# ai-forever/Kandinsky-2

Hardware: AMD Instinct MI355X
Metric: UNet denoise steps/sec @ 768x768 bs=1, 50 steps (higher is better)
Workload: dtype bf16; 1 GPU; Kandinsky-2.x text2img 768x768, decoder_steps=50, bs=1/GPU (CFG batch 2x4x96x96), 2.1-architecture UNet (1.23B) p_sampler step; parity pinned against the reference's modules; head=2.1, tile_configs_measured_in_this_process=0, images_per_gpu=1, parallelism=prompt-sharded x1, weights by one RCCL broadcast, world_size_observed=1, graph=True, chains=1, loop_graph=a 5-step loop replayed as ONE hipGraph (83 replay(s) = 415 timed steps)

## Files before the change

### include/k22.h

```cpp
#ifndef K22_H
#define K22_H
#include <stddef.h>
#include <stdint.h>
#ifdef __cplusplus
extern "C" {
#endif

#define K22_OK 0
#define K22_EINVAL (-1)
#define K22_EHIP (-2)
#define K22_ENOMEM (-3)

#define K22_BF16 0
#define K22_F32 1
#define K22_F16 2
#define K22_F16X3 3
#define K22_F16X2 4

int k22_version(void);
#define K22_BUILD_PACKED_FP32 1
#define K22_BUILD_DEBUG_VARIANTS 2
int k22_build_flags(void);
const char* k22_last_error(void);
int k22_set_option(const char* name, int value);
// ... 48 lines not shown

int k22_unet_sample_loop(K22UNet* u, float* x, float* x_tmp, const float* timesteps, const float* noise_seq, const float* init_img,
                         const float* mask, const float* inpaint_image, const float* inpaint_mask, const float* table,
                         const int* table_rows, int n_steps, float guidance, float clamp_lo, float clamp_hi, int pct_index,
                         double pct_gamma, void* scratch, int use_graph, void* stream);
enum { K22_LOOP_DDIM = 0, K22_LOOP_PLMS = 1 };
int k22_unet_ddim_loop(K22UNet* u, int kind, float* x, float* x_tmp, float* x0_out, const float* timesteps, const float* table,
                       const float* noise_seq, const float* inpaint_image, const float* inpaint_mask, float* eps_hist, int n_steps,
                       float guidance, int use_graph, void* stream);
int k22_unet_num_ops(const K22UNet* u);
int k22_unet_set_autotune(K22UNet* u, int on);
int k22_unet_tuning_report(const K22UNet* u, char* buf, size_t cap);

int k22_comm_broadcast_weights(void* arena, size_t bytes, int root, void* nccl_comm, void* stream);

int k22_tile_table_load(const char* path);
int k22_tile_table_save(const char* path);
int k22_tile_table_size(void);
int k22_tile_table_measured(void);
void k22_tile_table_clear(void);

int k22_unet_profile(K22UNet* u, int reps, double* ms, double* flops, double* bytes, int* launches, void* stream);

size_t k22_sampler_scratch_bytes(int N, int HW);
int k22_ddim_step(const float* x, const float* model_out, const float* noise, const float* table_row, float guidance, int use_cfg,
                  float* x_out, float* x0_out, int N, int HW, void* stream);
int k22_prepare_mask(const float* mask, float* out, int C, int H, int W, void* stream);
int k22_plms_step(const float* x, const float* model_out, const float* eps_hist1, const float* eps_hist2, const float* eps_hist3, int order,
                  const float* table_row, float guidance, int use_cfg, float* x_out, float* eps_out, float* x0_out, int N, int HW, void* stream);
int k22_sampler_step(const float* x, const float* model_out, const float* noise, const float* init_img,
                     const float* mask, const float* table, int step_index, float guidance, int use_cfg,
                     float clamp_lo, float clamp_hi, int pct_index, double pct_gamma, void* scratch,
                     float* x_out, float* x0_out, int N, int HW, void* stream);

int k22_gemm(const void* A0, const void* A1, const void* Wp, const float* bias, const void* residual, void* out,
             void* partial, int M, int N, int Npad, int K0, int K1, long lda0, long lda1, int ldo, int ldr,
             int out_f32, int act, int splitk, int bm, int bn, int dtype, void* stream);
int k22_x3_pack(const float* src, void* dst, long n, float scale, void* stream);
int k22_conv3x3(const void* x_padded, const void* Wp, const float* bias, const void* residual, void* out,
                void* partial, int B, int H, int W, int Cin, int Cout, int Npad, int out_mode, int act, int splitk,
                int bm, int bn, int dtype, void* stream);
int k22_conv3x3_skip(const void* x_padded, const void* Wp, const float* bias, const void* skip0, const void* skip1,
                     int SK0, int SK1, const void* Ws, const float* bias_s, void* out, void* partial, int B, int H, int W,
                     int Cin, int Cout, int Npad, int splitk, int bm, int dtype, void* stream);
int k22_conv3x3_gnstats(const void* x_padded, const void* Wp, const float* bias, const void* residual, void* out,
                        void* partial, int B, int H, int W, int Cin, int Cout, int Npad, int splitk, int bm, int bn,
                        float* stats, int stats_capacity_rows, int* rows_per_image, int dtype, void* stream);
int k22_gemm_gnstats(const void* A, const void* Wp, const float* bias, const void* residual, void* out, void* partial,
                     int B, int H, int W, int N, int Npad, int K, int splitk, int bm, float* stats,
                     int stats_capacity_rows, int* rows_per_image, int dtype, void* stream);
typedef struct K22IgemmProblem {
  int dtype, taps, M, N, Kc, K0, H, W;
  int out_mode, res_f32, act, a_raw, want_stats;
  int SK0, SK1;
  int att_T, att_S, att_Tkp;
  int ldo, ldr;
  int has_frag;
  int algo, bm, bn, splitk, stages;
} K22IgemmProblem;
typedef struct K22IgemmOperands {
  const void *A0, *A1, *Wp, *bias, *residual;
  void *out, *partial;
  const void *S0, *S1, *Ws, *bias2;
  void *kall, *vtall;
  const void *Wfrag, *Wsfrag;
  float* stats;
  int stats_capacity_rows;
} K22IgemmOperands;
int k22_igemm_cfg_accepted(const K22IgemmProblem* pr);
int k22_igemm_cfg(const K22IgemmProblem* pr, const K22IgemmOperands* ops, int* rows_per_image, void* stream);
int k22_debug_conv_trace(const void* x_padded, const void* Wp, const float* bias, void* out, int B, int H, int W, int Cin, int Cout,
                         int Npad, unsigned long long* trace, void* stream);
int k22_conv3x3_gn(const void* x0, const void* x1, int C0, int C1, const float* gamma, const float* beta, const float* film, long film_ld,
                   float eps, int act, void* scratch, const void* Wp, const float* bias, const void* residual, void* out, void* partial,
                   int B, int H, int W, int Cout, int Npad, int splitk, int bm, int algo, int dtype, void* stream);
int k22_groupnorm(const void* x0, const void* x1, int C0, int C1, int B, int H, int W, const float* gamma,
                  const float* beta, const float* film, long film_ld, float eps, int act, int mode, int pad,
                  void* scratch, void* out, int dtype, void* stream);
size_t k22_groupnorm_scratch_bytes(int B, int C);
int k22_attention(const void* qkv, const void* ctxkv, void* kall, void* vtall, void* out, int B, int H, int T, int S,
                  int dtype, void* stream);
int k22_qkv_project(const void* x, const void* Wp, const float* bias, void* q_out, void* kall, void* vtall,
                    int B, int H, int T, int S, int K, int bm, int bn, int dtype, void* stream);
int k22_qkv_project_stream(const void* x, const void* Wp, const float* bias, void* q_out, void* kall, void* vtall, void* partial,
                           int B, int H, int T, int S, int K, int bm, int splitk, int dtype, void* stream);
int k22_linear_smallm(const float* x, const void* W, const float* bias, const float* add, float* out, int M, int N,
                      int K, int act_in, int act_out, int wdtype, void* stream);
int k22_conv3x3_direct(const float* x, const float* w, const float* bias, float* y, int B, int Cin, int Cout, int Hin, int Win,
                       int stride, int act, void* stream);

size_t k22_afrag_bytes(int M, int K);
int k22_afrag_pack(const void* A, long lda, void* out, int M, int K, int dtype, void* stream);
int k22_skinny_gemm(const void* Afrag, const void* Wfrag, const float* bias, void* out, float* partial, int M, int N, int Npad, int K,
                    int splitk, int epi, int act, int ldo, int mt, int nb, int dtype, void* stream);
int k22_finish_ln(const float* partial, int splitk, const float* bias, float* x, long ldx, const float* gain, const float* beta, void* yfrag,
                  int M, int N, float eps, int dtype, void* stream);
int k22_small_attention(const void* qkv, const float* qkv_partial, int nsplit, const float* qkv_bias, void* out, int out_frag, int B, int H, int T,
                        int causal, const float* key_valid, int kv_n, int dtype, void* stream);

typedef struct K22PriorConfig {
  int dtype;
  int text_ctx;
  int xf_width;
  int xf_layers;
  int xf_heads;
  int xf_final_ln;
  int clip_dim;
  int clip_xf_width;
} K22PriorConfig;
typedef struct K22Prior K22Prior;
int k22_prior_create(const K22PriorConfig* cfg, const K22Weight* weights, int n_weights, K22Prior** out);
void k22_prior_destroy(K22Prior* m);
int k22_prior_plan(K22Prior* m, int B, size_t* workspace_bytes);
int k22_prior_bind(K22Prior* m, void* workspace, size_t workspace_bytes);
int k22_prior_tuning_report(const K22Prior* m, char* buf, size_t cap);
int k22_prior_forward(K22Prior* m, const float* x, const float* timesteps, const float* text_emb, const float* text_enc,
                      const float* key_valid, float* out, void* stream);
int k22_prior_sampler_step(const float* x, const float* model_out, const float* noise, const float* scales, const float* table_row,
                           float clamp, float* x_out, int bs, int D, void* stream);

typedef struct K22MoVQConfig {
  int dtype;
  int ch;
  int n_levels;
  int ch_mult[8];
  int num_res_blocks;
  int attn_levels;
  int z_channels;
  int out_ch;
} K22MoVQConfig;
typedef struct K22MoVQ K22MoVQ;
int k22_movq_create(const K22MoVQConfig* cfg, const K22Weight* weights, int n_weights, K22MoVQ** out);
void k22_movq_destroy(K22MoVQ* m);
int k22_movq_plan(K22MoVQ* m, int B, int h, int w, size_t* workspace_bytes);
int k22_movq_bind(K22MoVQ* m, void* workspace, size_t workspace_bytes);
int k22_movq_decode(K22MoVQ* m, const float* z, float* out, unsigned char* out_u8, void* stream);
int k22_movq_plan_encoder(K22MoVQ* m, int B, int H, int W, size_t* workspace_bytes);
int k22_movq_encode(K22MoVQ* m, const float* image, float* latent, void* stream);
int k22_movq_num_ops(const K22MoVQ* m);

enum { K22_ENC_CLIP_TEXT = 0, K22_ENC_CLIP_VISION = 1, K22_ENC_XLMR = 2 };
typedef struct K22EncoderConfig {
  int dtype;
  int kind;
  int width;
  int layers;
  int heads;
  int n_ctx;
  int vocab;
  int out_dim;
  int image_size;
  int patch;
  int max_pos;
  int pad_id;
  float ln_eps;
  int mlp_dim;
  int hidden_act;
} K22EncoderConfig;
typedef struct K22Encoder K22Encoder;
int k22_encoder_create(const K22EncoderConfig* cfg, const K22Weight* weights, int n_weights, K22Encoder** out);
void k22_encoder_destroy(K22Encoder* m);
int k22_encoder_plan(K22Encoder* m, int B, size_t* workspace_bytes);
int k22_encoder_bind(K22Encoder* m, void* workspace, size_t workspace_bytes);
int k22_encoder_forward(K22Encoder* m, const int* tokens, const float* key_valid, const float* image, float* seq_out, float* pooled_out,
                        void* stream);

// ... 34 lines not shown
```

### kandinsky-2_amd/_lib.py

```python
from __future__ import annotations

import ctypes as C
import os

_HERE = os.path.dirname(os.path.abspath(__file__))
LIB_PATH = os.environ.get("K22_LIB_PATH") or os.path.join(_HERE, "libk22hip.so")
TILE_TABLE_PATH = os.path.join(_HERE, "tiles_gfx950.txt")

K22_BF16, K22_F32, K22_F16, K22_F16X3, K22_F16X2 = 0, 1, 2, 3, 4
K22_LOOP_DDIM, K22_LOOP_PLMS = 0, 1
F16X3 = "f16x3"
F16X2 = "f16x2"
SPLIT_DTYPES = (F16X3, F16X2)
X3_WSCALE = 256.0


def dtype_code(backend_dtype) -> int:
    import torch
    try:
        return {torch.bfloat16: K22_BF16, torch.float32: K22_F32, torch.float16: K22_F16, F16X3: K22_F16X3, F16X2: K22_F16X2}[backend_dtype]
    except KeyError:
        raise ValueError('backend_dtype must be torch.bfloat16, torch.float16, torch.float32 "f16x3" or "f16x2"') from None
ACT_NONE, ACT_SILU, ACT_GELU = 0, 1, 2
OUT_ROWMAJOR, OUT_ROWMAJOR_F32, OUT_NCHW_F32, OUT_QKV = 0, 1, 2, 3
# ... 32 lines not shown


class K22EncoderConfig(C.Structure):
    _fields_ = [("dtype", C.c_int), ("kind", C.c_int), ("width", C.c_int), ("layers", C.c_int), ("heads", C.c_int), ("n_ctx", C.c_int),
                ("vocab", C.c_int), ("out_dim", C.c_int), ("image_size", C.c_int), ("patch", C.c_int), ("max_pos", C.c_int),
                ("pad_id", C.c_int), ("ln_eps", C.c_float), ("mlp_dim", C.c_int), ("hidden_act", C.c_int)]


class K22Weight(C.Structure):
    _fields_ = [("name", C.c_char_p), ("ptr", C.c_void_p)]


_P, _I, _L, _F, _D, _Z = C.c_void_p, C.c_int, C.c_long, C.c_float, C.c_double, C.c_size_t

SIGNATURES = {
    "k22_version": (_I, []),
    "k22_build_flags": (_I, []),
    "k22_last_error": (C.c_char_p, []),
    "k22_set_option": (_I, [C.c_char_p, _I]),
    "k22_comm_broadcast_weights": (_I, [_P, _Z, _I, _P, _P]),
    "k22_tile_table_load": (_I, [C.c_char_p]),
    "k22_tile_table_save": (_I, [C.c_char_p]),
    "k22_tile_table_size": (_I, []),
    "k22_tile_table_measured": (_I, []),
    "k22_tile_table_clear": (None, []),
    "k22_unet_create": (_I, [C.POINTER(K22UNetConfig), C.POINTER(K22Weight), _I, C.POINTER(_P)]),
    "k22_unet_destroy": (None, [_P]),
    "k22_unet_plan": (_I, [_P, _I, _I, _I, C.POINTER(_Z)]),
    "k22_unet_bind": (_I, [_P, _P, _Z]),
    "k22_unet_set_condition": (_I, [_P, _P, _P, _P, _P]),
    "k22_unet_set_hint": (_I, [_P, _P, _P]),
    "k22_unet_forward": (_I, [_P, _P, _P, _P, _P, _P, _I, _P]),
    "k22_unet_sample_loop": (_I, [_P, _P, _P, _P, _P, _P, _P, _P, _P, _P, C.POINTER(_I), _I, _F, _F, _F, _I, _D, _P, _I, _P]),
    "k22_unet_ddim_loop": (_I, [_P, _I, _P, _P, _P, _P, _P, _P, _P, _P, _P, _I, _F, _I, _P]),
    "k22_unet_num_ops": (_I, [_P]),
    "k22_unet_set_autotune": (_I, [_P, _I]),
    "k22_unet_tuning_report": (_I, [_P, C.c_char_p, _Z]),
    "k22_unet_profile": (_I, [_P, _I, C.POINTER(_D), C.POINTER(_D), C.POINTER(_D), C.POINTER(_I), _P]),
    "k22_afrag_bytes": (_Z, [_I, _I]),
    "k22_afrag_pack": (_I, [_P, _L, _P, _I, _I, _I, _P]),
    "k22_skinny_gemm": (_I, [_P, _P, _P, _P, _P, _I, _I, _I, _I, _I, _I, _I, _I, _I, _I, _I, _P]),
    "k22_finish_ln": (_I, [_P, _I, _P, _P, _L, _P, _P, _P, _I, _I, _F, _I, _P]),
    "k22_small_attention": (_I, [_P, _P, _I, _P, _P, _I, _I, _I, _I, _I, _P, _I, _I, _P]),
    "k22_prior_create": (_I, [C.POINTER(K22PriorConfig), C.POINTER(K22Weight), _I, C.POINTER(_P)]),
    "k22_prior_destroy": (None, [_P]),
    "k22_prior_plan": (_I, [_P, _I, C.POINTER(_Z)]),
    "k22_prior_bind": (_I, [_P, _P, _Z]),
    "k22_prior_tuning_report": (_I, [_P, C.c_char_p, _Z]),
    "k22_prior_forward": (_I, [_P, _P, _P, _P, _P, _P, _P, _P]),
    "k22_prior_sampler_step": (_I, [_P, _P, _P, _P, _P, _F, _P, _I, _I, _P]),
    "k22_encoder_create": (_I, [C.POINTER(K22EncoderConfig), C.POINTER(K22Weight), _I, C.POINTER(_P)]),
    "k22_encoder_destroy": (None, [_P]),
    "k22_encoder_plan": (_I, [_P, _I, C.POINTER(_Z)]),
    "k22_encoder_bind": (_I, [_P, _P, _Z]),
    "k22_encoder_forward": (_I, [_P, _P, _P, _P, _P, _P, _P]),
    "k22_movq_create": (_I, [C.POINTER(K22MoVQConfig), C.POINTER(K22Weight), _I, C.POINTER(_P)]),
    "k22_movq_destroy": (None, [_P]),
    "k22_movq_plan": (_I, [_P, _I, _I, _I, C.POINTER(_Z)]),
    "k22_movq_bind": (_I, [_P, _P, _Z]),
    "k22_movq_decode": (_I, [_P, _P, _P, _P, _P]),
    "k22_movq_plan_encoder": (_I, [_P, _I, _I, _I, C.POINTER(_Z)]),
    "k22_movq_encode": (_I, [_P, _P, _P, _P]),
    "k22_movq_num_ops": (_I, [_P]),
    "k22_ddim_step": (_I, [_P, _P, _P, _P, _F, _I, _P, _P, _I, _I, _P]),
    "k22_blend_noised": (_I, [_P, _P, _P, _P, _F, _F, _P, _I, _I, _I, _I, _P]),
    "k22_prepare_mask": (_I, [_P, _P, _I, _I, _I, _P]),
    "k22_plms_step": (_I, [_P, _P, _P, _P, _P, _I, _P, _F, _I, _P, _P, _P, _I, _I, _P]),
    "k22_sampler_scratch_bytes": (_Z, [_I, _I]),
    "k22_sampler_step": (_I, [_P, _P, _P, _P, _P, _P, _I, _F, _I, _F, _F, _I, _D, _P, _P, _P, _I, _I, _P]),
    "k22_gemm": (_I, [_P, _P, _P, _P, _P, _P, _P, _I, _I, _I, _I, _I, _L, _L, _I, _I, _I, _I, _I, _I, _I, _I, _P]),
    "k22_x3_pack": (_I, [_P, _P, _L, _F, _P]),
    "k22_conv3x3": (_I, [_P, _P, _P, _P, _P, _P, _I, _I, _I, _I, _I, _I, _I, _I, _I, _I, _I, _I, _P]),
    "k22_conv3x3_skip": (_I, [_P, _P, _P, _P, _P, _I, _I, _P, _P, _P, _P, _I, _I, _I, _I, _I, _I, _I, _I, _I, _P]),
    "k22_gemm_gnstats": (_I, [_P, _P, _P, _P, _P, _P, _I, _I, _I, _I, _I, _I, _I, _I, _P, _I, C.POINTER(_I), _I, _P]),
    "k22_conv3x3_gnstats": (_I, [_P, _P, _P, _P, _P, _P, _I, _I, _I, _I, _I, _I, _I, _I, _I, _P, _I, C.POINTER(_I), _I, _P]),
    "k22_igemm_cfg_accepted": (_I, [C.POINTER(K22IgemmProblem)]),
    "k22_igemm_cfg": (_I, [C.POINTER(K22IgemmProblem), C.POINTER(K22IgemmOperands), C.POINTER(_I), _P]),
    "k22_conv3x3_gn": (_I, [_P, _P, _I, _I, _P, _P, _P, _L, _F, _I, _P, _P, _P, _P, _P, _P, _I, _I, _I, _I, _I, _I, _I, _I, _I, _P]),
    "k22_debug_conv_trace": (_I, [_P, _P, _P, _P, _I, _I, _I, _I, _I, _I, _P, _P]),
    "k22_groupnorm": (_I, [_P, _P, _I, _I, _I, _I, _I, _P, _P, _P, _L, _F, _I, _I, _I, _P, _P, _I, _P]),
    "k22_groupnorm_scratch_bytes": (_Z, [_I, _I]),
    "k22_attention": (_I, [_P, _P, _P, _P, _P, _I, _I, _I, _I, _I, _P]),
    "k22_qkv_project": (_I, [_P, _P, _P, _P, _P, _P, _I, _I, _I, _I, _I, _I, _I, _I, _P]),
    "k22_qkv_project_stream": (_I, [_P, _P, _P, _P, _P, _P, _P, _I, _I, _I, _I, _I, _I, _I, _I, _P]),
    "k22_linear_smallm": (_I, [_P, _P, _P, _P, _P, _I, _I, _I, _I, _I, _I, _P]),
    "k22_conv3x3_direct": (_I, [_P, _P, _P, _P, _I, _I, _I, _I, _I, _I, _I, _P]),
    "k22_debug_counter": (_L, [C.c_char_p]),
    "k22_stream_frag_bytes": (C.c_size_t, [_I, _I, _I, _I]),
    "k22_stream_repack": (_I, [_P, _P, _I, _I, _I, _I, _P]),
    "k22_debug_set_stream_frag": (_I, [_P, _P]),
    "k22_debug_set_stream_scratch": (_I, [_P, C.c_size_t]),
    "k22_spatialnorm_apply": (_I, [_P, _P, _P, _P, _P, _P, _P, _P, _I, _I, _I, _I, _I, _I, _I, _I, _I, _I, _P]),
    "k22_upsample2_pad": (_I, [_P, _P, _I, _I, _I, _I, _I, _P]),
    "k22_pad_copy": (_I, [_P, _P, _I, _I, _I, _I, _I, _P]),
    "k22_subsample_odd": (_I, [_P, _P, _I, _I, _I, _I, _I, _P]),
    "k22_softmax_rows": (_I, [_P, _L, _I, _F, _I, _P]),
    "k22_movq_prepare": (_I, [_P, _P, _P, _P, _P, _I, _I, _I, _I, _I, _P]),
    "k22_movq_enc_prepare": (_I, [_P, _P, _I, _I, _I, _I, _I, _P]),
    "k22_movq_quant_conv": (_I, [_P, _P, _P, _P, _I, _I, _P]),
    "k22_to_uint8_nhwc": (_I, [_P, _P, _I, _I, _I, _I, _P]),
    "k22_enc_layernorm": (_I, [_P, _L, _P, _P, _P, _L, _P, _I, _I, _F, _I, _P]),
    "k22_enc_embed": (_I, [_P, _P, _P, _P, _P, _I, _I, _I, _I, _I, _I, _I, _P]),
    "k22_enc_gather_eot": (_I, [_P, _P, _P, _I, _I, _I, _P]),
    "k22_enc_masked_mean": (_I, [_P, _P, _P, _I, _I, _I, _P]),
    "k22_enc_patchify": (_I, [_P, _P, _I, _I, _I, _I, _I, _P]),
    "k22_enc_vision_assemble": (_I, [_P, _P, _P, _P, _I, _I, _I, _P]),
    "k22_enc_mlp_act": (_I, [_P, _P, _L, _I, _I, _P]),
    "k22_enc_attention_generic": (_I, [_P, _P, _I, _I, _I, _I, _I, _P]),
    "k22_prior_layernorm": (_I, [_P, _L, _P, _P, _P, _I, _I, _I, _I, _P]),
    "k22_prior_finish_input": (_I, [_P, _P, _P, _I, _I, _I, _P]),
    "k22_attention_masked": (_I, [_P, _P, _P, _P, _P, _I, _I, _I, _I, _I, _P, _I, _I, _I, _P]),
}

_lib = None


def lib() -> C.CDLL:
    global _lib
    if _lib is None:
        if not os.path.exists(LIB_PATH):
            raise RuntimeError(
                f"{LIB_PATH} is missing: the HIP extension is the only compute path (no CPU fallback). "
                "Build it with `python -c 'import __graft_entry__ as g; g.build()'`.")
        l = C.CDLL(LIB_PATH)
        for name, (res, args) in SIGNATURES.items():
            fn = getattr(l, name)
            fn.restype = res
            fn.argtypes = args
        _lib = l
        tbl = os.environ.get("K22_TILE_TABLE", TILE_TABLE_PATH)
        if tbl != "0" and os.path.exists(tbl):
            if l.k22_tile_table_load(tbl.encode()) < 0:
                raise RuntimeError(f"k22: cannot read the tile table {tbl}")
    return _lib


def check(rc: int) -> None:
    if rc != 0:
        msg = lib().k22_last_error()
        raise RuntimeError(f"k22 error {rc}: {msg.decode() if msg else ''}")


def weight_array(arena, table):
    base = arena.data_ptr()
    arr = (K22Weight * len(table))()
    names = []
    for i, (name, (off, _n)) in enumerate(table.items()):
        nb = name.encode()
        names.append(nb)
        arr[i].name = nb
        arr[i].ptr = base + off
    return arr, names


def plan_and_bind(plan_fn, bind_fn, handle, device, *shape):
    import torch
    nbytes = C.c_size_t()
    check(plan_fn(handle, *shape, C.byref(nbytes)))
    ws = torch.empty(nbytes.value + 256, dtype=torch.uint8, device=device)
    check(bind_fn(handle, (ws.data_ptr() + 255) // 256 * 256, nbytes.value))
    return ws


def ptr(t) -> int:
    if t is None:
        return None
# ... 8 lines not shown
```

### kandinsky-2_amd/csrc/capi.hip

```cpp
#include "kernels.h"
#include "elementwise.h"
#include "../../include/k22.h"
#include "tuning.h"
#include "skinny.h"
#include <dlfcn.h>
#include <stdio.h>
#include <string.h>

static thread_local char g_err[512] = "";

int k22_set_error(int code, const char* msg) {
  snprintf(g_err, sizeof(g_err), "%s", msg ? msg : "");
  return code;
}
int k22_set_error_hip(hipError_t e, const char* file, int line) {
  snprintf(g_err, sizeof(g_err), "HIP error %d (%s) at %s:%d", (int)e, hipGetErrorString(e), file, line);
  return K22_EHIP;
}

extern "C" {

int k22_version(void) { return 100; }
int k22_build_flags(void) {
  int f = 0;
#ifndef K22_NOPK
  f |= K22_BUILD_PACKED_FP32;
#endif
#if defined(K22_DEBUG_VARIANTS) || defined(K22_STREAM_DEBUG) || defined(K22_SKINNY_DEBUG)
  f |= K22_BUILD_DEBUG_VARIANTS;
#endif
  return f;
}

int k22_set_option(const char* name, int value) {
  if (name && !strcmp(name, "igemm_stages")) { igemm_set_default_stages(value); return K22_OK; }
  if (name && !strcmp(name, "igemm_xcd_remap")) { igemm_set_xcd_remap(value); return K22_OK; }
  if (name && !strcmp(name, "conv_algo")) { igemm_set_conv_algo(value); return K22_OK; }
  if (name && !strcmp(name, "gemm_algo")) { igemm_set_gemm_algo(value); return K22_OK; }
  if (name && !strcmp(name, "att_pipe")) { attention_set_pipe(value); return K22_OK; }
  return k22_set_error(K22_EINVAL, "k22_set_option: unknown option");
}
const char* k22_last_error(void) { return g_err; }

#ifdef K22_STREAM_DEBUG
static unsigned long long* g_dbg_trace = nullptr;
extern "C" int k22_debug_set_stream_trace(unsigned long long* t) { g_dbg_trace = t; return K22_OK; }
#define K22_DBG_TRACE(p) (p).st_trace = g_dbg_trace
#else
#define K22_DBG_TRACE(p) (void)0
#endif
static const void* g_dbg_wfrag = nullptr;
static const void* g_dbg_wsfrag = nullptr;
static void* g_dbg_scratch = nullptr;
static size_t g_dbg_scratch_bytes = 0;
static int dbg_frag(IgemmParams& p, int dtype, hipStream_t st) {
  K22_DBG_TRACE(p);
  p.Wfrag = g_dbg_wfrag; p.Wsfrag = g_dbg_wsfrag;
  if (g_dbg_wfrag || !g_dbg_scratch || dtype == K22_F32 || (p.taps != 1 && p.taps != 9) || p.Kc % 64 || p.Npad % 64) return K22_OK;
  const size_t n1 = stream_frag_bytes(p.Npad, p.taps, p.Kc, dtype);
  const bool skip = p.S0 != nullptr && p.Ws != nullptr && (p.SK0 + p.SK1) % 64 == 0;
  const size_t n2 = skip ? stream_frag_bytes(p.Npad, 1, p.SK0 + p.SK1, dtype) : 0;
  if (n1 + n2 > g_dbg_scratch_bytes) return k22_set_error(K22_ENOMEM, "debug stream scratch too small");
  if (int rc = launch_stream_repack(p.Wp, g_dbg_scratch, p.Npad, p.taps, p.Kc, dtype, st)) return rc;
  p.Wfrag = g_dbg_scratch;
  if (skip) {
    void* w2 = static_cast<char*>(g_dbg_scratch) + n1;
    if (int rc = launch_stream_repack(p.Ws, w2, p.Npad, 1, p.SK0 + p.SK1, dtype, st)) return rc;
    p.Wsfrag = w2;
  }
  return K22_OK;
}
#define K22_DBG_FRAG(p) do { if (int rc_ = dbg_frag((p), dtype, reinterpret_cast<hipStream_t>(stream))) return rc_; } while (0)
int k22_debug_set_stream_frag(const void* wfrag, const void* wsfrag) { g_dbg_wfrag = wfrag; g_dbg_wsfrag = wsfrag; return K22_OK; }
int k22_debug_set_stream_scratch(void* scratch, size_t bytes) { g_dbg_scratch = scratch; g_dbg_scratch_bytes = scratch ? bytes : 0; return K22_OK; }
size_t k22_stream_frag_bytes(int Npad, int taps, int Kc, int dtype) { return stream_frag_bytes(Npad, taps, Kc, dtype); }
int k22_stream_repack(const void* W, void* out, int Npad, int taps, int Kc, int dtype, void* stream) {
  return launch_stream_repack(W, out, Npad, taps, Kc, dtype, reinterpret_cast<hipStream_t>(stream));
}

long k22_debug_counter(const char* name) {
  if (name && !strcmp(name, "stream_launches")) return stream_launch_count();
  if (name && !strcmp(name, "loop_captures")) return loop_capture_count();
  if (name && !strcmp(name, "loop_launches")) return loop_launch_count();
  return -1;
}

int k22_comm_broadcast_weights(void* arena, size_t bytes, int root, void* nccl_comm, void* stream) {
  if (!arena || !nccl_comm) return k22_set_error(K22_EINVAL, "k22_comm_broadcast_weights: null arena / communicator");
  typedef int (*bcast_fn)(const void*, void*, size_t, int , int, void*, hipStream_t);
  static bcast_fn fn = nullptr;
  if (!fn) {
    void* sym = dlsym(RTLD_DEFAULT, "ncclBroadcast");
    if (!sym) {
      void* h = dlopen("librccl.so.1", RTLD_NOW | RTLD_GLOBAL);
      if (!h) h = dlopen("librccl.so", RTLD_NOW | RTLD_GLOBAL);
      if (h) sym = dlsym(h, "ncclBroadcast");
    }
    if (!sym) return k22_set_error(K22_EINVAL, "k22_comm_broadcast_weights: RCCL (ncclBroadcast) is not loadable in this process");
    fn = reinterpret_cast<bcast_fn>(sym);
  }
  const size_t piece = (size_t)1 << 30;
  char* base = reinterpret_cast<char*>(arena);
  for (size_t off = 0; off < bytes; off += piece) {
    const size_t n = bytes - off < piece ? bytes - off : piece;
    const int rc = fn(base + off, base + off, n,  1, root, nccl_comm, reinterpret_cast<hipStream_t>(stream));
    if (rc != 0) { char msg[96]; snprintf(msg, sizeof msg, "k22_comm_broadcast_weights: ncclBroadcast returned %d", rc); return k22_set_error(K22_EHIP, msg); }
  }
  return K22_OK;
}

int k22_tile_table_load(const char* path) {
  if (!path) return k22_set_error(K22_EINVAL, "k22_tile_table_load: null path");
  const int n = tile_table_load_file(path);
  if (n < 0) return k22_set_error(K22_EINVAL, "k22_tile_table_load: cannot read the file");
  return n;
}
int k22_tile_table_save(const char* path) {
  if (!path) return k22_set_error(K22_EINVAL, "k22_tile_table_save: null path");
  const int n = tile_table_save_file(path);
  if (n < 0) return k22_set_error(K22_EINVAL, "k22_tile_table_save: cannot write the file");
  return n;
}
int k22_tile_table_size(void) {
  TileTable& tt = tile_table();
  std::lock_guard<std::mutex> lk(tt.mu);
  return (int)tt.m.size();
}
int k22_tile_table_measured(void) {
  TileTable& tt = tile_table();
  std::lock_guard<std::mutex> lk(tt.mu);
  return (int)tt.measured;
}
void k22_tile_table_clear(void) {
  TileTable& tt = tile_table();
  std::lock_guard<std::mutex> lk(tt.mu);
  tt.m.clear();
  tt.measured = 0;
}

int k22_gemm(const void* A0, const void* A1, const void* Wp, const float* bias, const void* residual, void* out,
             void* partial, int M, int N, int Npad, int K0, int K1, long lda0, long lda1, int ldo, int ldr,
             int out_f32, int act, int splitk, int bm, int bn, int dtype, void* stream) {
  IgemmParams p = {};
    p.stages = -1;
  p.A0 = A0; p.A1 = A1; p.Wp = Wp; p.bias = bias; p.residual = residual; p.out = out;
  p.partial = reinterpret_cast<float*>(partial);
  p.M = M; p.N = N; p.Npad = Npad; p.Kc = K0 + K1; p.K0 = K0; p.taps = 1; p.lda0 = lda0; p.lda1 = lda1;
  p.ldo = ldo; p.ldr = ldr; p.out_mode = out_f32 ? IG_OUT_ROWMAJOR_F32 : IG_OUT_ROWMAJOR; p.act = act;
  p.splitk = splitk; p.force_bm = bm; p.force_bn = bn;
  p.a_raw = k22_is_split(dtype) ? 1 : 0;
  if (p.splitk == 0) p.splitk = partial ? igemm_choose_splitk(p, dtype) : 1;
  K22_DBG_FRAG(p);
  return launch_igemm(p, dtype, reinterpret_cast<hipStream_t>(stream));
}

int k22_x3_pack(const float* src, void* dst, long n, float scale, void* stream) {
  if (!src || !dst || n < 0) return k22_set_error(K22_EINVAL, "x3_pack: null argument");
  return launch_x3_pack(src, dst, n, scale, reinterpret_cast<hipStream_t>(stream));
}

int k22_conv3x3(const void* x_padded, const void* Wp, const float* bias, const void* residual, void* out,
                void* partial, int B, int H, int W, int Cin, int Cout, int Npad, int out_mode, int act, int splitk,
                int bm, int bn, int dtype, void* stream) {
  IgemmParams p = {};
    p.stages = -1;
  p.A0 = x_padded; p.Wp = Wp; p.bias = bias; p.residual = residual; p.out = out;
// ... 127 lines not shown
  }
  return launch_igemm(q, d.dtype, reinterpret_cast<hipStream_t>(stream));
}

int k22_debug_conv_trace(const void* x_padded, const void* Wp, const float* bias, void* out, int B, int H, int W, int Cin, int Cout,
                         int Npad, unsigned long long* trace, void* stream) {
  IgemmParams p = {};
  p.stages = -1;
  p.A0 = x_padded; p.Wp = Wp; p.bias = bias; p.out = out;
  p.M = B * H * W; p.N = Cout; p.Npad = Npad; p.Kc = Cin; p.K0 = Cin; p.taps = 9; p.H = H; p.W = W;
  p.ldo = Cout; p.ldr = Cout; p.out_mode = IG_OUT_ROWMAJOR; p.act = K22_ACT_NONE; p.splitk = 1; p.trace = trace;
  return launch_conv3_halo_trace(p, K22_BF16, reinterpret_cast<hipStream_t>(stream));
}

size_t k22_groupnorm_scratch_bytes(int B, int C) {
  return (size_t)B * 128 * C * 2 * sizeof(float) + (size_t)B * C * 2 * sizeof(float) + 512;
}

int k22_groupnorm(const void* x0, const void* x1, int C0, int C1, int B, int H, int W, const float* gamma,
                  const float* beta, const float* film, long film_ld, float eps, int act, int mode, int pad,
                  void* scratch, void* out, int dtype, void* stream) {
  hipStream_t st = reinterpret_cast<hipStream_t>(stream);
  const int C = C0 + C1, HW = H * W;
  const int out_x3 = k22_is_split(dtype) ? 1 : 0;
  dtype = k22_storage_dtype(dtype);
  float* partial = reinterpret_cast<float*>(scratch);
  float* coeff = partial + (size_t)B * 128 * C * 2;
  const int rc = launch_gn_stats_coeff(x0, x1, C0, C1, B, HW, eps, gamma, beta, film, film_ld, partial, coeff, dtype, st);
  if (rc) return rc;
  GnApplyParams ap = {};
  ap.x0 = x0; ap.x1 = x1; ap.C0 = C0; ap.C1 = C1; ap.B = B; ap.H = H; ap.W = W; ap.mode = mode; ap.pad = pad; ap.act = act;
  ap.coeff = coeff; ap.out = out; ap.out_x3 = out_x3;
  return launch_gn_apply(ap, dtype, st);
}

int k22_conv3x3_gn(const void* x0, const void* x1, int C0, int C1, const float* gamma, const float* beta, const float* film, long film_ld,
                   float eps, int act, void* scratch, const void* Wp, const float* bias, const void* residual, void* out, void* partial,
                   int B, int H, int W, int Cout, int Npad, int splitk, int bm, int algo, int dtype, void* stream) {
  hipStream_t st = reinterpret_cast<hipStream_t>(stream);
  const int C = C0 + C1, HW = H * W;
  const int sdt = k22_storage_dtype(dtype);
  float* part = reinterpret_cast<float*>(scratch);
  float* coeff = part + (size_t)B * 128 * C * 2;
  const int rc = launch_gn_stats_coeff(x0, x1, C0, C1, B, HW, eps, gamma, beta, film, film_ld, part, coeff, sdt, st);
  if (rc) return rc;
  IgemmParams p = {};
  p.stages = -1;
  p.Wp = Wp; p.bias = bias; p.residual = residual; p.out = out; p.partial = reinterpret_cast<float*>(partial);
  p.M = B * H * W; p.N = Cout; p.Npad = Npad; p.Kc = C; p.K0 = C; p.taps = 9; p.H = H; p.W = W;
  p.ldo = Cout; p.ldr = Cout; p.out_mode = IG_OUT_ROWMAJOR; p.act = K22_ACT_NONE; p.splitk = splitk > 0 ? splitk : 1; p.force_bm = bm; p.algo = algo;
  p.gn_coeff = coeff; p.gn_x0 = x0; p.gn_x1 = x1; p.gn_C0 = C0; p.gn_act = act;
  return launch_igemm(p, dtype, st);
}


int k22_attention(const void* qkv, const void* ctxkv, void* kall, void* vtall, void* out, int B, int H, int T, int S,
                  int dtype, void* stream) {
  hipStream_t st = reinterpret_cast<hipStream_t>(stream);
  const int C = H * 64, Tk = S + T, Tkp = (Tk + 63) / 64 * 64;
  KvPackParams kp;
  kp.qkv = qkv; kp.ctxkv = ctxkv; kp.kall = kall; kp.vtall = vtall; kp.B = B; kp.H = H; kp.T = T; kp.S = S; kp.Tkp = Tkp;
  int rc = launch_kv_pack(kp, k22_storage_dtype(dtype), st);
  if (rc) return rc;
  AttentionParams ap = {};
  ap.q = qkv; ap.ldq = 3 * C; ap.kall = kall; ap.vtall = vtall; ap.out = out; ap.ldo = C;
  ap.B = B; ap.H = H; ap.T = T; ap.Tk = Tk; ap.Tkp = Tkp; ap.scale = 0.125f;
  return launch_attention(ap, dtype, st);
}

int k22_qkv_project(const void* x, const void* Wp, const float* bias, void* q_out, void* kall, void* vtall,
                    int B, int H, int T, int S, int K, int bm, int bn, int dtype, void* stream) {
  const int C = H * 64, Tkp = (S + T + 63) / 64 * 64;
  IgemmParams p = {};
  p.stages = -1;
  p.A0 = x; p.Wp = Wp; p.bias = bias; p.out = q_out; p.kall = kall; p.vtall = vtall;
  p.M = B * T; p.N = 3 * C; p.Npad = 3 * C; p.Kc = K; p.K0 = K; p.taps = 1; p.lda0 = K; p.lda1 = 0;
  p.ldo = C; p.ldr = 3 * C; p.out_mode = IG_OUT_QKV; p.act = K22_ACT_NONE; p.splitk = 1; p.force_bm = bm; p.force_bn = bn;
  p.att_T = T; p.att_S = S; p.att_Tkp = Tkp; p.H = 1; p.W = T;
  p.a_raw = k22_is_split(dtype) ? 1 : 0;
  K22_DBG_FRAG(p);
  return launch_igemm(p, dtype, reinterpret_cast<hipStream_t>(stream));
}

int k22_qkv_project_stream(const void* x, const void* Wp, const float* bias, void* q_out, void* kall, void* vtall, void* partial,
                           int B, int H, int T, int S, int K, int bm, int splitk, int dtype, void* stream) {
  const int C = H * 64, Tkp = (S + T + 63) / 64 * 64;
  IgemmParams p = {};
  p.stages = -1;
  p.A0 = x; p.Wp = Wp; p.bias = bias; p.out = q_out; p.kall = kall; p.vtall = vtall; p.partial = reinterpret_cast<float*>(partial);
  p.M = B * T; p.N = 3 * C; p.Npad = 3 * C; p.Kc = K; p.K0 = K; p.taps = 1; p.lda0 = K; p.lda1 = 0;
  p.ldo = C; p.ldr = 3 * C; p.out_mode = IG_OUT_QKV; p.act = K22_ACT_NONE; p.splitk = splitk > 0 ? splitk : 1; p.force_bm = bm; p.algo = 20;
  p.att_T = T; p.att_S = S; p.att_Tkp = Tkp; p.H = 1; p.W = T;
  if (!stream_supported(p, dtype, bm == 288 ? 9 : 5)) return k22_set_error(K22_EINVAL, "qkv_project_stream: unsupported problem");
  K22_DBG_FRAG(p);
  return launch_igemm(p, dtype, reinterpret_cast<hipStream_t>(stream));
}

size_t k22_afrag_bytes(int M, int K) { return afrag_bytes(M, K); }
int k22_afrag_pack(const void* A, long lda, void* out, int M, int K, int dtype, void* stream) {
  return launch_afrag_pack(A, lda, out, M, K, dtype, reinterpret_cast<hipStream_t>(stream));
}
int k22_skinny_gemm(const void* Afrag, const void* Wfrag, const float* bias, void* out, float* partial, int M, int N, int Npad, int K,
                    int splitk, int epi, int act, int ldo, int mt, int nb, int dtype, void* stream) {
  SkinnyParams q = {};
  q.Af = Afrag; q.Wf = Wfrag; q.bias = bias; q.out = out; q.partial = partial; q.M = M; q.N = N; q.Npad = Npad; q.K = K; q.MA = (M + 31) / 32;
  q.splitk = splitk > 0 ? splitk : 1; q.epi = epi; q.act = act; q.ldo = ldo;
  q.trace = reinterpret_cast<unsigned long long*>(g_dbg_scratch);
  return launch_skinny(q, dtype, mt, nb, reinterpret_cast<hipStream_t>(stream));
}
int k22_finish_ln(const float* partial, int splitk, const float* bias, float* x, long ldx, const float* gain, const float* beta, void* yfrag,
                  int M, int N, float eps, int dtype, void* stream) {
  FinishLnParams q = {};
  q.partial = partial; q.splitk = splitk; q.bias = bias; q.x = x; q.ldx = ldx; q.g = gain; q.b = beta; q.yfrag = yfrag; q.M = M; q.N = N;
  q.MA = (M + 31) / 32; q.eps = eps;
  return launch_finish_ln(q, dtype, reinterpret_cast<hipStream_t>(stream));
}
int k22_small_attention(const void* qkv, const float* qkv_partial, int nsplit, const float* qkv_bias, void* out, int out_frag, int B, int H, int T,
                        int causal, const float* key_valid, int kv_n, int dtype, void* stream) {
  SmallAttnParams ap = {};
  ap.qkv = qkv; ap.part = qkv_partial; ap.nsplit = nsplit; ap.bias = qkv_bias; ap.ldq = 3 * H * 64; ap.out = out; ap.ldo = H * 64; ap.out_frag = out_frag; ap.MA = (B * T + 31) / 32;
  ap.B = B; ap.H = H; ap.T = T; ap.scale = 0.125f; ap.causal = causal; ap.key_valid = key_valid; ap.kv_ld = kv_n; ap.kv_n = kv_n;
  return launch_small_attention(ap, dtype, reinterpret_cast<hipStream_t>(stream));
}

int k22_linear_smallm(const float* x, const void* W, const float* bias, const float* add, float* out, int M, int N,
                      int K, int act_in, int act_out, int wdtype, void* stream) {
  LinearSmallParams lp = {};
  lp.x = x; lp.ldx = K; lp.W = W; lp.bias = bias; lp.add = add; lp.ld_add = N; lp.out = out; lp.ldo = N;
  lp.M = M; lp.N = N; lp.K = K; lp.act_in = act_in; lp.act_out = act_out;
  return launch_linear_smallm(lp, wdtype, reinterpret_cast<hipStream_t>(stream));
}

int k22_conv3x3_direct(const float* x, const float* w, const float* bias, float* y, int B, int Cin, int Cout, int Hin, int Win,
                       int stride, int act, void* stream) {
  if (!x || !w || !bias || !y) return k22_set_error(K22_EINVAL, "conv3x3_direct: null argument");
  if (B < 1 || Cin < 1 || Cout < 1 || Hin < 1 || Win < 1) return k22_set_error(K22_EINVAL, "conv3x3_direct: empty shape");
  if (act != K22_ACT_NONE && act != K22_ACT_SILU) return k22_set_error(K22_EINVAL, "conv3x3_direct: act must be 0 (none) or 1 (SiLU)");
  ConvDirectParams p = {};
  p.x = x; p.w = w; p.bias = bias; p.y = y;
  p.B = B; p.Cin = Cin; p.Cout = Cout; p.Hin = Hin; p.Win = Win; p.stride = stride; p.act = act;
  return launch_conv3x3_direct(p, reinterpret_cast<hipStream_t>(stream));
}

int k22_ddim_step(const float* x, const float* model_out, const float* noise, const float* table_row, float guidance, int use_cfg,
                  float* x_out, float* x0_out, int N, int HW, void* stream) {
  if (!x || !model_out || !table_row || !x_out) return k22_set_error(K22_EINVAL, "ddim_step: null argument");
  return launch_ddim_step(x, model_out, noise, table_row, guidance, use_cfg, x_out, x0_out, N, HW, reinterpret_cast<hipStream_t>(stream));
}

int k22_prepare_mask(const float* mask, float* out, int C, int H, int W, void* stream) {
  if (!mask || !out) return k22_set_error(K22_EINVAL, "prepare_mask: null argument");
  return launch_prepare_mask(mask, out, C, H, W, reinterpret_cast<hipStream_t>(stream));
}

int k22_plms_step(const float* x, const float* model_out, const float* eps_hist1, const float* eps_hist2, const float* eps_hist3, int order,
                  const float* table_row, float guidance, int use_cfg, float* x_out, float* eps_out, float* x0_out, int N, int HW, void* stream) {
  if (!x || !model_out || !table_row || !x_out) return k22_set_error(K22_EINVAL, "plms_step: null argument");
  return launch_plms_step(x, model_out, eps_hist1, eps_hist2, eps_hist3, order, table_row, guidance, use_cfg, x_out, eps_out, x0_out, N, HW,
                          reinterpret_cast<hipStream_t>(stream));
}

size_t k22_sampler_scratch_bytes(int N, int HW) { return (size_t)N * 4 * HW * sizeof(float) + 256; }

int k22_sampler_step(const float* x, const float* model_out, const float* noise, const float* init_img,
                     const float* mask, const float* table, int step_index, float guidance, int use_cfg,
                     float clamp_lo, float clamp_hi, int pct_index, double pct_gamma, void* scratch,
// ... 98 lines not shown
```

### kandinsky-2_amd/csrc/conv3_halo.hip

```cpp
#include "conv3_common.h"

int launch_conv3_halo_spec(const IgemmParams& p, int dtype, int bm, int nbst, int splitk, hipStream_t stream);
#ifdef K22_DEBUG_VARIANTS
int launch_conv3_halo_spec_debug(const IgemmParams& p, int nbst, int splitk, hipStream_t stream);
#endif

template <typename T, int BM, int NBST, bool TRACE = false, int LW = 8, int MODE = 0>
__global__ __launch_bounds__(512) void conv3_halo_kernel(const IgemmParams p) {
  constexpr bool PIPE = MODE == 1;
  constexpr bool GASM = MODE == 1 || MODE == 2;
  constexpr bool DBG_NOLOAD = MODE == 3;
  constexpr bool DBG_NOMMA = MODE == 4;
  using TR = TT<T>;
  constexpr int BK = TR::BK, EPC = TR::EPC, KSTEPS = TR::KSTEPS;
  constexpr int BN = HALO_BN, NW = LW, WM = 4, WN = 2;
  constexpr int MI = BM / (WM * 32), NI = BN / (WN * 32);
  constexpr int B_SLOTS = BN / 8 / NW;
  constexpr int B_BYTES = BN * 128;
  constexpr int APT = HALO_NW / LW;
  constexpr int A_SLOTS = (10 - NBST) * APT;
  constexpr int GM = 8;
  extern __shared__ __attribute__((aligned(16))) char smem[];

  const int tid = threadIdx.x, lane = tid & 63;
// ... 130 lines not shown
          constexpr int ta_ = ((TAP) + NBST - 1) % 9;                                                      \
          const int sa_ = ((TAP) + NBST - 1 >= 9) ? sn : s;                                                \
          K22_ISSUE_B(sa_, ta_, fill);                                                                     \
          if constexpr ((TAP) <= 9 - NBST) {                                                               \
            _Pragma("unroll") for (int a_ = 0; a_ < APT; ++a_) {                                           \
              constexpr int qb_ = ((TAP) <= 9 - NBST ? (TAP) : 0) * APT;                                   \
              K22_ISSUE_A(qb_ + a_, sn, Anext);                                                            \
            }                                                                                              \
          }                                                                                                \
        }                                                                                                  \
        const char* Bcur = Bst + cur * B_BYTES;                                                            \
        const int shift = ((TAP) / 3) * W2 + ((TAP) % 3);                                                  \
        const char* arow[MI];                                                                              \
        int asw[MI];                                                                                       \
        _Pragma("unroll") for (int mi = 0; mi < MI; ++mi) {                                                \
          const int ar = abase + mi * 32 + shift;                                                          \
          arow[mi] = Acur + ar * 128;                                                                      \
          asw[mi] = (ar >> 1) & 7;                                                                         \
        }                                                                                                  \
        if constexpr (PIPE) {                                                                              \
          FragA<T> ca[MI];                                                                                 \
          Frag<T> cb[NI];                                                                                  \
          _Pragma("unroll") for (int ks = 0; ks < KSTEPS; ks += 2) {                                       \
            _Pragma("unroll") for (int mi = 0; mi < MI; ++mi) ld_frag_at(ca[mi], arow[mi], asw[mi], ks, h); \
            _Pragma("unroll") for (int ni = 0; ni < NI; ++ni) ld_frag_at(cb[ni], Bcur + brow[ni], bsw, ks, h); \
            __builtin_amdgcn_sched_barrier(0);                                                             \
            _Pragma("unroll") for (int mi = 0; mi < MI; ++mi)                                              \
              _Pragma("unroll") for (int ni = 0; ni < NI; ++ni) mma_atom(acc[mi][ni], pb[ni], pa[mi]);     \
            __builtin_amdgcn_sched_barrier(0);                                                             \
            _Pragma("unroll") for (int mi = 0; mi < MI; ++mi) ld_frag_at(pa[mi], arow[mi], asw[mi], ks + 1, h); \
            _Pragma("unroll") for (int ni = 0; ni < NI; ++ni) ld_frag_at(pb[ni], Bcur + brow[ni], bsw, ks + 1, h); \
            __builtin_amdgcn_sched_barrier(0);                                                             \
            _Pragma("unroll") for (int mi = 0; mi < MI; ++mi)                                              \
              _Pragma("unroll") for (int ni = 0; ni < NI; ++ni) mma_atom(acc[mi][ni], cb[ni], ca[mi]);     \
            __builtin_amdgcn_sched_barrier(0);                                                             \
          }                                                                                                \
           \
          asm volatile("s_waitcnt lgkmcnt(0)" ::: "memory");                                               \
        } else {                                                                                           \
        _Pragma("unroll") for (int ks = 0; ks < KSTEPS; ++ks) {                                            \
          FragA<T> a[MI];                                                                                  \
          Frag<T> b[NI];                                                                                   \
          _Pragma("unroll") for (int mi = 0; mi < MI; ++mi) ld_frag_at(a[mi], arow[mi], asw[mi], ks, h);   \
          _Pragma("unroll") for (int ni = 0; ni < NI; ++ni) ld_frag_at(b[ni], Bcur + brow[ni], bsw, ks, h); \
          if constexpr (DBG_NOMMA) {                                                                       \
            _Pragma("unroll") for (int mi = 0; mi < MI; ++mi) asm volatile("" ::"v"(a[mi].v));             \
            _Pragma("unroll") for (int ni = 0; ni < NI; ++ni) asm volatile("" ::"v"(b[ni].v));             \
          } else {                                                                                         \
          _Pragma("unroll") for (int mi = 0; mi < MI; ++mi)                                                \
            _Pragma("unroll") for (int ni = 0; ni < NI; ++ni) mma_atom(acc[mi][ni], b[ni], a[mi]);         \
          }                                                                                                \
        }                                                                                                  \
         \
        asm volatile("s_waitcnt lgkmcnt(0)" ::: "memory");                                                 \
        }                                                                                                  \
        if constexpr (TRACE) {                                                                             \
                      \
          asm volatile("" ::"v"(acc[0][0][0]), "v"(acc[MI - 1][NI - 1][15]));                             \
          const unsigned long long tr3_ = __builtin_amdgcn_s_memtime();                                    \
          if (blockIdx.x == 0 && (wave == 0 || wave == 5) && lane == 0 && p.trace != nullptr) {            \
            unsigned long long* o_ = p.trace + ((size_t)(wave ? 1 : 0) * 4096 + (size_t)trace_it * 4);     \
            if (trace_it < 1024) { o_[0] = tr0_; o_[1] = tr1_; o_[2] = tr2_; o_[3] = tr3_; }                \
          }                                                                                                \
          ++trace_it;                                                                                      \
        }                                                                                                  \
        cur = (cur + 1 == NBST) ? 0 : cur + 1;                                                             \
        fill = (fill + 1 == NBST) ? 0 : fill + 1;                                                          \
      }
      K22_TAP(0) K22_TAP(1) K22_TAP(2) K22_TAP(3) K22_TAP(4) K22_TAP(5) K22_TAP(6) K22_TAP(7) K22_TAP(8)
#undef K22_TAP
    }
  }
#undef K22_ISSUE_A
#undef K22_ISSUE_B
  if constexpr (PIPE) {
#pragma unroll
    for (int mi = 0; mi < MI; ++mi)
#pragma unroll
      for (int ni = 0; ni < NI; ++ni) mma_atom(acc[mi][ni], pb[ni], pa[mi]);
  }
  halo_tail<T, BM>(p, acc, smem, bx, bz, img, v0, n0);
}

template <typename T, int BM, int NST, bool ARAW = false>
__global__ __launch_bounds__(512) void gemm8_kernel(const IgemmParams p) {
  using TR = TT<T>;
  constexpr int BK = TR::BK, EPC = TR::EPC, KSTEPS = TR::KSTEPS;
  constexpr int BN = HALO_BN, NW = HALO_NW, WM = 4, WN = 2;
  constexpr int MI = BM / (WM * 32), NI = BN / (WN * 32);
  constexpr int A_SLOTS = BM / 8 / NW, B_SLOTS = BN / 8 / NW, CH = A_SLOTS + B_SLOTS;
  constexpr int A_BYTES = BM * 128, B_BYTES = BN * 128, BUF = A_BYTES + B_BYTES;
  constexpr int GM = 8;
  extern __shared__ __attribute__((aligned(16))) char smem[];

  const int tid = threadIdx.x, lane = tid & 63;
  const int wave = __builtin_amdgcn_readfirstlane(tid >> 6);
  const int wm = wave >> 1, wn = wave & 1;
  const int h = lane >> 5, l31 = lane & 31;

  const int HW = p.H > 0 ? p.H * p.W : p.M;
  const int TPI = (HW + BM - 1) / BM;
  const int B = p.M / HW;
  const int gx = B * TPI, gy = (p.N + BN - 1) / BN;
  int L = p.xcd_remap ? xcd_remap_h(blockIdx.x, gridDim.x) : (int)blockIdx.x;
  const int per_z = gx * gy;
  const int bz = L / per_z;
  L -= bz * per_z;
  const int grp = L / (GM * gy);
  const int first_m = grp * GM;
  const int gsz = gx - first_m < GM ? gx - first_m : GM;
  const int lin = L - grp * GM * gy;
  const int bx = first_m + lin % gsz, by = lin / gsz;
  const int img = bx / TPI, v0 = (bx - img * TPI) * BM;
  const int n0 = by * BN;

  const T* __restrict__ A = reinterpret_cast<const T*>(p.A0) + (int64_t)img * HW * p.lda0;
  const T* __restrict__ Wp = reinterpret_cast<const T*>(p.Wp);
  int aoff[A_SLOTS], boff[B_SLOTS];
#pragma unroll
  for (int i = 0; i < A_SLOTS; ++i) {
    const int row = 8 * (wave + NW * i) + (lane >> 3);
    int v = v0 + row;
    if (v > HW - 1) v = HW - 1;
    aoff[i] = v * (int)p.lda0 + ((lane & 7) ^ ((row >> 1) & 7)) * EPC;
  }
#pragma unroll
  for (int i = 0; i < B_SLOTS; ++i) {
    const int row = 8 * (wave + NW * i) + (lane >> 3);
    int n = n0 + row;
    if (n > p.Npad - 1) n = p.Npad - 1;
    boff[i] = n * p.Kc + ((lane & 7) ^ ((row >> 1) & 7)) * EPC;
  }
  const int nslab = p.Kc / BK;
  int s0 = 0, s1 = nslab;
  if (p.splitk > 1) {
    const int per = (nslab + p.splitk - 1) / p.splitk;
    s0 = bz * per;
    s1 = s0 + per < nslab ? s0 + per : nslab;
  }

  f32x16_t acc[MI][NI];
#pragma unroll
  for (int mi = 0; mi < MI; ++mi)
#pragma unroll
    for (int ni = 0; ni < NI; ++ni)
#pragma unroll
      for (int r = 0; r < 16; ++r) acc[mi][ni][r] = 0.f;

  const unsigned lds0 = __builtin_amdgcn_readfirstlane((unsigned)(size_t)(__attribute__((address_space(3))) char*)smem);
#define K22_ISSUE_G(SLAB, STAGE)                                                                           \
  {                                                                                                        \
    int sl_ = (SLAB);                                                                                      \
    if (sl_ > s1 - 1) sl_ = s1 - 1;       \
    const unsigned d_ = lds0 + (STAGE) * BUF + wave * 1024;                                                \
    _Pragma("unroll") for (int i = 0; i < A_SLOTS; ++i)                                                    \
        glds16_asm(A + aoff[i] + sl_ * BK, __builtin_amdgcn_readfirstlane(d_ + i * NW * 1024));            \
    _Pragma("unroll") for (int i = 0; i < B_SLOTS; ++i)                                                    \
        glds16w_asm(Wp + boff[i] + sl_ * BK, __builtin_amdgcn_readfirstlane(d_ + A_BYTES + i * NW * 1024)); \
  }
  int arow[MI], brow[NI];
#pragma unroll
  for (int mi = 0; mi < MI; ++mi) arow[mi] = (wm * (BM / WM) + mi * 32 + l31) * 128;
#pragma unroll
  for (int ni = 0; ni < NI; ++ni) brow[ni] = A_BYTES + (wn * (BN / WN) + ni * 32 + l31) * 128;
  const int sw = (l31 >> 1) & 7;

  if (s0 < s1) {
#pragma unroll
    for (int t = 0; t < NST - 1; ++t) K22_ISSUE_G(s0 + t, t);
    int cur = 0, fill = NST - 1;
    for (int s = s0; s < s1; ++s) {
      wait_vmcnt<(NST - 2) * CH>();
      raw_barrier();
      K22_ISSUE_G(s + NST - 1, fill);
      const char* St = smem + cur * BUF;
#pragma unroll
      for (int ks = 0; ks < KSTEPS; ++ks) {
        FragA<T> a[MI];
        Frag<T> b[NI];
#pragma unroll
        for (int mi = 0; mi < MI; ++mi) ld_frag_at_a<ARAW, T>(a[mi], St + arow[mi], sw, ks, h);
#pragma unroll
        for (int ni = 0; ni < NI; ++ni) ld_frag_at(b[ni], St + brow[ni], sw, ks, h);
#pragma unroll
        for (int mi = 0; mi < MI; ++mi)
#pragma unroll
          for (int ni = 0; ni < NI; ++ni) mma_atom(acc[mi][ni], b[ni], a[mi]);
      }
      cur = (cur + 1 == NST) ? 0 : cur + 1;
      fill = (fill + 1 == NST) ? 0 : fill + 1;
    }
  }
#undef K22_ISSUE_G
  halo_tail<T, BM, true>(p, acc, smem, bx, bz, img, v0, n0);
}

template <typename T, int BM, int NST>
__global__ __launch_bounds__(512) void gemm8_spec_kernel(const IgemmParams p) {
  using TR = TT<T>;
  static_assert(sizeof(T) == 2, "gemm8_spec_kernel: 16-bit operands");
  constexpr int BK = TR::BK, EPC = TR::EPC, KSTEPS = TR::KSTEPS;
  static_assert(KSTEPS % 2 == 0, "two-set fragment pipeline");
  constexpr int BN = HALO_BN, NWL = 4, WM = 2, WN = 2;
  constexpr int MI = BM / (WM * 32), NI = BN / (WN * 32);
  constexpr int A_SLOTS = BM / 8 / NWL, B_SLOTS = BN / 8 / NWL, CH = A_SLOTS + B_SLOTS;
  constexpr int A_BYTES = BM * 128, B_BYTES = BN * 128, BUF = A_BYTES + B_BYTES;
  constexpr int GM = 8;
  extern __shared__ __attribute__((aligned(16))) char smem[];

  const int tid = threadIdx.x, lane = tid & 63;
  const int wave = __builtin_amdgcn_readfirstlane(tid >> 6);
  const bool producer = wave >= 4;
  const int h = lane >> 5, l31 = lane & 31;

  const int HW = p.H > 0 ? p.H * p.W : p.M;
  const int TPI = (HW + BM - 1) / BM;
  const int B = p.M / HW;
  const int gx = B * TPI, gy = (p.N + BN - 1) / BN;
  int L = p.xcd_remap ? xcd_remap_h(blockIdx.x, gridDim.x) : (int)blockIdx.x;
  const int per_z = gx * gy;
  const int bz = L / per_z;
  L -= bz * per_z;
  const int grp = L / (GM * gy);
  const int first_m = grp * GM;
  const int gsz = gx - first_m < GM ? gx - first_m : GM;
  const int lin = L - grp * GM * gy;
  const int bx = first_m + lin % gsz, by = lin / gsz;
  const int img = bx / TPI, v0 = (bx - img * TPI) * BM;
  const int n0 = by * BN;

  const int nslab = p.Kc / BK;
  int s0 = 0, s1 = nslab;
  if (p.splitk > 1) {
    const int per = (nslab + p.splitk - 1) / p.splitk;
    s0 = bz * per;
    s1 = s0 + per < nslab ? s0 + per : nslab;
  }

  f32x16_t acc[MI][NI];
#pragma unroll
  for (int mi = 0; mi < MI; ++mi)
#pragma unroll
    for (int ni = 0; ni < NI; ++ni)
#pragma unroll
      for (int r = 0; r < 16; ++r) acc[mi][ni][r] = 0.f;

  if (s0 < s1) {
    if (producer) {
      const int lw = wave - 4;
      const T* __restrict__ A = reinterpret_cast<const T*>(p.A0) + (int64_t)img * HW * p.lda0;
      const T* __restrict__ Wp = reinterpret_cast<const T*>(p.Wp);
      int aoff[A_SLOTS], boff[B_SLOTS];
#pragma unroll
      for (int i = 0; i < A_SLOTS; ++i) {
        const int row = 8 * (lw + NWL * i) + (lane >> 3);
        int v = v0 + row;
        if (v > HW - 1) v = HW - 1;
        aoff[i] = v * (int)p.lda0 + ((lane & 7) ^ ((row >> 1) & 7)) * EPC;
      }
#pragma unroll
      for (int i = 0; i < B_SLOTS; ++i) {
        const int row = 8 * (lw + NWL * i) + (lane >> 3);
        int n = n0 + row;
        if (n > p.Npad - 1) n = p.Npad - 1;
        boff[i] = n * p.Kc + ((lane & 7) ^ ((row >> 1) & 7)) * EPC;
      }
      const unsigned lds0 = __builtin_amdgcn_readfirstlane((unsigned)(size_t)(__attribute__((address_space(3))) char*)smem);
#define K22_ISSUE_GS(SLAB, STAGE)                                                                          \
      {                                                                                                    \
        int sl_ = (SLAB);                                                                                  \
        if (sl_ > s1 - 1) sl_ = s1 - 1;    \
        const unsigned d_ = lds0 + (STAGE) * BUF + lw * 1024;                                              \
        _Pragma("unroll") for (int i = 0; i < A_SLOTS; ++i)                                                \
            glds16_asm(A + aoff[i] + sl_ * BK, __builtin_amdgcn_readfirstlane(d_ + i * NWL * 1024));       \
        _Pragma("unroll") for (int i = 0; i < B_SLOTS; ++i)                                                \
            glds16w_asm(Wp + boff[i] + sl_ * BK, __builtin_amdgcn_readfirstlane(d_ + A_BYTES + i * NWL * 1024)); \
      }
#pragma unroll
      for (int t = 0; t < NST - 1; ++t) K22_ISSUE_GS(s0 + t, t);
      int fill = NST - 1;
      for (int s = s0; s < s1; ++s) {
        wait_vmcnt<(NST - 2) * CH>();
        raw_barrier();
        K22_ISSUE_GS(s + NST - 1, fill);
        fill = (fill + 1 == NST) ? 0 : fill + 1;
      }
#undef K22_ISSUE_GS
    } else {
      const int wm = wave >> 1, wn = wave & 1;
      int arow[MI], brow[NI];
#pragma unroll
      for (int mi = 0; mi < MI; ++mi) arow[mi] = (wm * (BM / WM) + mi * 32 + l31) * 128;
#pragma unroll
      for (int ni = 0; ni < NI; ++ni) brow[ni] = A_BYTES + (wn * (BN / WN) + ni * 32 + l31) * 128;
      const int sw = (l31 >> 1) & 7;
      Frag<T> pa[MI], pb[NI];
#pragma unroll
      for (int mi = 0; mi < MI; ++mi) pa[mi] = Frag<T>{};
#pragma unroll
      for (int ni = 0; ni < NI; ++ni) pb[ni] = Frag<T>{};
      constexpr int NRD = MI + NI, NMF = MI * NI, MPR = NMF / NRD;
#define K22_GS_INTERLEAVE()                                                                                \
      {                                                                                                    \
        _Pragma("unroll") for (int i_ = 0; i_ < NRD; ++i_) {                                               \
          __builtin_amdgcn_sched_group_barrier(0x008, MPR, 0);                                             \
          __builtin_amdgcn_sched_group_barrier(0x100, 1, 0);                                               \
        }                                                                                                  \
        if constexpr (NMF - MPR * NRD > 0) __builtin_amdgcn_sched_group_barrier(0x008, NMF - MPR * NRD, 0); \
        __builtin_amdgcn_sched_barrier(0);                                                                 \
      }
      int cur = 0;
      for (int s = s0; s < s1; ++s) {
        raw_barrier();
        const char* St = smem + cur * BUF;
        Frag<T> ca[MI], cb[NI];
#pragma unroll
        for (int ks = 0; ks < KSTEPS; ks += 2) {
#pragma unroll
          for (int mi = 0; mi < MI; ++mi) ld_frag_at(ca[mi], St + arow[mi], sw, ks, h);
#pragma unroll
          for (int ni = 0; ni < NI; ++ni) ld_frag_at(cb[ni], St + brow[ni], sw, ks, h);
#pragma unroll
          for (int mi = 0; mi < MI; ++mi)
#pragma unroll
            for (int ni = 0; ni < NI; ++ni) mma_atom(acc[mi][ni], pb[ni], pa[mi]);
          K22_GS_INTERLEAVE();
#pragma unroll
          for (int mi = 0; mi < MI; ++mi) ld_frag_at(pa[mi], St + arow[mi], sw, ks + 1, h);
#pragma unroll
          for (int ni = 0; ni < NI; ++ni) ld_frag_at(pb[ni], St + brow[ni], sw, ks + 1, h);
#pragma unroll
          for (int mi = 0; mi < MI; ++mi)
#pragma unroll
            for (int ni = 0; ni < NI; ++ni) mma_atom(acc[mi][ni], cb[ni], ca[mi]);
          K22_GS_INTERLEAVE();
        }
        asm volatile("s_waitcnt lgkmcnt(0)" ::: "memory");
        cur = (cur + 1 == NST) ? 0 : cur + 1;
      }
#undef K22_GS_INTERLEAVE
#pragma unroll
      for (int mi = 0; mi < MI; ++mi)
#pragma unroll
        for (int ni = 0; ni < NI; ++ni) mma_atom(acc[mi][ni], pb[ni], pa[mi]);
    }
  }
  halo_tail<T, BM, true, true>(p, acc, smem, bx, bz, img, v0, n0);
}

namespace {
__device__ __forceinline__ void ld_frag64(Frag<bf16_t>& f, const char* rowp, int sw, int ks, int h) {
  f.v = *reinterpret_cast<const u32x4_t*>(rowp + (((2 * ks + h) ^ sw) << 4));
}
__device__ __forceinline__ void ld_frag64(Frag<f16_t>& f, const char* rowp, int sw, int ks, int h) {
  f.v = *reinterpret_cast<const u32x4_t*>(rowp + (((2 * ks + h) ^ sw) << 4));
}
__device__ __forceinline__ void ld_frag64(Frag<float>& f, const char* rowp, int sw, int , int h) {
  const float4 a = *reinterpret_cast<const float4*>(rowp + (((2 * h) ^ sw) << 4));
  const float4 b = *reinterpret_cast<const float4*>(rowp + (((2 * h + 1) ^ sw) << 4));
  f.v[0] = a.x; f.v[1] = a.y; f.v[2] = a.z; f.v[3] = a.w;
  f.v[4] = b.x; f.v[5] = b.y; f.v[6] = b.z; f.v[7] = b.w;
}
template <int RB> constexpr int halo3_wait(int ky) { return RB == 2 ? 0 : (RB == 3 ? (ky == 0 ? 3 : 6) : (ky == 0 ? 6 : (ky == 1 ? 9 : 12))); }
constexpr int HALO3_ASLOTS = 6;
}

template <typename T, int BM, int RB>
__global__ __launch_bounds__(512) void conv3_halo3_kernel(const IgemmParams p) {
  constexpr int EPH = 64 / (int)sizeof(T);
  constexpr int EPC = TT<T>::EPC;
  constexpr int KS_U = EPH / 16;
// ... 98 lines not shown
      K22_ISSUE_B3(hs_, j % 3, j);
    }
    int cur = 0, fill = RB - 1;
    for (int hs = h0; hs < h1; ++hs) {
      char* const Acur = smem + ((hs - h0) & 1) * A_BYTES;
      char* const Anext = smem + (((hs - h0) & 1) ^ 1) * A_BYTES;
      const int hn = hs + 1 < h1 ? hs + 1 : h1 - 1;
#define K22_IT3(KY)                                                                                        \
      {                                                                                                    \
        wait_vmcnt<halo3_wait<RB>(KY)>();                                                                  \
        raw_barrier();                                                                      \
        if constexpr ((KY) < 2) {                                                                          \
          K22_ISSUE_A3(3 * ((KY) < 2 ? (KY) : 0) + 0, hn, Anext);                                          \
          K22_ISSUE_A3(3 * ((KY) < 2 ? (KY) : 0) + 1, hn, Anext);                                          \
          K22_ISSUE_A3(3 * ((KY) < 2 ? (KY) : 0) + 2, hn, Anext);                                          \
        }                                                                                                  \
        {                                                                                                  \
          constexpr int kya_ = ((KY) + RB - 1) % 3;                                                        \
          int hsa_ = hs + ((KY) + RB - 1) / 3;                                                             \
          if (hsa_ > h1 - 1) hsa_ = h1 - 1;                                                                \
          K22_ISSUE_B3(hsa_, kya_, fill);                                                                  \
        }                                                                                                  \
        const char* Bcur = Bring + cur * BT_BYTES;                                                         \
        _Pragma("unroll") for (int kx = 0; kx < 3; ++kx) {                                                 \
          const int shift = (KY) * W2 + kx;                                                                \
          const char* arow[MI];                                                                            \
          int asw[MI];                                                                                     \
          _Pragma("unroll") for (int mi = 0; mi < MI; ++mi) {                                              \
            const int ar = abase + mi * 32 + shift;                                                        \
            arow[mi] = Acur + ar * 64;                                                                     \
            asw[mi] = (ar >> 2) & 3;                                                                       \
          }                                                                                                \
          _Pragma("unroll") for (int ks = 0; ks < KS_U; ++ks) {                                            \
            Frag<T> a[MI], b[NI];                                                                          \
            _Pragma("unroll") for (int mi = 0; mi < MI; ++mi) ld_frag64(a[mi], arow[mi], asw[mi], ks, h);  \
            _Pragma("unroll") for (int ni = 0; ni < NI; ++ni) ld_frag64(b[ni], Bcur + kx * BN * 64 + brow[ni], bsw, ks, h); \
            _Pragma("unroll") for (int mi = 0; mi < MI; ++mi)                                              \
              _Pragma("unroll") for (int ni = 0; ni < NI; ++ni) mma_atom(acc[mi][ni], b[ni], a[mi]);       \
          }                                                                                                \
        }                                                                                                  \
        cur = (cur + 1 == RB) ? 0 : cur + 1;                                                               \
        fill = (fill + 1 == RB) ? 0 : fill + 1;                                                            \
      }
      K22_IT3(0) K22_IT3(1) K22_IT3(2)
#undef K22_IT3
    }
  }
#undef K22_ISSUE_A3
#undef K22_ISSUE_B3
  halo_tail<T, BM>(p, acc, smem, bx, bz, img, v0, n0);
}

static int halo3_rows(const IgemmParams& p, int bm) { return (bm + 2 * (p.W + 2) + 2 + 15) & ~15; }
static size_t halo3_smem_bytes(const IgemmParams& p, int bm, int rb) {
  const size_t main_loop = (size_t)2 * halo3_rows(p, bm) * 64 + (size_t)rb * 3 * HALO_BN * 64;
  const size_t epi = (size_t)bm * (HALO_BN * 4 + 16);
  const size_t skip = p.S0 ? (size_t)(bm == 256 ? 3 : 4) * (bm * 128 + HALO_BN * 128) : 0;
  size_t m = main_loop > epi ? main_loop : epi;
  return m > skip ? m : skip;
}
static int halo3_pick_rb(const IgemmParams& p, int bm) {
  if (halo3_rows(p, bm) / 16 > HALO3_ASLOTS * HALO_NW) return 0;
  for (int rb : {4, 3, 2})
    if (halo3_smem_bytes(p, bm, rb) <= 160 * 1024) return rb;
  return 0;
}

static int gemm8_nst(int bm, int stages) { return bm == 256 ? 3 : (stages == 2 ? 2 : 4); }
static size_t gemm8_smem_bytes(int bm, int nst) {
  const size_t main_loop = (size_t)nst * (bm + HALO_BN) * 128;
  const size_t epi = (size_t)bm * (HALO_BN * 4 + 16);
  return main_loop > epi ? main_loop : epi;
}
int gemm8_tiles_per_image(const IgemmParams& p, int bm) { return ((p.H > 0 ? p.H * p.W : p.M) + bm - 1) / bm; }

bool gemm8_supported(const IgemmParams& p, int dtype, int bm) {
  const int BK = k22_bk(dtype);
  if (p.taps != 1 || (bm != 256 && bm != 128) || p.N < 128) return false;
  if (p.K0 != p.Kc || p.S0 != nullptr || p.res_f32) return false;
  if (p.out_mode != IG_OUT_ROWMAJOR && p.out_mode != IG_OUT_ROWMAJOR_F32 && p.out_mode != IG_OUT_QKV) return false;
  if (p.N % 8 || p.ldo % 8 || (p.residual && p.ldr % 8) || p.Kc % BK || p.lda0 % 8) return false;
  const int hw = p.H > 0 ? p.H * p.W : p.M;
  if (hw <= 0 || p.M % hw) return false;
  if (p.out_mode == IG_OUT_QKV && (p.att_T != hw || p.N % 384)) return false;
  if ((int64_t)p.M * p.lda0 >= (1ll << 31) || (int64_t)p.Npad * p.Kc >= (1ll << 31)) return false;
  return true;
}

template <typename T, int BM, int NST, bool ARAW = false>
static int launch_gemm8_cfg(const IgemmParams& p, int splitk, hipStream_t stream) {
  if constexpr (is_x3<T>::value && !ARAW) { if (p.a_raw) return launch_gemm8_cfg<T, BM, NST, true>(p, splitk, stream); }
  const size_t smem = gemm8_smem_bytes(BM, NST);
  static LdsAttrGuard attr_guard;
  if (int rc_ = k22_ensure_lds_attr(attr_guard, reinterpret_cast<const void*>(&gemm8_kernel<T, BM, NST, ARAW>), 160 * 1024, __FILE__, __LINE__)) return rc_;
  IgemmParams q = p;
  q.splitk = splitk;
  const int hw = p.H > 0 ? p.H * p.W : p.M;
  const int nblocks = (p.M / hw) * gemm8_tiles_per_image(p, BM) * ((p.N + HALO_BN - 1) / HALO_BN) * splitk;
  hipLaunchKernelGGL((gemm8_kernel<T, BM, NST, ARAW>), dim3(nblocks), dim3(512), smem, stream, q);
  K22_CHECK_LAUNCH();
  return K22_OK;
}

template <typename T, int BM, int NST>
static int launch_gemm8_spec_cfg(const IgemmParams& p, int splitk, hipStream_t stream) {
  const size_t smem = gemm8_smem_bytes(BM, NST);
  static LdsAttrGuard attr_guard;
  if (int rc_ = k22_ensure_lds_attr(attr_guard, reinterpret_cast<const void*>(&gemm8_spec_kernel<T, BM, NST>), 160 * 1024, __FILE__, __LINE__)) return rc_;
  IgemmParams q = p;
  q.splitk = splitk;
  const int hw = p.H > 0 ? p.H * p.W : p.M;
  const int nblocks = (p.M / hw) * gemm8_tiles_per_image(p, BM) * ((p.N + HALO_BN - 1) / HALO_BN) * splitk;
  hipLaunchKernelGGL((gemm8_spec_kernel<T, BM, NST>), dim3(nblocks), dim3(512), smem, stream, q);
  K22_CHECK_LAUNCH();
  return K22_OK;
}

bool gemm8_spec_supported(int dtype) { return dtype == K22_BF16 || dtype == K22_F16; }

int launch_gemm8(const IgemmParams& p, int dtype, int bm, int splitk, hipStream_t stream) {
  if (!gemm8_supported(p, dtype, bm)) return k22_set_error(K22_EINVAL, "gemm8: unsupported problem");
  if ((p.stages == 3 || p.stages == 4) && gemm8_spec_supported(dtype)) {
    if (p.stages == 4 && bm == 128) return dtype == K22_BF16 ? launch_gemm8_spec_cfg<bf16_t, 128, 2>(p, splitk, stream) : launch_gemm8_spec_cfg<f16_t, 128, 2>(p, splitk, stream);
    if (dtype == K22_BF16) return bm == 256 ? launch_gemm8_spec_cfg<bf16_t, 256, 3>(p, splitk, stream) : launch_gemm8_spec_cfg<bf16_t, 128, 4>(p, splitk, stream);
    return bm == 256 ? launch_gemm8_spec_cfg<f16_t, 256, 3>(p, splitk, stream) : launch_gemm8_spec_cfg<f16_t, 128, 4>(p, splitk, stream);
  }
  const int nst = gemm8_nst(bm, p.stages);
  if (dtype == K22_BF16) {
    if (bm == 256) return launch_gemm8_cfg<bf16_t, 256, 3>(p, splitk, stream);
    return nst == 2 ? launch_gemm8_cfg<bf16_t, 128, 2>(p, splitk, stream) : launch_gemm8_cfg<bf16_t, 128, 4>(p, splitk, stream);
  }
  if (dtype == K22_F16) {
    if (bm == 256) return launch_gemm8_cfg<f16_t, 256, 3>(p, splitk, stream);
    return nst == 2 ? launch_gemm8_cfg<f16_t, 128, 2>(p, splitk, stream) : launch_gemm8_cfg<f16_t, 128, 4>(p, splitk, stream);
  }
  if (dtype == K22_F16X3) {
    if (bm == 256) return launch_gemm8_cfg<x3_t, 256, 3>(p, splitk, stream);
    return nst == 2 ? launch_gemm8_cfg<x3_t, 128, 2>(p, splitk, stream) : launch_gemm8_cfg<x3_t, 128, 4>(p, splitk, stream);
  }
  if (dtype == K22_F16X2) {
    if (bm == 256) return launch_gemm8_cfg<x2_t, 256, 3>(p, splitk, stream);
    return nst == 2 ? launch_gemm8_cfg<x2_t, 128, 2>(p, splitk, stream) : launch_gemm8_cfg<x2_t, 128, 4>(p, splitk, stream);
  }
  if (bm == 256) return launch_gemm8_cfg<float, 256, 3>(p, splitk, stream);
  return nst == 2 ? launch_gemm8_cfg<float, 128, 2>(p, splitk, stream) : launch_gemm8_cfg<float, 128, 4>(p, splitk, stream);
}

bool conv3_halo_supported(const IgemmParams& p, int dtype, int bm) {
  const int BK = k22_bk(dtype);
  if (p.taps != 9 || (bm != 256 && bm != 128)) return false;
  if (k22_is_split(dtype) && (p.a_raw || p.algo == 3)) return false;
  if (p.gn_coeff != nullptr) {
    if (!conv3_algo_fuses_gn(p.algo) || !p.gn_x0 || p.gn_C0 <= 0 || p.gn_C0 > p.Kc || p.gn_C0 % BK || (p.gn_C0 < p.Kc && !p.gn_x1)) return false;
    if ((int64_t)p.H * p.W * p.Kc >= (1ll << 31)) return false;
  }
  if (p.out_mode != IG_OUT_ROWMAJOR && p.out_mode != IG_OUT_ROWMAJOR_F32) return false;
  if (p.N % 8 || p.ldo % 8 || (p.residual && p.ldr % 8) || p.Kc % BK) return false;
  if (p.H <= 0 || p.W <= 0 || p.M % (p.H * p.W)) return false;
  if (p.S0 != nullptr) {
    if (!p.Ws || p.SK0 % BK || p.SK1 % BK || (p.SK1 > 0 && !p.S1) || p.SK0 <= 0) return false;
    if ((int64_t)p.M * (p.SK0 > p.SK1 ? p.SK0 : p.SK1) >= (1ll << 31) || (int64_t)p.Npad * (p.SK0 + p.SK1) >= (1ll << 31)) return false;
  }
  if ((p.algo == 3 ? halo3_pick_rb(p, bm) : halo_pick_nbst(p, bm)) == 0) return false;
  if ((int64_t)(p.H + 2) * (p.W + 2) * p.Kc >= (1ll << 31) || (int64_t)p.Npad * 9 * p.Kc >= (1ll << 31)) return false;
  return true;
}

int conv3_halo_tiles_per_image(const IgemmParams& p, int bm) { return (p.H * (p.W + 2) + bm - 1) / bm; }

template <typename T, int BM, int NBST, int LW, int MODE>
static int launch_halo_cfg(const IgemmParams& p, int splitk, hipStream_t stream) {
  const size_t smem = halo_smem_bytes(p, BM, NBST);
  static LdsAttrGuard attr_guard;
  if (int rc_ = k22_ensure_lds_attr(attr_guard, reinterpret_cast<const void*>(&conv3_halo_kernel<T, BM, NBST, false, LW, MODE>), 160 * 1024, __FILE__, __LINE__)) return rc_;
  IgemmParams q = p;
  q.splitk = splitk;
  const int B = p.M / (p.H * p.W);
  const int nblocks = B * conv3_halo_tiles_per_image(p, BM) * ((p.N + HALO_BN - 1) / HALO_BN) * splitk;
  hipLaunchKernelGGL((conv3_halo_kernel<T, BM, NBST, false, LW, MODE>), dim3(nblocks), dim3(512), smem, stream, q);
  K22_CHECK_LAUNCH();
  return K22_OK;
}

template <typename T, int BM, int LW, int MODE>
static int launch_halo_nbst(const IgemmParams& p, int nbst, int splitk, hipStream_t stream) {
  if (nbst == 2) return launch_halo_cfg<T, BM, 2, LW, MODE>(p, splitk, stream);
  if (nbst == 3) return launch_halo_cfg<T, BM, 3, LW, MODE>(p, splitk, stream);
  if (nbst <= 5) return launch_halo_cfg<T, BM, 4, LW, MODE>(p, splitk, stream);
  return launch_halo_cfg<T, BM, 6, LW, MODE>(p, splitk, stream);
}

template <typename T, int BM, int RB>
static int launch_halo3_cfg(const IgemmParams& p, int splitk, hipStream_t stream) {
  const size_t smem = halo3_smem_bytes(p, BM, RB);
  static LdsAttrGuard attr_guard;
  if (int rc_ = k22_ensure_lds_attr(attr_guard, reinterpret_cast<const void*>(&conv3_halo3_kernel<T, BM, RB>), 160 * 1024, __FILE__, __LINE__)) return rc_;
// ... 83 lines not shown
```

### kandinsky-2_amd/csrc/elementwise.h

```cpp
#pragma once
#include "common.h"

struct GnStatsParams {
  const void* x0; const void* x1;
  int C0, C1, HW, B, groups, nsplit;
  float* partial;
};
struct GnSrc { const float* st; int rpi, C; };
struct GnCoeffParams {
  GnSrc src[2];
  int HW, C, groups; float eps;
  const float* gamma; const float* beta;
  const float* film; int64_t film_ld;
  float* coeff;
};
struct GnApplyParams {
  const void* x0; const void* x1; int C0, C1;
  int B, H, W;
  int mode;
  int pad;
  int act;
  const float* coeff;
  void* out;
  int out_x3;
};
struct ConvInParams {
  const float* x; const float* img; const float* mask;
  const float* w; const float* bias;
  void* out;
  int B, H, W, Cin, Cout;
  int img_premul;
};
struct ConvDirectParams {
  const float* x; const float* w; const float* bias; float* y;
  int B, Cin, Cout, Hin, Win, stride, act;
};
int launch_conv3x3_direct(const ConvDirectParams& p, hipStream_t s);
struct LinearSmallParams {
  const float* x; int64_t ldx;
  const void* W;
  const float* bias;
  const float* add; int64_t ld_add;
  int add_mod;
  float* out; int64_t ldo;
  int M, N, K, act_in, act_out;
  int rows_per_wave;
};
struct KvPackParams {
  const void* qkv; const void* ctxkv; void* kall; void* vtall;
  int B, H, T, S, Tkp;
};
struct AttentionParams {
  const void* q; int64_t ldq;
  const void* kall; const void* vtall;
  void* out; int64_t ldo;
  int B, H, T, Tk, Tkp;
  float scale;
  int causal;
  const float* key_valid;
  int kv_ld, kv_n;
  int out_x3;
};
struct SmallAttnParams {
  const void* qkv; int64_t ldq;
  const float* part; int nsplit; const float* bias;
  void* out; int64_t ldo;
  int out_frag, MA;
  int B, H, T;
  float scale;
  int causal;
  const float* key_valid; int kv_ld, kv_n;
};
struct SamplerParams {
  const float* x;
  const float* model_out;
  const float* noise;
  const float* init_img;
  const float* mask;
  const float* table;
  const int* step;
  int step_host;
  float guidance, clamp_lo, clamp_hi;
  int use_cfg;
  int n_lo; double gamma;
  float* x0_buf;
  float* s_buf;
  float* x_out;
  float* x0_out;
  int N, HW;
};

int launch_x3_pack(const float* in, void* out, int64_t n, float scale, hipStream_t s);
int gn_nsplit(int B, int HW);
int launch_gn_stats(const GnStatsParams& p, int dtype, hipStream_t s);
int launch_gn_coeff(const GnCoeffParams& p, int B, hipStream_t s);
inline int launch_gn_stats_coeff(const void* x0, const void* x1, int C0, int C1, int B, int HW, float eps, const float* gamma, const float* beta,
                                 const float* film, int64_t film_ld, float* partial, float* coeff, int dtype, hipStream_t s) {
  const int nsplit = gn_nsplit(B, HW), C = C0 + C1;
  GnStatsParams sp = {};
  sp.x0 = x0; sp.x1 = x1; sp.C0 = C0; sp.C1 = C1; sp.HW = HW; sp.B = B; sp.groups = 32; sp.nsplit = nsplit; sp.partial = partial;
  const int rc = launch_gn_stats(sp, dtype, s);
  if (rc) return rc;
  GnCoeffParams cp = {};
  cp.src[0].st = partial; cp.src[0].rpi = nsplit; cp.src[0].C = C;
  cp.HW = HW; cp.C = C; cp.groups = 32; cp.eps = eps; cp.gamma = gamma; cp.beta = beta; cp.film = film; cp.film_ld = film_ld; cp.coeff = coeff;
  return launch_gn_coeff(cp, B, s);
}
int launch_gn_apply(const GnApplyParams& p, int dtype, hipStream_t s);
int launch_resample(const void* x, void* y, int B, int H, int W, int C, int mode, int dtype, hipStream_t s);
int launch_conv_in(const ConvInParams& p, int dtype, hipStream_t s);
int launch_timestep_embedding(const float* t, const float* freqs, float* out, int B, int half, hipStream_t s);
int launch_linear_smallm(const LinearSmallParams& p, int wdtype, hipStream_t s);
int launch_layernorm_f32(const float* x, const float* g, const float* b, float* y, int rows, int D, float eps, hipStream_t s);
int launch_cast_rows(const float* x, void* y, int rows, int cols, int64_t ldx, int64_t ldy, int dtype, hipStream_t s);
// ... 30 lines not shown
```

### kandinsky-2_amd/csrc/elementwise.hip

```cpp
#include "kernels.h"
#include "elementwise.h"

__device__ __forceinline__ void load4(const bf16_t* p, float* f) {
  const uint2 r = *reinterpret_cast<const uint2*>(p);
  f[0] = __uint_as_float(r.x << 16); f[1] = __uint_as_float(r.x & 0xffff0000u);
  f[2] = __uint_as_float(r.y << 16); f[3] = __uint_as_float(r.y & 0xffff0000u);
}
__device__ __forceinline__ void load4(const f16_t* p, float* f) {
  const uint2 r = *reinterpret_cast<const uint2*>(p);
  unpack2_f16(r.x, f[0], f[1]); unpack2_f16(r.y, f[2], f[3]);
}
__device__ __forceinline__ void load4(const float* p, float* f) {
  const float4 r = *reinterpret_cast<const float4*>(p);
  f[0] = r.x; f[1] = r.y; f[2] = r.z; f[3] = r.w;
}

template <typename T>
__global__ __launch_bounds__(256) void gn_stats_kernel(GnStatsParams p) {
  __shared__ float red[1024 * 2 * 2];
  const int tid = threadIdx.x, b = blockIdx.y, s = blockIdx.x;
  const int C = p.C0 + p.C1, VP = C / 4;
  const int per = (p.HW + p.nsplit - 1) / p.nsplit;
  const int pix0 = s * per, pix1 = min(p.HW, pix0 + per);
  const T* x0 = reinterpret_cast<const T*>(p.x0) + (int64_t)b * p.HW * p.C0;
// ... 100 lines not shown
          const float2 v = *reinterpret_cast<const float2*>(base + ((int64_t)r * sr.C + cc) * 2);
          s += (double)v.x;
          q += (double)v.y;
        }
      }
    }
    off += sr.C;
  }
#pragma unroll
  for (int o = 32; o > 0; o >>= 1) {
    s += __shfl_xor(s, o, 64);
    q += __shfl_xor(q, o, 64);
  }
  if (lane == 0) { red[wave][0] = s; red[wave][1] = q; }
  __syncthreads();
  if (tid == 0) {
    const double st = (red[0][0] + red[1][0]) + (red[2][0] + red[3][0]);
    const double qt = (red[0][1] + red[1][1]) + (red[2][1] + red[3][1]);
    const double n = (double)p.HW * (double)cg;
    const double mean = st / n;
    double var = qt / n - mean * mean;
    if (var < 0.0) var = 0.0;
    ms[0] = (float)mean;
    ms[1] = (float)(1.0 / sqrt(var + (double)p.eps));
  }
  __syncthreads();
  const float mean_f = ms[0], rstd_f = ms[1];
  if (tid < cg) {
    const int c = g * cg + tid;
    float A = rstd_f * pg;
    float Bc = pb - mean_f * A;
    if (p.film != nullptr) {
      A *= psc;
      Bc = Bc * psc + psh;
    }
    *reinterpret_cast<float2*>(p.coeff + ((int64_t)b * p.C + c) * 2) = make_float2(A, Bc);
  }
}

template <typename T>
__global__ __launch_bounds__(256) void gn_apply_kernel(GnApplyParams p) {
  constexpr int EPV = Vec16<T>::N;
  const bool fast = p.out_x3 != 0;
  const int C = p.C0 + p.C1, CV = C / EPV;
  const int Ho = p.mode == 1 ? p.H / 2 : (p.mode == 2 ? p.H * 2 : p.H);
  const int Wo = p.mode == 1 ? p.W / 2 : (p.mode == 2 ? p.W * 2 : p.W);
  const int pad = p.pad, Hp = Ho + 2 * pad, Wp = Wo + 2 * pad;
  const int idx = blockIdx.x * 256 + threadIdx.x;
  if (idx >= Wp * CV) return;
  const int xp = idx / CV, cv = idx - xp * CV;
  const int xo = xp - pad, yo = (int)blockIdx.y - pad, b = blockIdx.z;
  T* out = reinterpret_cast<T*>(p.out) + (((int64_t)b * Hp + blockIdx.y) * Wp + xp) * C + cv * EPV;
  Vec16<T> o;
  if (xo < 0 || yo < 0 || xo >= Wo || yo >= Ho) {
#pragma unroll
    for (int k = 0; k < EPV / 2; ++k) o.set2(k, 0.f, 0.f);
  } else {
    const int c = cv * EPV;
    const T* src; int cs, ld;
    if (c < p.C0) { src = reinterpret_cast<const T*>(p.x0); cs = c; ld = p.C0; }
    else { src = reinterpret_cast<const T*>(p.x1); cs = c - p.C0; ld = p.C1; }
    float A[EPV], Bc[EPV];
    const float* cf = p.coeff + ((int64_t)b * C + c) * 2;
#pragma unroll
    for (int k = 0; k < EPV; k += 2) {
      const float4 q = *reinterpret_cast<const float4*>(cf + 2 * k);
      A[k] = q.x; Bc[k] = q.y; A[k + 1] = q.z; Bc[k + 1] = q.w;
    }
    float r[EPV];
    if (p.mode == 1) {
      Vec16<T> v[4];
#pragma unroll
      for (int dy = 0; dy < 2; ++dy)
#pragma unroll
        for (int dx = 0; dx < 2; ++dx)
          v[dy * 2 + dx].raw = *reinterpret_cast<const decltype(v[0].raw)*>(src + ((int64_t)(b * p.H + 2 * yo + dy) * p.W + 2 * xo + dx) * ld + cs);
#pragma unroll
      for (int k = 0; k < EPV; ++k) {
        float acc = 0.f;
#pragma unroll
        for (int q = 0; q < 4; ++q) acc += fast ? apply_act_sel<true>(v[q].get(k) * A[k] + Bc[k], p.act) : apply_act_sel<false>(v[q].get(k) * A[k] + Bc[k], p.act);
        r[k] = acc * 0.25f;
      }
    } else {
      const int yi = p.mode == 2 ? yo >> 1 : yo, xi = p.mode == 2 ? xo >> 1 : xo;
      Vec16<T> v;
      v.raw = *reinterpret_cast<const decltype(v.raw)*>(src + ((int64_t)(b * p.H + yi) * p.W + xi) * ld + cs);
#pragma unroll
      for (int k = 0; k < EPV; ++k) r[k] = fast ? apply_act_sel<true>(v.get(k) * A[k] + Bc[k], p.act) : apply_act_sel<false>(v.get(k) * A[k] + Bc[k], p.act);
    }
#pragma unroll
    for (int k = 0; k < EPV / 2; ++k) o.set2(k, r[2 * k], r[2 * k + 1]);
  }
  if constexpr (sizeof(T) == 4) {
    if (p.out_x3) { x3_store4(out, x3_split4(o.raw)); return; }
  }
  *reinterpret_cast<decltype(o.raw)*>(out) = o.raw;
}

template <typename T>
__global__ __launch_bounds__(256) void resample_kernel(const void* xin, void* yout, int B, int H, int W, int C, int mode) {
  constexpr int EPV = Vec16<T>::N;
  const int CV = C / EPV;
  const int Ho = mode == 1 ? H / 2 : H * 2, Wo = mode == 1 ? W / 2 : W * 2;
  const int64_t total = (int64_t)B * Ho * Wo * CV;
  const T* x = reinterpret_cast<const T*>(xin);
  T* y = reinterpret_cast<T*>(yout);
  for (int64_t i = (int64_t)blockIdx.x * 256 + threadIdx.x; i < total; i += (int64_t)gridDim.x * 256) {
    const int cv = (int)(i % CV);
    int64_t t = i / CV;
    const int xo = (int)(t % Wo); t /= Wo;
    const int yo = (int)(t % Ho);
    const int b = (int)(t / Ho);
    Vec16<T> o;
    if (mode == 1) {
      float r[EPV];
#pragma unroll
      for (int k = 0; k < EPV; ++k) r[k] = 0.f;
#pragma unroll
      for (int dy = 0; dy < 2; ++dy)
#pragma unroll
        for (int dx = 0; dx < 2; ++dx) {
          Vec16<T> v;
          v.raw = *reinterpret_cast<const decltype(v.raw)*>(x + ((int64_t)(b * H + 2 * yo + dy) * W + 2 * xo + dx) * C + cv * EPV);
#pragma unroll
          for (int k = 0; k < EPV; ++k) r[k] += v.get(k);
        }
#pragma unroll
      for (int k = 0; k < EPV / 2; ++k) o.set2(k, r[2 * k] * 0.25f, r[2 * k + 1] * 0.25f);
    } else {
      o.raw = *reinterpret_cast<const decltype(o.raw)*>(x + ((int64_t)(b * H + (yo >> 1)) * W + (xo >> 1)) * C + cv * EPV);
    }
    *reinterpret_cast<decltype(o.raw)*>(y + i * EPV) = o.raw;
  }
}

constexpr int CONV_IN_PT = 8;
template <typename T, int CIN>
__global__ __launch_bounds__(128) void conv_in_kernel(ConvInParams p) {
  constexpr int PT = CONV_IN_PT, PW = PT + 2;
  __shared__ float patch[CIN][3][PW];
  const int tid = threadIdx.x;
  const int xt = blockIdx.x, y = blockIdx.y, b = blockIdx.z;
  const int x0 = xt * PT;
  const int hw = p.H * p.W;
  for (int i = tid; i < CIN * 3 * PW; i += 128) {
    const int c = i / (3 * PW), r = (i / PW) % 3, xx = i % PW;
    const int yy = y + r - 1, xs = x0 + xx - 1;
    float v = 0.f;
    if (yy >= 0 && yy < p.H && xs >= 0 && xs < p.W) {
      const int64_t o = (int64_t)yy * p.W + xs;
      if (c < 4) v = p.x[((int64_t)b * 4 + c) * hw + o];
      else if (c < 8) v = p.img[((int64_t)b * 4 + (c - 4)) * hw + o] * (p.img_premul ? 1.f : p.mask[(int64_t)b * hw + o]);
      else v = p.mask[(int64_t)b * hw + o];
    }
    patch[c][r][xx] = v;
  }
  __syncthreads();
  T* out = reinterpret_cast<T*>(p.out);
  for (int n = tid; n < p.Cout; n += 128) {
    float w[CIN * 9];
#pragma unroll
    for (int k = 0; k < CIN * 9; ++k) w[k] = p.w[(int64_t)k * p.Cout + n];
    const float bias = p.bias[n];
    for (int px = 0; px < PT && x0 + px < p.W; ++px) {
      float acc = bias;
#pragma unroll
      for (int c = 0; c < CIN; ++c)
#pragma unroll
        for (int r = 0; r < 3; ++r)
#pragma unroll
          for (int q = 0; q < 3; ++q) acc += w[c * 9 + r * 3 + q] * patch[c][r][px + q];
      out[((int64_t)(b * p.H + y) * p.W + x0 + px) * p.Cout + n] = from_f32<T>(acc);
    }
  }
}

template <int OCB>
__global__ __launch_bounds__(256) void conv3x3_direct_kernel(ConvDirectParams p) {
  const int Ho = (p.Hin - 1) / p.stride + 1, Wo = (p.Win - 1) / p.stride + 1;
  const int pix = blockIdx.x * 256 + threadIdx.x;
  const int oc0 = blockIdx.y * OCB, b = blockIdx.z;
  if (pix >= Ho * Wo) return;
  const int yo = pix / Wo, xo = pix - yo * Wo;
  const int yi = yo * p.stride - 1, xi = xo * p.stride - 1;
  float acc[OCB];
#pragma unroll
  for (int o = 0; o < OCB; ++o) acc[o] = (oc0 + o < p.Cout) ? p.bias[oc0 + o] : 0.f;
  const int64_t plane = (int64_t)p.Hin * p.Win;
  for (int c = 0; c < p.Cin; ++c) {
    const float* xp = p.x + ((int64_t)b * p.Cin + c) * plane;
    float v[9];
#pragma unroll
    for (int r = 0; r < 3; ++r)
#pragma unroll
      for (int q = 0; q < 3; ++q) {
        const int yy = yi + r, xx = xi + q;
        v[r * 3 + q] = (yy >= 0 && yy < p.Hin && xx >= 0 && xx < p.Win) ? xp[(int64_t)yy * p.Win + xx] : 0.f;
      }
#pragma unroll
    for (int o = 0; o < OCB; ++o) {
      if (oc0 + o < p.Cout) {
        const float* wp = p.w + ((int64_t)(oc0 + o) * p.Cin + c) * 9;
#pragma unroll
        for (int k = 0; k < 9; ++k) acc[o] += wp[k] * v[k];
      }
    }
  }
#pragma unroll
  for (int o = 0; o < OCB; ++o)
    if (oc0 + o < p.Cout) p.y[(((int64_t)b * p.Cout + oc0 + o) * Ho + yo) * Wo + xo] = apply_act(acc[o], p.act);
}

__global__ void timestep_embedding_kernel(const float* t, const float* freqs, float* out, int B, int half) {
  const int i = blockIdx.x * blockDim.x + threadIdx.x;
  if (i >= B * half) return;
  const int b = i / half, k = i - b * half;
  const float a = t[b] * freqs[k];
  out[(int64_t)b * 2 * half + k] = cosf(a);
  out[(int64_t)b * 2 * half + half + k] = sinf(a);
}

template <typename TW, int MT>
__global__ __launch_bounds__(256) void linear_smallm_kernel(LinearSmallParams p) {
  constexpr int EPC = 16 / sizeof(TW);
  extern __shared__ __attribute__((aligned(16))) char smem_lin[];
  float* xs = reinterpret_cast<float*>(smem_lin);
  const int tid = threadIdx.x, lane = tid & 63, wave = tid >> 6;
  for (int i = tid; i < MT * p.K; i += 256) {
    const int m = i / p.K, k = i - m * p.K;
    float xv = m < p.M ? p.x[(int64_t)m * p.ldx + k] : 0.f;
    if (p.act_in == K22_ACT_SILU) xv = silu_f(xv);
    xs[i] = xv;
  }
  __syncthreads();
  const int per_wave = p.rows_per_wave;
  const int n_begin = (blockIdx.x * 4 + wave) * per_wave;
  for (int r = 0; r < per_wave; ++r) {
    const int n = n_begin + r;
    if (n >= p.N) return;
    const TW* w = reinterpret_cast<const TW*>(p.W) + (int64_t)n * p.K;
    float acc[MT];
#pragma unroll
    for (int m = 0; m < MT; ++m) acc[m] = 0.f;
    for (int k = lane * EPC; k < p.K; k += 64 * EPC) {
      Vec16<TW> wv;
      wv.raw = *reinterpret_cast<const decltype(wv.raw)*>(w + k);
#pragma unroll
      for (int m = 0; m < MT; ++m) {
        const float* xr = xs + m * p.K + k;
#pragma unroll
        for (int e = 0; e < EPC; e += 4) {
          const float4 xv = *reinterpret_cast<const float4*>(xr + e);
          acc[m] += xv.x * wv.get(e) + xv.y * wv.get(e + 1) + xv.z * wv.get(e + 2) + xv.w * wv.get(e + 3);
        }
      }
    }
// ... 22 lines not shown
  const float mean = (red[0] + red[1] + red[2] + red[3]) / D;
  float q = 0.f;
  for (int i = tid; i < D; i += 256) { const float d = xr[i] - mean; q += d * d; }
  q = wave_sum(q);
  if ((tid & 63) == 0) red[4 + (tid >> 6)] = q;
  __syncthreads();
  const float rstd = rsqrtf((red[4] + red[5] + red[6] + red[7]) / D + eps);
  for (int i = tid; i < D; i += 256) y[(int64_t)row * D + i] = (xr[i] - mean) * rstd * g[i] + bta[i];
}

template <typename T>
__global__ void cast_rows_kernel(const float* x, void* yout, int rows, int cols, int64_t ldx, int64_t ldy) {
  T* y = reinterpret_cast<T*>(yout);
  const int64_t total = (int64_t)rows * cols;
  for (int64_t i = (int64_t)blockIdx.x * blockDim.x + threadIdx.x; i < total; i += (int64_t)gridDim.x * blockDim.x) {
    const int r = (int)(i / cols), c = (int)(i - (int64_t)r * cols);
    y[r * ldy + c] = from_f32<T>(x[r * ldx + c]);
  }
}

template <typename T>
__global__ __launch_bounds__(256) void kv_pack_kernel(KvPackParams p) {
  __shared__ T vt[64][66];
  const int tid = threadIdx.x, jt = blockIdx.x, h = blockIdx.y, b = blockIdx.z;
  const int C = p.H * 64, Tk = p.S + p.T;
  const T* qkv = reinterpret_cast<const T*>(p.qkv);
  const T* ckv = reinterpret_cast<const T*>(p.ctxkv);
  T* Kall = reinterpret_cast<T*>(p.kall) + ((int64_t)(b * p.H + h) * p.Tkp) * 64;
  T* VTall = reinterpret_cast<T*>(p.vtall) + ((int64_t)(b * p.H + h) * 64) * p.Tkp;
  for (int i = tid; i < 64 * 64; i += 256) {
    const int jj = i >> 6, d = i & 63;
    const int j = jt * 64 + jj;
    T kv = from_f32<T>(0.f), vv = from_f32<T>(0.f);
    if (j < p.S) {
      const T* r = ckv + (int64_t)(b * p.S + j) * 2 * C + h * 64 + d;
      kv = r[0]; vv = r[C];
    } else if (j < Tk) {
      const T* r = qkv + (int64_t)(b * p.T + (j - p.S)) * 3 * C + C + h * 64 + d;
      kv = r[0]; vv = r[C];
    }
    Kall[(int64_t)j * 64 + d] = kv;
    vt[d][jj] = vv;
  }
  __syncthreads();
  for (int i = tid; i < 64 * 64; i += 256) {
    const int d = i >> 6, jj = i & 63;
    VTall[(int64_t)d * p.Tkp + jt * 64 + jj] = vt[d][jj];
  }
}

__global__ __launch_bounds__(256) void x3_pack_kernel(const float4* __restrict__ in, u32x4_t* __restrict__ out, int64_t n4, float scale) {
  for (int64_t i = (int64_t)blockIdx.x * 256 + threadIdx.x; i < n4; i += (int64_t)gridDim.x * 256) {
    const float4 v = in[i];
    x3_store4(out + i, x3_split4(v.x * scale, v.y * scale, v.z * scale, v.w * scale));
  }
}
int launch_x3_pack(const float* in, void* out, int64_t n, float scale, hipStream_t s) {
  if (n % 8 || (uintptr_t)in % 16 || (uintptr_t)out % 32) return k22_set_error(K22_EINVAL, "x3_pack: n % 8 == 0, 16-byte aligned input, 32-byte aligned output (groups of eight)");
  const int64_t n4 = n / 4;
  int nb = (int)((n4 + 255) / 256);
  if (nb > 4096) nb = 4096;
  if (nb < 1) return K22_OK;
  hipLaunchKernelGGL(x3_pack_kernel, dim3(nb), dim3(256), 0, s, reinterpret_cast<const float4*>(in), reinterpret_cast<u32x4_t*>(out), n4, scale);
  K22_CHECK_LAUNCH();
  return K22_OK;
}

static inline int grid_for(int64_t total, int threads, int cap) {
  int64_t nb = (total + threads - 1) / threads;
  if (nb > cap) nb = cap;
  if (nb < 1) nb = 1;
  return (int)nb;
}

int gn_nsplit(int B, int HW) {
  int ns = 512 / (B > 0 ? B : 1);
  if (ns > 128) ns = 128;
  while (ns > 1 && HW / ns < 32) ns >>= 1;
  return ns < 1 ? 1 : ns;
}

int launch_gn_stats(const GnStatsParams& p, int dtype, hipStream_t s) {
  const int C = p.C0 + p.C1;
  if (p.groups != 32 || C % 128 != 0 || p.C0 % 4 != 0) return k22_set_error(K22_EINVAL, "gn_stats: need 32 groups, C % 128 == 0");
  if (C / 4 > 768) return k22_set_error(K22_EINVAL, "gn_stats: C too large (max 3072)");
  if (C / 4 < 256 && (256 / (C / 4)) * C > 2048) return k22_set_error(K22_EINVAL, "gn_stats: internal LDS bound");
  dim3 grid(p.nsplit, p.B);
  if (dtype == K22_BF16) hipLaunchKernelGGL(gn_stats_kernel<bf16_t>, grid, dim3(256), 0, s, p);
  else if (dtype == K22_F16) hipLaunchKernelGGL(gn_stats_kernel<f16_t>, grid, dim3(256), 0, s, p);
  else hipLaunchKernelGGL(gn_stats_kernel<float>, grid, dim3(256), 0, s, p);
  K22_CHECK_LAUNCH();
  return K22_OK;
}
int launch_gn_coeff(const GnCoeffParams& p, int B, hipStream_t s) {
  if (p.C / p.groups > 256) return k22_set_error(K22_EINVAL, "gn_coeff: more than 256 channels per group");
  hipLaunchKernelGGL(gn_coeff_kernel, dim3(p.groups, B), dim3(256), 0, s, p);
  K22_CHECK_LAUNCH();
  return K22_OK;
}
int launch_gn_apply(const GnApplyParams& p, int dtype, hipStream_t s) {
  const int C = p.C0 + p.C1;
  const int epv = dtype == K22_F32 ? 4 : 8;
  if (C % epv || p.C0 % epv) return k22_set_error(K22_EINVAL, "gn_apply: channel alignment");
  if (p.out_x3 && dtype != K22_F32) return k22_set_error(K22_EINVAL, "gn_apply: x3-chunk output is an option of the fp32 launch");
  const int Ho = p.mode == 1 ? p.H / 2 : (p.mode == 2 ? p.H * 2 : p.H);
  const int Wo = p.mode == 1 ? p.W / 2 : (p.mode == 2 ? p.W * 2 : p.W);
  const int Hp = Ho + 2 * p.pad, Wp = Wo + 2 * p.pad;
  if (Hp > 65535 || p.B > 65535) return k22_set_error(K22_EINVAL, "gn_apply: tensor too large");
  dim3 grid((Wp * (C / epv) + 255) / 256, Hp, p.B);
  if (dtype == K22_BF16) hipLaunchKernelGGL(gn_apply_kernel<bf16_t>, grid, dim3(256), 0, s, p);
  else if (dtype == K22_F16) hipLaunchKernelGGL(gn_apply_kernel<f16_t>, grid, dim3(256), 0, s, p);
  else hipLaunchKernelGGL(gn_apply_kernel<float>, grid, dim3(256), 0, s, p);
  K22_CHECK_LAUNCH();
  return K22_OK;
}
int launch_resample(const void* x, void* y, int B, int H, int W, int C, int mode, int dtype, hipStream_t s) {
  const int epv = dtype == K22_F32 ? 4 : 8;
  const int Ho = mode == 1 ? H / 2 : H * 2, Wo = mode == 1 ? W / 2 : W * 2;
  const int nb = grid_for((int64_t)B * Ho * Wo * (C / epv), 256, 8192);
  if (dtype == K22_BF16) hipLaunchKernelGGL(resample_kernel<bf16_t>, dim3(nb), dim3(256), 0, s, x, y, B, H, W, C, mode);
  else if (dtype == K22_F16) hipLaunchKernelGGL(resample_kernel<f16_t>, dim3(nb), dim3(256), 0, s, x, y, B, H, W, C, mode);
  else hipLaunchKernelGGL(resample_kernel<float>, dim3(nb), dim3(256), 0, s, x, y, B, H, W, C, mode);
  K22_CHECK_LAUNCH();
  return K22_OK;
}
int launch_conv_in(const ConvInParams& p, int dtype, hipStream_t s) {
  dim3 grid((p.W + CONV_IN_PT - 1) / CONV_IN_PT, p.H, p.B);
  if (p.Cin == 4) {
    if (dtype == K22_BF16) hipLaunchKernelGGL((conv_in_kernel<bf16_t, 4>), grid, dim3(128), 0, s, p);
    else if (dtype == K22_F16) hipLaunchKernelGGL((conv_in_kernel<f16_t, 4>), grid, dim3(128), 0, s, p);
    else hipLaunchKernelGGL((conv_in_kernel<float, 4>), grid, dim3(128), 0, s, p);
  } else if (p.Cin == 9) {
    if (dtype == K22_BF16) hipLaunchKernelGGL((conv_in_kernel<bf16_t, 9>), grid, dim3(128), 0, s, p);
    else if (dtype == K22_F16) hipLaunchKernelGGL((conv_in_kernel<f16_t, 9>), grid, dim3(128), 0, s, p);
    else hipLaunchKernelGGL((conv_in_kernel<float, 9>), grid, dim3(128), 0, s, p);
  } else if (p.Cin == 8) {
    if (dtype == K22_BF16) hipLaunchKernelGGL((conv_in_kernel<bf16_t, 8>), grid, dim3(128), 0, s, p);
    else if (dtype == K22_F16) hipLaunchKernelGGL((conv_in_kernel<f16_t, 8>), grid, dim3(128), 0, s, p);
    else hipLaunchKernelGGL((conv_in_kernel<float, 8>), grid, dim3(128), 0, s, p);
  } else {
    return k22_set_error(K22_EINVAL, "conv_in: in_channels must be 4, 8 or 9");
  }
  K22_CHECK_LAUNCH();
  return K22_OK;
}
int launch_conv3x3_direct(const ConvDirectParams& p, hipStream_t s) {
  if (p.stride != 1 && p.stride != 2) return k22_set_error(K22_EINVAL, "conv3x3_direct: stride must be 1 or 2");
  const int Ho = (p.Hin - 1) / p.stride + 1, Wo = (p.Win - 1) / p.stride + 1;
  constexpr int OCB = 8;
  dim3 grid((Ho * Wo + 255) / 256, (p.Cout + OCB - 1) / OCB, p.B);
  hipLaunchKernelGGL((conv3x3_direct_kernel<OCB>), grid, dim3(256), 0, s, p);
  K22_CHECK_LAUNCH();
  return K22_OK;
}
int launch_timestep_embedding(const float* t, const float* freqs, float* out, int B, int half, hipStream_t s) {
  hipLaunchKernelGGL(timestep_embedding_kernel, dim3((B * half + 255) / 256), dim3(256), 0, s, t, freqs, out, B, half);
  K22_CHECK_LAUNCH();
  return K22_OK;
}
template <typename TW>
static void launch_linear_m(const LinearSmallParams& p, int Mt, dim3 grid, size_t smem, hipStream_t s) {
  switch (Mt) {
    case 1: hipLaunchKernelGGL((linear_smallm_kernel<TW, 1>), grid, dim3(256), smem, s, p); break;
    case 2: hipLaunchKernelGGL((linear_smallm_kernel<TW, 2>), grid, dim3(256), smem, s, p); break;
    case 4: hipLaunchKernelGGL((linear_smallm_kernel<TW, 4>), grid, dim3(256), smem, s, p); break;
    default: hipLaunchKernelGGL((linear_smallm_kernel<TW, 8>), grid, dim3(256), smem, s, p); break;
  }
}
int launch_linear_smallm(const LinearSmallParams& p0, int wdtype, hipStream_t s) {
  if (p0.M > 8 || p0.M < 1) return k22_set_error(K22_EINVAL, "linear_smallm: M must be in 1..8");
  const int epc = wdtype == K22_F32 ? 4 : 8;
  if (p0.K % epc) return k22_set_error(K22_EINVAL, "linear_smallm: K alignment");
  const int Mt = p0.M <= 2 ? p0.M : (p0.M <= 4 ? 4 : 8);
  const size_t smem = (size_t)Mt * p0.K * 4;
  if (smem > 64 * 1024) return k22_set_error(K22_EINVAL, "linear_smallm: M*K too large for the LDS stage");
  LinearSmallParams p = p0;
  int rpw = 1;
  while (rpw < 8 && (p.N + 8 * rpw - 1) / (8 * rpw) >= 1024) rpw *= 2;
  p.rows_per_wave = rpw;
  dim3 grid((p.N + 4 * rpw - 1) / (4 * rpw));
  if (wdtype == K22_BF16) launch_linear_m<bf16_t>(p, Mt, grid, smem, s);
  else if (wdtype == K22_F16) launch_linear_m<f16_t>(p, Mt, grid, smem, s);
  else launch_linear_m<float>(p, Mt, grid, smem, s);
  K22_CHECK_LAUNCH();
  return K22_OK;
}
int launch_layernorm_f32(const float* x, const float* g, const float* b, float* y, int rows, int D, float eps, hipStream_t s) {
  hipLaunchKernelGGL(layernorm_f32_kernel, dim3(rows), dim3(256), 0, s, x, g, b, y, D, eps);
  K22_CHECK_LAUNCH();
  return K22_OK;
}
int launch_cast_rows(const float* x, void* y, int rows, int cols, int64_t ldx, int64_t ldy, int dtype, hipStream_t s) {
  const int nb = grid_for((int64_t)rows * cols, 256, 4096);
  if (dtype == K22_BF16) hipLaunchKernelGGL(cast_rows_kernel<bf16_t>, dim3(nb), dim3(256), 0, s, x, y, rows, cols, ldx, ldy);
  else if (dtype == K22_F16) hipLaunchKernelGGL(cast_rows_kernel<f16_t>, dim3(nb), dim3(256), 0, s, x, y, rows, cols, ldx, ldy);
  else hipLaunchKernelGGL(cast_rows_kernel<float>, dim3(nb), dim3(256), 0, s, x, y, rows, cols, ldx, ldy);
  K22_CHECK_LAUNCH();
  return K22_OK;
}
int launch_kv_pack(const KvPackParams& p, int dtype, hipStream_t s) {
  if (p.Tkp % 64) return k22_set_error(K22_EINVAL, "kv_pack: Tkp % 64");
  dim3 grid(p.Tkp / 64, p.H, p.B);
  if (dtype == K22_BF16) hipLaunchKernelGGL(kv_pack_kernel<bf16_t>, grid, dim3(256), 0, s, p);
  else if (dtype == K22_F16) hipLaunchKernelGGL(kv_pack_kernel<f16_t>, grid, dim3(256), 0, s, p);
  else hipLaunchKernelGGL(kv_pack_kernel<float>, grid, dim3(256), 0, s, p);
  K22_CHECK_LAUNCH();
  return K22_OK;
}
```

### kandinsky-2_amd/csrc/engine.hip

```cpp
#include "kernels.h"
#include "elementwise.h"
#include "../../include/k22.h"
#include "tuning.h"
#include "plan.h"

#include <atomic>
#include <deque>
#include <functional>
#include <map>
#include <memory>
#include <string>
#include <tuple>
#include <unordered_map>
#include <vector>
#include <stdio.h>
#include <stdlib.h>
#include <string.h>

int launch_step_advance(int* step, int delta, hipStream_t s);

static std::atomic<long> g_loop_captures{0}, g_loop_launches{0};
long loop_capture_count() { return g_loop_captures.load(); }
long loop_launch_count() { return g_loop_launches.load(); }
static void loop_count_capture() { g_loop_captures.fetch_add(1); }
static void loop_count_launch() { g_loop_launches.fetch_add(1); }
enum : unsigned long long { K22_LOOP_KIND_P = 0, K22_LOOP_KIND_DDIM = 1, K22_LOOP_KIND_PLMS = 2 };
static unsigned long long loop_key_ptr(const void* p) { return (unsigned long long)(uintptr_t)p; }
static unsigned long long loop_key_bits(double v) { unsigned long long b; memcpy(&b, &v, 8); return b; }

namespace {

enum OpKind { OP_CONV3 = 0, OP_GEMM = 1, OP_GN = 2, OP_ATTN = 3, OP_MISC = 4, OP_NKINDS = 5 };

struct Op {
  std::function<int(hipStream_t)> fn;
  int kind = OP_MISC;
  double flops = 0.0;
  double flops2 = 0.0;
  double bytes = 0.0;
  int kernels = 1;
  Op() {}
  template <typename F> Op(F f, int k = OP_MISC, double fl = 0.0, double by = 0.0, int nk = 1) : fn(f), kind(k), flops(fl), bytes(by), kernels(nk) {}
  int operator()(hipStream_t st) const { return fn(st); }
};
typedef std::vector<Op> OpList;

struct Act {
  Slot* s0 = nullptr; int C0 = 0;
  Slot* s1 = nullptr; int C1 = 0;
  int H = 0, W = 0;
  const Tuned* p0 = nullptr; Slot* st0 = nullptr;
  const Tuned* p1 = nullptr; Slot* st1 = nullptr;
  int C() const { return C0 + C1; }
};

}

struct K22UNet : GraphPlan {
  K22UNetConfig cfg;
  int sdt;

  int B = 0, H = 0, W = 0;
  OpList ops;
  OpList cond_ops;
  OpList hint_ops;
  bool hint_set = false;
  int fuse_skip = 1;
  int fuse_gn = 0;
  struct GnLink { const Tuned* consumer = nullptr; };
  std::deque<GnLink> gn_links;
  int stream_frag = 1;
  struct FragJob { const void* W; Slot* slot; int Npad, taps, Kc; };
  std::vector<FragJob> frag_jobs;
  bool frag_done = false;
  int repack_frags(hipStream_t st) {
    for (auto& j : frag_jobs) {
      int rc = launch_stream_repack(j.W, ptr(j.slot), j.Npad, j.taps, j.Kc, dtype, st);
      if (rc) return rc;
    }
    frag_done = true;
    return K22_OK;
  }
  bool cond_set = false;
  GraphCache loop;
  std::vector<unsigned long long> loop_key;

  Slot *s_xin, *s_img, *s_mask, *s_t, *s_out;
  Slot *s_temb, *s_e1, *s_emb, *s_film, *s_xfproj, *s_ctx;
  Slot *s_full, *s_pool, *s_imgemb, *s_tmpf, *s_tmpf2, *s_fullT;
  Slot *s_part, *s_coeff, *s_P1, *s_U1, *s_P2, *s_S, *s_N, *s_QKV, *s_KALL, *s_VT, *s_ATT, *s_splitk, *s_flush;
  Slot *s_U1st;
  Slot *s_ctxf = nullptr, *s_hint = nullptr, *s_hintin = nullptr, *s_hbuf[2] = {nullptr, nullptr};
  Slot* s_h[3];
  Slot* s_hst[3];
  std::vector<Slot*> s_ctxkv;
  int n_attn = 0;
  int64_t film_total = 0;
  float* film_all = nullptr;
  size_t film_all_bytes = 0;
  int hoist_time = 1;
  const float* film_cur = nullptr;
  const float* film_base() const { return film_cur ? film_cur : ptr<float>(s_film); }
  struct TimeW { const float* freqs; const float* w0; const float* b0; const float* w2; const float* b2; const void* we; const float* be; int mc, ted, dt; } tw = {};
  int time_rows(const float* t, float* temb, float* e1, float* emb, float* film, int rows, hipStream_t st) {
    int rc = launch_timestep_embedding(t, tw.freqs, temb, rows, tw.mc / 2, st);
    if (rc) return rc;
    LinearSmallParams lp = {};
    lp.x = temb; lp.ldx = tw.mc; lp.W = tw.w0; lp.bias = tw.b0; lp.out = e1; lp.ldo = tw.ted;
    lp.M = rows; lp.N = tw.ted; lp.K = tw.mc; lp.act_in = K22_ACT_NONE; lp.act_out = K22_ACT_SILU;
    rc = launch_linear_smallm(lp, K22_F32, st);
    if (rc) return rc;
    lp.x = e1; lp.ldx = tw.ted; lp.W = tw.w2; lp.bias = tw.b2; lp.add = ptr<float>(s_xfproj); lp.ld_add = tw.ted; lp.add_mod = B;
    lp.out = emb; lp.K = tw.ted; lp.act_out = K22_ACT_NONE;
    rc = launch_linear_smallm(lp, K22_F32, st);
    if (rc) return rc;
    LinearSmallParams le = {};
    le.x = emb; le.ldx = tw.ted; le.W = tw.we; le.bias = tw.be; le.out = film; le.ldo = film_total;
    le.M = rows; le.N = (int)film_total; le.K = tw.ted; le.act_in = K22_ACT_SILU; le.act_out = K22_ACT_NONE;
    return launch_linear_smallm(le, tw.dt, st);
  }

  float* model_out() { return ptr<float>(s_out); }
  int exec(hipStream_t st) { return run_ops(st); }
  int exec_eager(hipStream_t st) { return run_eager(st, [this](hipStream_t s) { return exec(s); }); }
  int prepare_run(hipStream_t st) {
    if (!frag_done) { int rc = repack_frags(st); if (rc) return rc; }
    return tune_once(s_flush, st);
  }

  ~K22UNet() {
    if (film_all) (void)hipFree(film_all);
  }

  struct LoopRows {
    bool hoist = false;
    float *film = nullptr, *temb = nullptr, *e1 = nullptr, *emb = nullptr;
  };
  int loop_begin(int n_calls, hipStream_t st, LoopRows* lr) {
    if (int rc = prepare_run(st)) return rc;
    lr->hoist = B <= 8 && hoist_time;
    if (!lr->hoist) return K22_OK;
    const int64_t rows_all = (int64_t)n_calls * B;
    const size_t need = (size_t)rows_all * (size_t)(film_total + tw.mc + 2 * tw.ted) * sizeof(float);
    if (need > film_all_bytes) {
      loop.drop();
      if (film_all) { (void)hipStreamSynchronize(st); (void)hipFree(film_all); film_all = nullptr; film_all_bytes = 0; }
      const hipError_t e = hipMalloc(reinterpret_cast<void**>(&film_all), need);
      if (e != hipSuccess) { film_all = nullptr; return k22_set_error_hip(e, __FILE__, __LINE__); }
      film_all_bytes = need;
    }
    lr->film = film_all;
    lr->temb = lr->film + rows_all * film_total;
    lr->e1 = lr->temb + rows_all * tw.mc;
    lr->emb = lr->e1 + rows_all * tw.ted;
    return K22_OK;
  }
  int loop_prologue(const LoopRows& lr, const float* timesteps, int n_calls, const float* inpaint_image, const float* inpaint_mask, hipStream_t s) {
    if (lr.hoist) {
      const int spl = 8 / B;
      for (int k0 = 0; k0 < n_calls; k0 += spl) {
        const int rows = (n_calls - k0 < spl ? n_calls - k0 : spl) * B;
        const int64_t r0 = (int64_t)k0 * B;
        const int rc = time_rows(timesteps + r0, lr.temb + r0 * tw.mc, lr.e1 + r0 * tw.ted, lr.emb + r0 * tw.ted, lr.film + r0 * film_total, rows, s);
        if (rc) return rc;
      }
    }
    if (cfg.in_channels == 9) {
      const size_t pb = (size_t)B, hw = (size_t)H * W;
      if (int rc = copy_d2d(ptr(s_img), inpaint_image, pb * 4 * hw * 4, s)) return rc;
      if (int rc = copy_d2d(ptr(s_mask), inpaint_mask, pb * hw * 4, s)) return rc;
    }
    return K22_OK;
  }
  int loop_model(const LoopRows& lr, const float* cur, const float* timesteps, int call, hipStream_t s) {
    const size_t half = (size_t)(B / 2) * 4 * H * W * sizeof(float);
    if (int rc = copy_d2d(ptr(s_xin), cur, half, s)) return rc;
    if (int rc = copy_d2d(ptr(s_xin) + half, cur, half, s)) return rc;
    if (lr.hoist) {
      film_cur = lr.film + (int64_t)call * B * film_total;
    } else {
      if (int rc = copy_d2d(ptr(s_t), timesteps + (size_t)call * B, (size_t)B * 4, s)) return rc;
    }
    return exec(s);
  }
  template <typename F> int loop_run(const std::vector<unsigned long long>& key, const float* timesteps, const float* inpaint_image,
                                     const float* inpaint_mask, int use_graph, hipStream_t st, F body) {
    auto run_loop = [&](hipStream_t s) -> int { const int rc = body(s); film_cur = nullptr; return rc; };
    if (!use_graph) {
      const int rc = run_loop(st);
      if (rc == K22_OK) loop_count_launch();
      return rc;
    }
    if (!loop || key != loop_key) {
      if (!warmed) {
        const size_t pb = (size_t)B, hw = (size_t)H * W;
        hipError_t e = hipMemsetAsync(ptr(s_xin), 0, pb * 4 * hw * 4, st);
        if (e != hipSuccess) return k22_set_error_hip(e, __FILE__, __LINE__);
        if (int rc = copy_d2d(ptr(s_t), timesteps, pb * 4, st)) return rc;
        if (cfg.in_channels == 9) {
          if (int rc = copy_d2d(ptr(s_img), inpaint_image, pb * 4 * hw * 4, st)) return rc;
          if (int rc = copy_d2d(ptr(s_mask), inpaint_mask, pb * hw * 4, st)) return rc;
        }
        if (int rc = exec_eager(st)) return rc;
        e = hipStreamSynchronize(st);
        if (e != hipSuccess) return k22_set_error_hip(e, __FILE__, __LINE__);
      }
      if (int rc = loop.capture(cap, run_loop)) return rc;
      loop_key = key;
      loop_count_capture();
    }
    const int rc = loop.launch(st);
    if (rc == K22_OK) loop_count_launch();
    return rc;
  }

  int run_ops_range(hipStream_t st, size_t lo, size_t hi) {
    for (size_t i = lo; i < hi && i < ops.size(); ++i) { int rc = ops[i](st); if (rc) return rc; }
    return K22_OK;
  }
  int run_ops(hipStream_t st) { return run_ops_range(st, 0, ops.size()); }

  void op_gn(OpList& L, const Act& in, const std::string& pfx, int64_t film_off,
             int act, int mode, int pad, Slot* dst, const GnLink* link = nullptr) {
    const int Bn = B, C = in.C(), HW = in.H * in.W;
    const int nsplit = gn_nsplit(Bn, HW);
    const bool fused = in.st0 != nullptr && (in.s1 == nullptr || in.st1 != nullptr);
    if (!fused) need(s_part, (size_t)Bn * nsplit * C * 2 * sizeof(float));
    need(s_coeff, (size_t)Bn * C * 2 * sizeof(float));
    const int Ho = mode == 1 ? in.H / 2 : (mode == 2 ? in.H * 2 : in.H);
    const int Wo = mode == 1 ? in.W / 2 : (mode == 2 ? in.W * 2 : in.W);
    need(dst, (size_t)Bn * (Ho + 2 * pad) * (Wo + 2 * pad) * C * esz);
    const float* gamma = Wf(pfx + ".weight");
    const float* beta = Wf(pfx + ".bias");
    const Act a = in;
    const int dt = sdt;
    const int x3 = k22_is_split(dtype) ? 1 : 0;
    const double gn_bytes = (double)Bn * HW * C * esz * (fused ? 1.0 : 2.0) + (double)Bn * (Ho + 2 * pad) * (Wo + 2 * pad) * C * esz;
    L.push_back(Op([=](hipStream_t st) {
      const void* x0 = ptr(a.s0);
      const void* x1 = a.s1 ? ptr(a.s1) : nullptr;
      GnCoeffParams cp = {};
      if (fused) {
        cp.src[0].st = ptr<float>(a.st0); cp.src[0].rpi = a.p0->rpi; cp.src[0].C = a.C0;
        if (a.s1) { cp.src[1].st = ptr<float>(a.st1); cp.src[1].rpi = a.p1->rpi; cp.src[1].C = a.C1; }
        if (cp.src[0].rpi <= 0 || (a.s1 && cp.src[1].rpi <= 0)) return k22_set_error(K22_EINVAL, "unet: producer delivered no GroupNorm partial sums");
      } else {
        GnStatsParams sp;
        sp.x0 = x0; sp.x1 = x1; sp.C0 = a.C0; sp.C1 = a.C1;
        sp.HW = HW; sp.B = Bn; sp.groups = 32; sp.nsplit = nsplit; sp.partial = ptr<float>(s_part);
        int rc = launch_gn_stats(sp, dt, st);
        if (rc) return rc;
        cp.src[0].st = ptr<float>(s_part); cp.src[0].rpi = nsplit; cp.src[0].C = C;
      }
      cp.HW = HW; cp.C = C; cp.groups = 32; cp.eps = 1e-5f;
      cp.gamma = gamma; cp.beta = beta;
      cp.film = film_off >= 0 ? film_base() + film_off : nullptr; cp.film_ld = film_total;
      cp.coeff = ptr<float>(s_coeff);
      GnApplyParams ap = {};
      ap.x0 = x0; ap.x1 = x1; ap.C0 = a.C0; ap.C1 = a.C1; ap.B = Bn; ap.H = a.H; ap.W = a.W;
      ap.mode = mode; ap.pad = pad; ap.act = act; ap.coeff = ptr<float>(s_coeff); ap.out = ptr(dst); ap.out_x3 = x3;
      int rc = launch_gn_coeff(cp, Bn, st);
      if (rc) return rc;
      if (link != nullptr && link->consumer != nullptr && conv3_algo_fuses_gn(link->consumer->cfg.algo)) return K22_OK;
      return launch_gn_apply(ap, dt, st);
    }, OP_GN, 0.0, gn_bytes, fused ? 2 : 3));
  }

  static void apply_cfg(IgemmParams& q, const Cfg& c) { tuned_apply_cfg(q, c); }
  int op_dt(const Tuned& t) const { return t.dt >= 0 ? t.dt : dtype; }
  void make_candidates(Tuned& t) { tuned_make_candidates(t, op_dt(t)); }
  void default_cfg(Tuned& t) { tuned_default_cfg(t, op_dt(t)); }
  void finish_cfg(Tuned& t) { tuned_finish_cfg(t, op_dt(t)); }
  size_t max_splitk_bytes(const Tuned& t) const { return tuned_max_splitk_bytes(t, autotune != 0); }
  int max_rpi(const Tuned& t) const { return tuned_max_rpi(t, op_dt(t), autotune != 0); }

  int x2_plan = 0;
  enum ConvRole { CONV_IN = 0, CONV_OUT = 1, CONV_HEAD = 2 };
  int conv_dt(int role, int Hc) const {
    if (dtype != K22_F16X2) return dtype;
    if (role == CONV_HEAD) return K22_F16X3;
    if (Hc >= H) return (x2_plan >> role) & 1 ? K22_F16X2 : K22_F16X3;
    return K22_F16X2;
  }
  int gemm_dt(bool qkv) const { return dtype == K22_F16X2 ? (qkv ? K22_F16X2 : K22_F16X3) : dtype; }

  Tuned* op_conv(OpList& L, int role, Slot* src, int Hc, int Wc, int Cin, int Cout,
                 const std::string& pfx, const Act* residual, Slot* dst, int out_mode, Slot* stats = nullptr,
                 const Act* skip_in = nullptr, const std::string& skip_pfx = std::string(), const Act* gn_in = nullptr, int gn_act = K22_ACT_NONE) {
    tuned.emplace_back();
    Tuned* t = &tuned.back();
    t->dt = conv_dt(role, Hc);
    IgemmParams& p = t->p;
    p.stages = -1;
    p.M = B * Hc * Wc; p.N = Cout; p.Npad = (Cout + 63) / 64 * 64; p.Kc = Cin; p.K0 = Cin; p.taps = 9;
    p.H = Hc; p.W = Wc; p.ldo = Cout; p.ldr = Cout; p.out_mode = out_mode; p.act = K22_ACT_NONE;
    p.Wp = W_(pfx + ".weight"); p.bias = Wf(pfx + ".bias");
    Act sk;
    if (skip_in) {
      sk = *skip_in;
      p.S0 = reinterpret_cast<const void*>(1); p.S1 = sk.s1 ? reinterpret_cast<const void*>(1) : nullptr;
      p.SK0 = sk.C0; p.SK1 = sk.C1;
      p.Ws = W_(skip_pfx + ".weight"); p.bias2 = Wf(skip_pfx + ".bias");
    }
    t->want_stats = stats != nullptr;
    Slot *wf = nullptr, *wsf = nullptr;
    if (stream_frag && k22_esz(dtype) == 2 && p.M <= 1152 && (stream_supported(p, dtype, 5) || stream_supported(p, dtype, 9))) {
      wf = new_slot();
      need(wf, stream_frag_bytes(p.Npad, 9, Cin, dtype));
      frag_jobs.push_back({p.Wp, wf, p.Npad, 9, Cin});
      p.Wfrag = reinterpret_cast<const void*>(1);
      if (skip_in) {
        wsf = new_slot();
        need(wsf, stream_frag_bytes(p.Npad, 1, p.SK0 + p.SK1, dtype));
        frag_jobs.push_back({p.Ws, wsf, p.Npad, 1, p.SK0 + p.SK1});
        p.Wsfrag = reinterpret_cast<const void*>(1);
      }
    }
    make_candidates(*t);
    default_cfg(*t);
    if (wf && t->cfg.algo != 20 && (t->from_table || !autotune)) {
      wf->bytes = 0; wf = nullptr;
      if (wsf) { wsf->bytes = 0; wsf = nullptr; frag_jobs.pop_back(); }
      frag_jobs.pop_back();
      p.Wfrag = nullptr; p.Wsfrag = nullptr;
      make_candidates(*t);
      default_cfg(*t);
    }
    need(s_splitk, max_splitk_bytes(*t));
    if (t->want_stats) need(stats, (size_t)B * max_rpi(*t) * Cout * 2 * sizeof(float));
    need(dst, out_mode == IG_OUT_ROWMAJOR ? (size_t)p.M * Cout * esz : (size_t)p.M * Cout * sizeof(float));
    Slot* rs = residual ? residual->s0 : nullptr;
    const int dt = t->dt;
    const bool gnf = gn_in != nullptr && fuse_gn;
    Act ga;
    if (gnf) ga = *gn_in;
    t->run = [=](hipStream_t st) {
      IgemmParams q = t->p;
      apply_cfg(q, t->cfg);
      q.A0 = ptr(src); q.residual = rs ? ptr(rs) : nullptr; q.out = ptr(dst); q.partial = ptr<float>(s_splitk);
      if (gnf && conv3_algo_fuses_gn(t->cfg.algo)) {
        q.gn_coeff = ptr<float>(s_coeff); q.gn_x0 = ptr(ga.s0); q.gn_x1 = ga.s1 ? ptr(ga.s1) : nullptr; q.gn_C0 = ga.C0; q.gn_act = gn_act;
      }
      q.stats = t->want_stats ? ptr<float>(stats) : nullptr;
      if (q.S0) { q.S0 = ptr(sk.s0); q.S1 = sk.s1 ? ptr(sk.s1) : nullptr; }
      q.Wfrag = wf ? ptr(wf) : nullptr; q.Wsfrag = wsf ? ptr(wsf) : nullptr;
      return launch_igemm(q, dt, st);
    };
    const double fl = 2.0 * p.M * (double)p.N * 9.0 * p.Kc;
    L.push_back(Op([=](hipStream_t st) { return t->run(st); }, OP_CONV3, fl, 0.0, 1));
    if (skip_in) L.back().flops2 = 2.0 * p.M * (double)p.N * (p.SK0 + p.SK1);
    return t;
  }

  Tuned* op_gemm(OpList& L, const Act& in, int M, int N, const std::string& pfx,
                 const Act* residual, Slot* dst, int ldo = 0, int out_mode = IG_OUT_ROWMAJOR, Slot* stats = nullptr, bool a_raw = false) {
    tuned.emplace_back();
    Tuned* t = &tuned.back();
    t->dt = gemm_dt(out_mode == IG_OUT_QKV);
    IgemmParams& p = t->p;
    p.stages = -1;
    p.M = M; p.N = N; p.Npad = (N + 63) / 64 * 64; p.Kc = in.C(); p.K0 = in.C0; p.taps = 1;
    p.lda0 = in.C0; p.lda1 = in.C1; p.ldo = ldo ? ldo : N; p.ldr = N; p.out_mode = out_mode;
    p.act = K22_ACT_NONE;
    if (in.H > 0 && in.W > 0 && M % (in.H * in.W) == 0 && M / (in.H * in.W) == B) { p.H = in.H; p.W = in.W; }
    if (out_mode == IG_OUT_QKV) p.att_T = in.H * in.W;
    p.Wp = W_(pfx + ".weight"); p.bias = Wf(pfx + ".bias");
    p.a_raw = (a_raw && k22_is_split(dtype)) ? 1 : 0;
    t->want_stats = stats != nullptr && p.H > 0;
    make_candidates(*t);
    if (t->want_stats && t->cands.empty()) { t->want_stats = false; make_candidates(*t); }
    default_cfg(*t);
    need(s_splitk, max_splitk_bytes(*t));
    if (t->want_stats) need(stats, (size_t)B * max_rpi(*t) * N * 2 * sizeof(float));
    need(dst, (size_t)M * p.ldo * esz);
    const Act a = in;
    Slot* rs = residual ? residual->s0 : nullptr;
    const int dt = t->dt;
    t->run = [=](hipStream_t st) {
      IgemmParams q = t->p;
      apply_cfg(q, t->cfg);
      q.A0 = ptr(a.s0); q.A1 = a.s1 ? ptr(a.s1) : nullptr;
      q.residual = rs ? ptr(rs) : nullptr; q.out = ptr(dst); q.partial = ptr<float>(s_splitk);
      if (t->aux0) { q.kall = ptr(reinterpret_cast<Slot*>(t->aux0)); q.vtall = ptr(reinterpret_cast<Slot*>(t->aux1)); }
      q.stats = t->want_stats ? ptr<float>(stats) : nullptr;
      return launch_igemm(q, dt, st);
    };
    L.push_back(Op([=](hipStream_t st) { return t->run(st); }, OP_GEMM, 2.0 * p.M * (double)p.N * p.Kc, 0.0, 1));
    return t;
  }

  Act resblock(const std::string& pfx, const Act& in, int Cout, int updown, int64_t& film_cursor, Slot* dst, Slot* dst_stats) {
    const int Cin = in.C();
    const int Ho = updown == 1 ? in.H / 2 : (updown == 2 ? in.H * 2 : in.H);
    const int Wo = updown == 1 ? in.W / 2 : (updown == 2 ? in.W * 2 : in.W);
    GnLink* l1 = nullptr;
    if (fuse_gn && updown == 0) { gn_links.emplace_back(); l1 = &gn_links.back(); }
    op_gn(ops, in, pfx + ".in_layers.0", -1, K22_ACT_SILU, updown, 1, s_P1, l1);
    Tuned* t1 = op_conv(ops, CONV_IN, s_P1, Ho, Wo, Cin, Cout, pfx + ".in_layers.2", nullptr, s_U1, IG_OUT_ROWMAJOR, s_U1st, nullptr, std::string(),
                        l1 ? &in : nullptr, K22_ACT_SILU);
    if (l1) l1->consumer = t1;
    Act u1; u1.s0 = s_U1; u1.C0 = Cout; u1.H = Ho; u1.W = Wo;
    if (t1->want_stats) { u1.p0 = t1; u1.st0 = s_U1st; }
    const int64_t film_off = film_cursor;
    film_cursor += 2 * Cout;
    GnLink* l2 = nullptr;
    if (fuse_gn) { gn_links.emplace_back(); l2 = &gn_links.back(); }
    op_gn(ops, u1, pfx + ".out_layers.0", film_off, K22_ACT_SILU, 0, 1, s_P2, l2);
    Act skip;
    skip.H = Ho; skip.W = Wo; skip.C0 = Cout;
    if (updown) {
      if (Cin != Cout || in.s1) { if (err.empty()) err = "updown ResBlock with channel change is not supported"; }
      need(s_S, (size_t)B * Ho * Wo * Cin * esz);
      const Act a = in; const int Bn = B, dt = sdt;
      ops.push_back([=](hipStream_t st) { return launch_resample(ptr(a.s0), ptr(s_S), Bn, a.H, a.W, Cin, updown, dt, st); });
      skip.s0 = s_S;
    } else if (Cin != Cout) {
      IgemmParams probe = {};
      probe.M = B * Ho * Wo; probe.N = Cout; probe.Npad = (Cout + 63) / 64 * 64; probe.Kc = Cout; probe.K0 = Cout; probe.taps = 9;
      probe.H = Ho; probe.W = Wo; probe.ldo = Cout; probe.ldr = Cout; probe.out_mode = IG_OUT_ROWMAJOR;
      probe.S0 = reinterpret_cast<const void*>(1); probe.S1 = in.s1 ? reinterpret_cast<const void*>(1) : nullptr;
      probe.SK0 = in.C0; probe.SK1 = in.C1; probe.Ws = reinterpret_cast<const void*>(1);
      if (fuse_skip && Cout >= 128 && (conv3_halo_supported(probe, dtype, 256) || conv3_halo_supported(probe, dtype, 128))) {
        Tuned* t2 = op_conv(ops, CONV_OUT, s_P2, Ho, Wo, Cout, Cout, pfx + ".out_layers.3", nullptr, dst, IG_OUT_ROWMAJOR, dst_stats,
                            &in, pfx + ".skip_connection", l2 ? &u1 : nullptr, K22_ACT_SILU);
        if (l2) l2->consumer = t2;
        Act out; out.s0 = dst; out.C0 = Cout; out.H = Ho; out.W = Wo;
        if (t2->want_stats) { out.p0 = t2; out.st0 = dst_stats; }
        return out;
      }
      op_gemm(ops, in, B * Ho * Wo, Cout, pfx + ".skip_connection", nullptr, s_S, 0, IG_OUT_ROWMAJOR, nullptr, true);
      skip.s0 = s_S;
    } else {
      if (in.s1) { if (err.empty()) err = "identity skip over a concat input"; }
      skip.s0 = in.s0;
    }
    Tuned* t2 = op_conv(ops, CONV_OUT, s_P2, Ho, Wo, Cout, Cout, pfx + ".out_layers.3", &skip, dst, IG_OUT_ROWMAJOR, dst_stats, nullptr, std::string(),
                        l2 ? &u1 : nullptr, K22_ACT_SILU);
    if (l2) l2->consumer = t2;
    Act out; out.s0 = dst; out.C0 = Cout; out.H = Ho; out.W = Wo;
    if (t2->want_stats) { out.p0 = t2; out.st0 = dst_stats; }
    return out;
  }

  Act attnblock(const std::string& pfx, const Act& in, Slot* dst, Slot* dst_stats = nullptr) {
    const int C = in.C0, T = in.H * in.W, Hh = C / 64, S = cfg.ctx_len;
    const int Tk = S + T, Tkp = (Tk + 63) / 64 * 64;
    n_attn++;
    op_gn(ops, in, pfx + ".norm", -1, K22_ACT_NONE, 0, 0, s_N);
    Act n; n.s0 = s_N; n.C0 = C; n.H = in.H; n.W = in.W;
    Slot* kall = new_slot((size_t)B * Hh * Tkp * 64 * esz);
    Slot* vtall = new_slot((size_t)B * Hh * Tkp * 64 * esz);
    Slot* ckv = new_slot((size_t)B * S * 2 * C * esz);
    s_ctxkv.push_back(ckv);
    const int Bn = B, dt = dtype, sd = sdt;
    {
      Act c; c.s0 = s_ctx; c.C0 = cfg.ctx_dim; c.H = 1; c.W = S;
      op_gemm(cond_ops, c, B * S, 2 * C, pfx + ".encoder_kv", nullptr, ckv, 0, IG_OUT_ROWMAJOR, nullptr, true);
      cond_ops.push_back(Op([=](hipStream_t st) {
        KvPackParams kp;
        kp.qkv = nullptr; kp.ctxkv = ptr(ckv); kp.kall = ptr(kall); kp.vtall = ptr(vtall);
        kp.B = Bn; kp.H = Hh; kp.T = 0; kp.S = S; kp.Tkp = Tkp;
        return launch_kv_pack(kp, sd, st);
      }));
    }
    need(s_QKV, (size_t)B * T * C * esz);
    {
      Tuned* t = op_gemm(ops, n, B * T, 3 * C, pfx + ".qkv", nullptr, s_QKV, C, IG_OUT_QKV);
      t->p.att_T = T; t->p.att_S = S; t->p.att_Tkp = Tkp;
      t->aux0 = kall; t->aux1 = vtall;
    }
    need(s_ATT, (size_t)B * T * C * esz);
    ops.push_back(Op([=](hipStream_t st) {
      AttentionParams ap = {};
      ap.q = ptr(s_QKV); ap.ldq = C; ap.kall = ptr(kall); ap.vtall = ptr(vtall); ap.out = ptr(s_ATT); ap.ldo = C;
      ap.B = Bn; ap.H = Hh; ap.T = T; ap.Tk = Tk; ap.Tkp = Tkp; ap.scale = 0.125f;
      ap.out_x3 = k22_is_split(dt) ? 1 : 0;
      return launch_attention(ap, dt, st);
    }, OP_ATTN, 4.0 * Bn * Hh * (double)T * Tk * 64.0, 0.0, 1));
    Act a; a.s0 = s_ATT; a.C0 = C; a.H = in.H; a.W = in.W;
    Tuned* tp = op_gemm(ops, a, B * T, C, pfx + ".proj_out", &in, dst, 0, IG_OUT_ROWMAJOR, dst_stats);
    Act out; out.s0 = dst; out.C0 = C; out.H = in.H; out.W = in.W;
    if (tp->want_stats) { out.p0 = tp; out.st0 = dst_stats; }
    return out;
  }

  bool has_attn(int ds) const {
    for (int i = 0; i < cfg.n_attention_ds; ++i) if (cfg.attention_ds[i] == ds) return true;
    return false;
  }

  int plan(int nB, int nH, int nW) {
    const int n_down = cfg.n_levels - 1;
    if (nB < 1 || nH < 1 || nW < 1) return k22_set_error(K22_EINVAL, "unet: B, H, W must be positive");
    if (nH % (1 << n_down) || nW % (1 << n_down)) return k22_set_error(K22_EINVAL, "unet: H, W must be divisible by 2^(levels-1)");
    if (nB > 8) return k22_set_error(K22_EINVAL, "unet: batch (2*bs) must be <= 8 per engine call");
    begin_plan();
    B = nB; H = nH; W = nW;
    gn_links.clear();
    ops.clear(); cond_ops.clear(); hint_ops.clear(); s_ctxkv.clear(); frag_jobs.clear(); frag_done = false; n_attn = 0;
    cond_set = false; hint_set = false;
    loop.drop();
    const int mc = cfg.model_channels, ted = 4 * mc;

    film_total = 0;
    {
      int ch = mc * cfg.channel_mult[0];
      for (int l = 0; l < cfg.n_levels; ++l) {
        for (int i = 0; i < cfg.num_res_blocks; ++i) { ch = mc * cfg.channel_mult[l]; film_total += 2 * ch; }
        if (l != cfg.n_levels - 1) film_total += 2 * ch;
      }
      film_total += 2 * 2 * ch;
      for (int l = cfg.n_levels - 1; l >= 0; --l)
        for (int i = 0; i <= cfg.num_res_blocks; ++i) {
          ch = mc * cfg.channel_mult[l];
          film_total += 2 * ch;
          if (l && i == cfg.num_res_blocks) film_total += 2 * ch;
        }
    }

    s_xin = new_slot((size_t)B * 4 * H * W * 4); s_img = new_slot((size_t)B * 4 * H * W * 4);
    s_mask = new_slot((size_t)B * H * W * 4); s_t = new_slot((size_t)B * 4 + 64);
    s_out = new_slot((size_t)B * cfg.out_channels * H * W * 4);
    s_temb = new_slot((size_t)B * mc * 4); s_e1 = new_slot((size_t)B * ted * 4); s_emb = new_slot((size_t)B * ted * 4);
    s_film = new_slot((size_t)B * film_total * 4); s_xfproj = new_slot((size_t)B * ted * 4);
    s_ctx = new_slot((size_t)B * cfg.ctx_len * cfg.ctx_dim * esz);
    const int ntext_p = cfg.ctx_len - cfg.n_image_embs;
    s_full = new_slot((size_t)B * (ntext_p > 0 ? ntext_p : 1) * cfg.text_dim1 * 4); s_pool = new_slot((size_t)B * cfg.text_dim2 * 4);
    s_imgemb = new_slot((size_t)B * cfg.image_dim * 4);
    s_tmpf = new_slot((size_t)B * cfg.n_image_embs * cfg.ctx_dim * 4 + (size_t)B * ted * 4);
    s_tmpf2 = new_slot((size_t)B * ted * 4);
    s_fullT = new_slot((size_t)B * (ntext_p > 0 ? ntext_p : 1) * cfg.text_dim1 * esz);
    s_ctxf = new_slot(cfg.head_type == 1 ? (size_t)B * cfg.ctx_len * cfg.ctx_dim * 4 : 0);
    if (cfg.hint_channels) {
      s_hint = new_slot((size_t)B * 4 * H * W * 4);
      s_hintin = new_slot((size_t)B * cfg.hint_channels * 64 * H * W * 4);
      for (int i = 0; i < 2; ++i) s_hbuf[i] = new_slot((size_t)B * 16 * 64 * H * W * 4);
    }
    s_part = new_slot(); s_coeff = new_slot(); s_P1 = new_slot(); s_U1 = new_slot(); s_P2 = new_slot(); s_S = new_slot();
    s_N = new_slot(); s_QKV = new_slot(); s_KALL = new_slot(); s_VT = new_slot(); s_ATT = new_slot();
    s_splitk = new_slot(256);
    s_U1st = new_slot();
    s_flush = new_slot(autotune ? ((size_t)320 << 20) : 0);
    for (int i = 0; i < 3; ++i) { s_h[i] = new_slot(); s_hst[i] = new_slot(); }
    int hrot = 0, hcur = 0;
    auto next_h = [&]() { hcur = hrot; hrot = (hrot + 1) % 3; return s_h[hcur]; };
    auto cur_hst = [&]() { return s_hst[hcur]; };

    if (cfg.head_type == 1) build_cond_ops_22(); else build_cond_ops();
    if (cfg.hint_channels) build_hint_ops();

    {
      tw.freqs = Wf("time_freqs");
      tw.w0 = Wf("time_embed.0.weight"); tw.b0 = Wf("time_embed.0.bias");
      tw.w2 = Wf("time_embed.2.weight"); tw.b2 = Wf("time_embed.2.bias");
      tw.we = W_("emb_layers.weight"); tw.be = Wf("emb_layers.bias");
      tw.mc = mc; tw.ted = ted; tw.dt = sdt;
      const int Bn = B;
      ops.push_back([=](hipStream_t st) {
        if (film_cur) return (int)K22_OK;
        return time_rows(ptr<float>(s_t), ptr<float>(s_temb), ptr<float>(s_e1), ptr<float>(s_emb), ptr<float>(s_film), Bn, st);
      });
    }

    int64_t film_cursor = 0;
    std::vector<Act> hs;
    int ch = mc * cfg.channel_mult[0];
    {
      Slot* d = new_slot((size_t)B * H * W * ch * esz);
      ConvInParams cp = {};
      cp.w = Wf("input_blocks.0.0.weight"); cp.bias = Wf("input_blocks.0.0.bias");
      cp.B = B; cp.H = H; cp.W = W; cp.Cin = cfg.in_channels; cp.Cout = ch;
      const int dt = sdt; const bool inpaint = cfg.in_channels == 9, hinted = cfg.in_channels == 8;
      const int premul = (hinted || cfg.head_type == 1) ? 1 : 0;
      ops.push_back([=](hipStream_t st) {
        ConvInParams q = cp;
        q.x = ptr<float>(s_xin); q.img = inpaint ? ptr<float>(s_img) : (hinted ? ptr<float>(s_hint) : nullptr);
        q.mask = inpaint ? ptr<float>(s_mask) : nullptr; q.img_premul = premul;
        q.out = ptr(d);
        return launch_conv_in(q, dt, st);
      });
      Act a; a.s0 = d; a.C0 = ch; a.H = H; a.W = W;
      hs.push_back(a);
    }
    Act h = hs.back();
    int ds = 1, blk = 1;
    for (int l = 0; l < cfg.n_levels; ++l) {
      for (int i = 0; i < cfg.num_res_blocks; ++i) {
        const int co = mc * cfg.channel_mult[l];
        const std::string pfx = "input_blocks." + std::to_string(blk);
        Slot* d = new_slot();
        if (has_attn(ds)) {
          Slot* rd = next_h();
          Act r = resblock(pfx + ".0", h, co, 0, film_cursor, rd, cur_hst());
          h = attnblock(pfx + ".1", r, d, new_slot());
        } else {
          h = resblock(pfx + ".0", h, co, 0, film_cursor, d, new_slot());
        }
        ch = co; hs.push_back(h); ++blk;
      }
      if (l != cfg.n_levels - 1) {
        const std::string pfx = "input_blocks." + std::to_string(blk);
        Slot* d = new_slot();
        h = resblock(pfx + ".0", h, ch, 1, film_cursor, d, new_slot());
        hs.push_back(h); ++blk; ds *= 2;
      }
    }
    {
      Slot* d0 = next_h(); Slot* st0 = cur_hst();
      Act r = resblock("middle_block.0", h, ch, 0, film_cursor, d0, st0);
      Slot* da = next_h(); Slot* sta = cur_hst();
      Act a = attnblock("middle_block.1", r, da, sta);
      Slot* d2 = next_h(); Slot* st2 = cur_hst();
      h = resblock("middle_block.2", a, ch, 0, film_cursor, d2, st2);
    }
    blk = 0;
    for (int l = cfg.n_levels - 1; l >= 0; --l) {
      for (int i = 0; i <= cfg.num_res_blocks; ++i) {
        const Act skip = hs.back(); hs.pop_back();
        Act cat; cat.s0 = h.s0; cat.C0 = h.C0; cat.s1 = skip.s0; cat.C1 = skip.C0; cat.H = h.H; cat.W = h.W;
        cat.p0 = h.p0; cat.st0 = h.st0; cat.p1 = skip.p0; cat.st1 = skip.st0;
        if (skip.H != h.H || skip.W != h.W) return k22_set_error(K22_EINVAL, "unet: skip shape mismatch");
        const int co = mc * cfg.channel_mult[l];
        const std::string pfx = "output_blocks." + std::to_string(blk);
        { Slot* d = next_h(); Slot* dst_st = cur_hst(); h = resblock(pfx + ".0", cat, co, 0, film_cursor, d, dst_st); }
        int sub = 1;
        if (has_attn(ds)) { Slot* da = next_h(); Slot* sta = cur_hst(); h = attnblock(pfx + "." + std::to_string(sub), h, da, sta); ++sub; }
        if (l && i == cfg.num_res_blocks) {
          { Slot* d = next_h(); Slot* dst_st = cur_hst(); h = resblock(pfx + "." + std::to_string(sub), h, co, 2, film_cursor, d, dst_st); }
          ds /= 2;
        }
        ch = co; ++blk;
      }
    }
    if (film_cursor != film_total) return k22_set_error(K22_EINVAL, "unet: internal FiLM width mismatch");
    op_gn(ops, h, "out.0", -1, K22_ACT_SILU, 0, 1, s_P1);
    op_conv(ops, CONV_HEAD, s_P1, H, W, ch, cfg.out_channels, "out.2", nullptr, s_out, IG_OUT_NCHW_F32);

    return finish_plan();
  }

  void build_cond_ops_22() {
    const int mc = cfg.model_channels, ted = 4 * mc, Bn = B, dt = sdt;
    const int cd = cfg.ctx_dim, S = cfg.ctx_len, di = cfg.image_dim;
    const float* w_cp = Wf("head22.ctx_proj.weight"); const float* b_cp = Wf("head22.ctx_proj.bias");
    const float* g_cn = Wf("head22.ctx_norm.weight"); const float* b_cn = Wf("head22.ctx_norm.bias");
    const float* w_ep = Wf("head22.emb_proj.weight"); const float* b_ep = Wf("head22.emb_proj.bias");
    const float* g_en = Wf("head22.emb_norm.weight"); const float* b_en = Wf("head22.emb_norm.bias");
    cond_ops.push_back([=](hipStream_t st) {
      float* proj = ptr<float>(s_tmpf);
      float* embp = ptr<float>(s_tmpf) + (size_t)Bn * S * cd;
      LinearSmallParams lp = {};
      lp.x = ptr<float>(s_imgemb); lp.ldx = di; lp.W = w_cp; lp.bias = b_cp; lp.out = proj; lp.ldo = S * cd;
      lp.M = Bn; lp.N = S * cd; lp.K = di;
      int rc = launch_linear_smallm(lp, K22_F32, st);
      if (rc) return rc;
      rc = launch_layernorm_f32(proj, g_cn, b_cn, ptr<float>(s_ctxf), Bn * S, cd, 1e-5f, st);
      if (rc) return rc;
      rc = launch_cast_rows(ptr<float>(s_ctxf), ptr(s_ctx), Bn * S, cd, cd, cd, dt, st);
      if (rc) return rc;
// ... 16 lines not shown
      Slot* dst = k == 7 ? s_hint : s_hbuf[k & 1];
      hint_ops.push_back([=](hipStream_t st) {
        ConvDirectParams q = {};
        q.x = ptr<float>(src); q.w = w; q.bias = b; q.y = ptr<float>(dst);
        q.B = Bn; q.Cin = ci; q.Cout = cout; q.Hin = hi; q.Win = wi; q.stride = stride; q.act = k == 7 ? K22_ACT_NONE : K22_ACT_SILU;
        return launch_conv3x3_direct(q, st);
      });
      cin = cout;
      if (stride == 2) { hin = (hin - 1) / 2 + 1; win = (win - 1) / 2 + 1; }
    }
  }

  void build_cond_ops() {
    const int mc = cfg.model_channels, ted = 4 * mc, Bn = B, dt = sdt;
    const int nie = cfg.n_image_embs, cd = cfg.ctx_dim, S = cfg.ctx_len, ntext = S - nie;
    const float* w_cs = Wf("clip_to_seq.weight"); const float* b_cs = Wf("clip_to_seq.bias");
    const float* w_pn = Wf("proj_n.weight"); const float* b_pn = Wf("proj_n.bias");
    const float* g_ln = Wf("ln_model_n.weight"); const float* b_ln = Wf("ln_model_n.bias");
    const float* w_il = Wf("img_layer.weight"); const float* b_il = Wf("img_layer.bias");
    const int d1 = cfg.text_dim1, d2 = cfg.text_dim2, di = cfg.image_dim;
    cond_ops.push_back([=](hipStream_t st) {
      float* clipseq = ptr<float>(s_tmpf);
      float* proj = ptr<float>(s_tmpf) + (size_t)Bn * nie * cd;
      LinearSmallParams lp = {};
      lp.x = ptr<float>(s_imgemb); lp.ldx = di; lp.W = w_cs; lp.bias = b_cs; lp.out = clipseq; lp.ldo = nie * cd;
      lp.M = Bn; lp.N = nie * cd; lp.K = di;
      int rc = launch_linear_smallm(lp, K22_F32, st);
      if (rc) return rc;
      for (int b = 0; b < Bn; ++b) {
        rc = launch_cast_rows(clipseq + (size_t)b * nie * cd, ptr(s_ctx) + (size_t)b * S * cd * esz, nie, cd, cd, cd, dt, st);
        if (rc) return rc;
      }
      lp.x = ptr<float>(s_pool); lp.ldx = d2; lp.W = w_pn; lp.bias = b_pn; lp.out = proj; lp.ldo = ted; lp.N = ted; lp.K = d2;
      rc = launch_linear_smallm(lp, K22_F32, st);
      if (rc) return rc;
      rc = launch_layernorm_f32(proj, g_ln, b_ln, ptr<float>(s_tmpf2), Bn, ted, 1e-5f, st);
      if (rc) return rc;
      lp.x = ptr<float>(s_imgemb); lp.ldx = di; lp.W = w_il; lp.bias = b_il; lp.add = ptr<float>(s_tmpf2); lp.ld_add = ted;
      lp.out = ptr<float>(s_xfproj); lp.ldo = ted; lp.N = ted; lp.K = di;
      rc = launch_linear_smallm(lp, K22_F32, st);
      if (rc) return rc;
      return launch_cast_rows(ptr<float>(s_full), ptr(s_fullT), Bn * ntext, d1, d1, d1, dt, st);
    });
    {
      IgemmParams p = {};
    p.stages = -1;
      p.M = ntext; p.N = cd; p.Npad = (cd + 63) / 64 * 64; p.Kc = d1; p.K0 = d1; p.taps = 1; p.lda0 = d1; p.ldo = cd;
      p.out_mode = IG_OUT_ROWMAJOR; p.splitk = 1;
      p.a_raw = k22_is_split(dtype) ? 1 : 0;
      p.Wp = W_("to_model_dim_n.weight"); p.bias = Wf("to_model_dim_n.bias");
      const size_t es = esz;
      const int gdt = gemm_dt(false);
      cond_ops.push_back([=](hipStream_t st) {
        for (int b = 0; b < Bn; ++b) {
          IgemmParams q = p;
          q.A0 = ptr(s_fullT) + (size_t)b * ntext * d1 * es;
          q.out = ptr(s_ctx) + ((size_t)b * S + nie) * cd * es;
          int rc = launch_igemm(q, gdt, st);
          if (rc) return rc;
        }
        return K22_OK;
      });
    }
  }
};

extern "C" {

int k22_unet_create(const K22UNetConfig* cfg, const K22Weight* weights, int n_weights, K22UNet** out) {
  if (!cfg || !out) return k22_set_error(K22_EINVAL, "unet_create: null argument");
  if (!k22_dtype_ok(cfg->dtype) && !k22_is_split(cfg->dtype)) return k22_set_error(K22_EINVAL, "unet_create: dtype");
  if (cfg->num_head_channels != 64) return k22_set_error(K22_EINVAL, "unet_create: only num_head_channels == 64");
  if (cfg->model_channels % 128) return k22_set_error(K22_EINVAL, "unet_create: model_channels % 128");
  if (cfg->n_levels < 1 || cfg->n_levels > 8) return k22_set_error(K22_EINVAL, "unet_create: n_levels");
  if (cfg->in_channels != 4 && cfg->in_channels != 9 && cfg->in_channels != 8) return k22_set_error(K22_EINVAL, "unet_create: in_channels must be 4, 8 or 9");
  if (cfg->head_type != 0 && cfg->head_type != 1) return k22_set_error(K22_EINVAL, "unet_create: head_type must be 0 (2.1) or 1 (2.2)");
  if ((cfg->hint_channels != 0) != (cfg->in_channels == 8) || (cfg->hint_channels != 0 && cfg->hint_channels != 3))
    return k22_set_error(K22_EINVAL, "unet_create: hint_channels = 3 goes with in_channels = 8 (latent + hint latent), else 0");
  if (cfg->head_type == 1 && cfg->n_image_embs != cfg->ctx_len) return k22_set_error(K22_EINVAL, "unet_create: the 2.2 head has image tokens only (n_image_embs == ctx_len)");
  K22UNet* u = new K22UNet();
  u->cfg = *cfg; u->set_dtype(cfg->dtype); u->sdt = k22_storage_dtype(cfg->dtype);
  u->stream_frag = env_flag("K22_STREAM", 1);
  u->fuse_gn = env_flag("K22_FUSE_GN", 0);
  u->fuse_skip = env_flag("K22_FUSE_SKIP", 1);
  u->hoist_time = env_flag("K22_HOIST_TIME", 1);
  const char* xp = getenv("K22_X2_PLAN");
  u->x2_plan = xp ? (atoi(xp) & 3) : 0;
  u->set_weights(weights, n_weights);
  *out = u;
  return K22_OK;
}

void k22_unet_destroy(K22UNet* u) { delete u; }

int k22_unet_plan(K22UNet* u, int B, int H, int W, size_t* workspace_bytes) {
  if (!u || !workspace_bytes) return k22_set_error(K22_EINVAL, "unet_plan: null argument");
  int rc = u->plan(B, H, W);
  if (rc) return rc;
  *workspace_bytes = u->ws_bytes;
  return K22_OK;
}

int k22_unet_bind(K22UNet* u, void* workspace, size_t workspace_bytes) {
  if (!u) return k22_set_error(K22_EINVAL, "unet_bind: null argument");
  if (int rc = u->bind(workspace, workspace_bytes, "unet_bind")) return rc;
  u->cond_set = false; u->hint_set = false; u->frag_done = false;
  u->loop.drop();
  return K22_OK;
}

int k22_unet_set_condition(K22UNet* u, const float* full_emb, const float* pooled_emb, const float* image_emb, void* stream) {
  if (!u || !u->ws) return k22_set_error(K22_EINVAL, "unet_set_condition: bind a workspace first");
  hipStream_t st = reinterpret_cast<hipStream_t>(stream);
  const K22UNetConfig& c = u->cfg;
  const int ntext = c.ctx_len - c.n_image_embs;
  if (!image_emb) return k22_set_error(K22_EINVAL, "unet_set_condition: image_emb is required");
  if (c.head_type == 0 && (!full_emb || !pooled_emb)) return k22_set_error(K22_EINVAL, "unet_set_condition: the 2.1 head needs full_emb and pooled_emb");
  const size_t pb = (size_t)u->B;
  if (c.head_type == 0) {
    if (int rc = copy_d2d(u->ptr(u->s_full), full_emb, pb * ntext * c.text_dim1 * 4, st)) return rc;
    if (int rc = copy_d2d(u->ptr(u->s_pool), pooled_emb, pb * c.text_dim2 * 4, st)) return rc;
  }
  if (int rc = copy_d2d(u->ptr(u->s_imgemb), image_emb, pb * c.image_dim * 4, st)) return rc;
  for (auto& op : u->cond_ops) { int rc = op(st); if (rc) return rc; }
  u->cond_set = true;
  return K22_OK;
}

int k22_unet_set_hint(K22UNet* u, const float* hint, void* stream) {
  if (!u || !u->ws) return k22_set_error(K22_EINVAL, "unet_set_hint: bind a workspace first");
  if (!u->cfg.hint_channels) return k22_set_error(K22_EINVAL, "unet_set_hint: this UNet has no hint input (hint_channels == 0)");
  if (!hint) return k22_set_error(K22_EINVAL, "unet_set_hint: null hint");
  hipStream_t st = reinterpret_cast<hipStream_t>(stream);
  const size_t per = (size_t)u->B * u->cfg.hint_channels * 64 * u->H * u->W;
  if (int rc = copy_d2d(u->ptr(u->s_hintin), hint, per * 4, st)) return rc;
  for (auto& op : u->hint_ops) { int rc = op(st); if (rc) return rc; }
  u->hint_set = true;
  return K22_OK;
}

int k22_unet_forward(K22UNet* u, const float* x, const float* timesteps, const float* inpaint_image,
                     const float* inpaint_mask, float* out, int use_graph, void* stream) {
  if (!u || !u->ws) return k22_set_error(K22_EINVAL, "unet_forward: bind a workspace first");
  if (!u->cond_set) return k22_set_error(K22_EINVAL, "unet_forward: call k22_unet_set_condition first");
  if (u->cfg.in_channels == 9 && (!inpaint_image || !inpaint_mask)) return k22_set_error(K22_EINVAL, "unet_forward: inpainting UNet needs inpaint_image and inpaint_mask");
  if (u->cfg.hint_channels && !u->hint_set) return k22_set_error(K22_EINVAL, "unet_forward: call k22_unet_set_hint first");
  hipStream_t st = reinterpret_cast<hipStream_t>(stream);
  const size_t hw = (size_t)u->H * u->W;
  const size_t pb = (size_t)u->B;
  if (int rc = copy_d2d(u->ptr(u->s_xin), x, pb * 4 * hw * 4, st)) return rc;
  if (int rc = copy_d2d(u->ptr(u->s_t), timesteps, pb * 4, st)) return rc;
  if (u->cfg.in_channels == 9) {
    if (int rc = copy_d2d(u->ptr(u->s_img), inpaint_image, pb * 4 * hw * 4, st)) return rc;
    if (int rc = copy_d2d(u->ptr(u->s_mask), inpaint_mask, pb * hw * 4, st)) return rc;
  }
  { int rc = u->prepare_run(st); if (rc) return rc; }
  const int rc = use_graph ? u->replay(u->graph, st, [u](hipStream_t s) { return u->exec(s); }) : u->exec_eager(st);
  if (rc) return rc;
  return copy_d2d(out, u->ptr(u->s_out), pb * u->cfg.out_channels * hw * 4, st);
}

int k22_unet_sample_loop(K22UNet* u, float* x, float* x_tmp, const float* timesteps, const float* noise_seq, const float* init_img,
                         const float* mask, const float* inpaint_image, const float* inpaint_mask, const float* table,
                         const int* table_rows, int n_steps, float guidance, float clamp_lo, float clamp_hi, int pct_index,
                         double pct_gamma, void* scratch, int use_graph, void* stream) {
  if (!u || !u->ws) return k22_set_error(K22_EINVAL, "unet_sample_loop: bind a workspace first");
// ... 158 lines not shown
```

### kandinsky-2_amd/csrc/igemm.hip

```cpp
#include "kernels.h"
#include <stdlib.h>

template <int N> __device__ __forceinline__ void wait_vmcnt() { asm volatile("s_waitcnt vmcnt(%0)" ::"n"(N) : "memory"); }

template <typename T> __device__ __forceinline__ void store4(T* dst, const float* v);
template <> __device__ __forceinline__ void store4<bf16_t>(bf16_t* dst, const float* v) {
  uint2 w;
  w.x = pack2_bf16(v[0], v[1]);
  w.y = pack2_bf16(v[2], v[3]);
  *reinterpret_cast<uint2*>(dst) = w;
}
template <> __device__ __forceinline__ void store4<f16_t>(f16_t* dst, const float* v) {
  uint2 w;
  w.x = pack2_f16(v[0], v[1]);
  w.y = pack2_f16(v[2], v[3]);
  *reinterpret_cast<uint2*>(dst) = w;
}
template <> __device__ __forceinline__ void store4<float>(float* dst, const float* v) {
  *reinterpret_cast<float4*>(dst) = make_float4(v[0], v[1], v[2], v[3]);
}
template <> __device__ __forceinline__ void store4<x3_t>(x3_t* dst, const float* v) { store4<float>(reinterpret_cast<float*>(dst), v); }
template <> __device__ __forceinline__ void store4<x2_t>(x2_t* dst, const float* v) { store4<float>(reinterpret_cast<float*>(dst), v); }
template <typename T> __device__ __forceinline__ void load4f(const T* src, float* v);
template <> __device__ __forceinline__ void load4f<bf16_t>(const bf16_t* src, float* v) {
// ... 540 lines not shown
  int nb = (int)((total / 4 + 255) / 256);
  if (nb > 2048) nb = 2048;
  if (nb < 1) nb = 1;
  hipLaunchKernelGGL((splitk_reduce_kernel<T>), dim3(nb), dim3(256), 0, stream, q);
  K22_CHECK_LAUNCH();
  return K22_OK;
}

template <typename T, int BM, int BN, int STAGES, bool ARAW = false>
static int launch_cfg(const IgemmParams& p, int splitk, hipStream_t stream) {
  constexpr int smem0 = STAGES * (BM + BN) * 128;
  static const int dbg_pad = getenv("K22_DBG_LDS_PAD") ? atoi(getenv("K22_DBG_LDS_PAD")) : 0;
  const int smem = dbg_pad == 1 ? (smem0 + 1279) / 1280 * 1280 : (dbg_pad == 2 ? smem0 + 4096 : smem0);
  static LdsAttrGuard attr_guard;
  if (int rc_ = k22_ensure_lds_attr(attr_guard, reinterpret_cast<const void*>(&igemm_kernel<T, BM, BN, STAGES, ARAW>), smem, __FILE__, __LINE__)) return rc_;
  IgemmParams q = p;
  q.splitk = splitk;
  q.xcd_remap = g_xcd_remap;
  const int nblocks = ((p.M + BM - 1) / BM) * ((p.N + BN - 1) / BN) * splitk;
  hipLaunchKernelGGL((igemm_kernel<T, BM, BN, STAGES, ARAW>), dim3(nblocks), dim3(256), smem, stream, q);
  K22_CHECK_LAUNCH();
  if (splitk > 1) {
    if constexpr (is_x3<T>::value) return launch_reduce<float>(q, stream);
    else return launch_reduce<T>(q, stream);
  }
  return K22_OK;
}

template <typename T, int BM, int BN>
static int launch_stages(const IgemmParams& p, const IgemmPlan& pl, hipStream_t stream) {
  if constexpr (is_x3<T>::value) {
    if (p.a_raw) {
      if (pl.stages == 2) return launch_cfg<T, BM, BN, 2, true>(p, pl.splitk, stream);
      if (pl.stages == 3) return launch_cfg<T, BM, BN, 3, true>(p, pl.splitk, stream);
      return launch_cfg<T, BM, BN, 4, true>(p, pl.splitk, stream);
    }
  }
  if (pl.stages == 2) return launch_cfg<T, BM, BN, 2>(p, pl.splitk, stream);
  if (pl.stages == 3) return launch_cfg<T, BM, BN, 3>(p, pl.splitk, stream);
  return launch_cfg<T, BM, BN, 4>(p, pl.splitk, stream);
}

template <typename T>
static int launch_typed(const IgemmParams& p, const IgemmPlan& pl, hipStream_t stream) {
  if (pl.bm == 128 && pl.bn == 128) return launch_stages<T, 128, 128>(p, pl, stream);
  if (pl.bm == 128 && pl.bn == 64) return launch_stages<T, 128, 64>(p, pl, stream);
  if (pl.bm == 64 && pl.bn == 128) return launch_stages<T, 64, 128>(p, pl, stream);
  if (pl.bm == 64 && pl.bn == 64) return launch_stages<T, 64, 64>(p, pl, stream);
  return k22_set_error(K22_EINVAL, "igemm: unsupported tile configuration");
}

static int launch_reduce_dt(const IgemmParams& q, int dtype, hipStream_t stream) {
  return dtype == K22_BF16 ? launch_reduce<bf16_t>(q, stream) : (dtype == K22_F16 ? launch_reduce<f16_t>(q, stream) : launch_reduce<float>(q, stream));
}

int launch_igemm(const IgemmParams& p, int dtype, hipStream_t stream) {
  const int BK = k22_bk(dtype);
  if (p.a_raw && !k22_is_split(dtype)) return k22_set_error(K22_EINVAL, "igemm: a_raw is an option of the split-precision arithmetics only");
  if (p.M <= 0 || p.N <= 0) return K22_OK;
  if (p.taps != 1 && p.taps != 9) return k22_set_error(K22_EINVAL, "igemm: taps must be 1 or 9");
  if (p.Kc % BK != 0 || p.K0 % BK != 0) return k22_set_error(K22_EINVAL, "igemm: K per tap must be a multiple of 64 (bf16) / 32 (fp32)");
  if (p.Npad % 64 != 0 || p.Npad < p.N) return k22_set_error(K22_EINVAL, "igemm: Npad must be roundup(N,64)");
  if (p.K0 < p.Kc && p.A1 == nullptr) return k22_set_error(K22_EINVAL, "igemm: A1 missing for concat operand");
  if (p.out_mode == IG_OUT_QKV) {
    if (p.taps != 1 || p.N % 192 || (p.ldo & 3) || !p.kall || !p.vtall || p.att_T <= 0 || p.M % p.att_T || p.residual)
      return k22_set_error(K22_EINVAL, "igemm: bad qkv-projection problem (N = 3*heads*64, no residual)");
  }
  IgemmPlan pl = igemm_plan(p, dtype);
  if (p.out_mode == IG_OUT_QKV && pl.halo != 20) {
    if (p.splitk > 1) return k22_set_error(K22_EINVAL, "igemm: the qkv projection splits K only on the streaming kernel");
    pl.splitk = 1;
  }
  if (pl.halo == 20) {
    if (p.partial == nullptr) return k22_set_error(K22_EINVAL, "igemm: the streaming kernel needs the fp32 partial buffer");
    IgemmParams q = p;
    q.splitk = pl.splitk;
    q.xcd_remap = g_xcd_remap;
    int rc = launch_stream(q, dtype, pl.bm / 32, pl.splitk, stream);
    if (rc) return rc;
    return launch_reduce_dt(q, dtype, stream);
  }
  if (pl.splitk > 1 && p.partial == nullptr) pl.splitk = 1;
  if (p.res_f32 && pl.halo) return k22_set_error(K22_EINVAL, "igemm: fp32 residual is not supported by the halo kernel");
  if (p.gn_coeff != nullptr && !conv3_algo_fuses_gn(pl.halo))
    return k22_set_error(K22_EINVAL, "igemm: the fused GroupNorm-apply input needs the specialised halo kernel (algo 11 / 12)");
  if (p.S0 != nullptr && !pl.halo) return k22_set_error(K22_EINVAL, "igemm: the fused 1x1 skip connection needs the halo kernel");
  if (p.stats != nullptr && pl.splitk == 1 && !pl.halo)
    return k22_set_error(K22_EINVAL, "igemm: GroupNorm partial sums requested from a configuration that cannot produce them");
  if (pl.halo == 10) {
    IgemmParams q = p;
    q.splitk = pl.splitk;
    q.xcd_remap = g_xcd_remap;
    if (q.stages < 2 && g_stages_override >= 0) q.stages = g_stages_override;
    int rc = launch_gemm8(q, dtype, pl.bm, pl.splitk, stream);
    if (rc || pl.splitk == 1) return rc;
    return launch_reduce_dt(q, dtype, stream);
  }
  if (pl.halo) {
    IgemmParams q = p;
    q.splitk = pl.splitk;
    q.xcd_remap = g_xcd_remap;
    q.algo = pl.halo;
    if (q.stages < 2 && g_stages_override >= 0) q.stages = g_stages_override;
    int rc = launch_conv3_halo(q, dtype, pl.bm, pl.splitk, stream);
    if (rc || pl.splitk == 1) return rc;
    return launch_reduce_dt(q, dtype, stream);
  }
  if (dtype == K22_BF16) return launch_typed<bf16_t>(p, pl, stream);
  else if (dtype == K22_F16) return launch_typed<f16_t>(p, pl, stream);
  if (dtype == K22_F32) return launch_typed<float>(p, pl, stream);
  if (dtype == K22_F16X3) return launch_typed<x3_t>(p, pl, stream);
  if (dtype == K22_F16X2) return launch_typed<x2_t>(p, pl, stream);
  return k22_set_error(K22_EINVAL, "igemm: bad dtype");
}
```

### kandinsky-2_amd/csrc/kernels.h

```cpp
#pragma once
#include "common.h"

#include <atomic>

#define K22_OK 0
#define K22_EINVAL (-1)
#define K22_EHIP (-2)
#define K22_ENOMEM (-3)

struct LdsAttrGuard { std::atomic<unsigned long long> done{0}; };
inline int k22_ensure_lds_attr(LdsAttrGuard& g, const void* fn, int bytes, const char* file, int line) {
  int dev = 0;
  (void)hipGetDevice(&dev);
  const unsigned long long bit = 1ull << (dev & 63);
  if (g.done.load(std::memory_order_acquire) & bit) return K22_OK;
  const hipError_t e = hipFuncSetAttribute(fn, hipFuncAttributeMaxDynamicSharedMemorySize, bytes);
  if (e != hipSuccess) return k22_set_error_hip(e, file, line);
  g.done.fetch_or(bit, std::memory_order_release);
  return K22_OK;
}

enum IgemmOut { IG_OUT_ROWMAJOR = 0,
                IG_OUT_ROWMAJOR_F32 = 1,
                IG_OUT_NCHW_F32 = 2,
                IG_OUT_QKV = 3 };

struct IgemmParams {
  const void* A0;
  const void* A1;
  const void* Wp;
  const float* bias;
  const void* residual;
  void* out;
  float* partial;
  int M, N, Npad;
  int Kc;
  int K0;
  int taps;
  int H, W;
  long lda0, lda1;
  int ldo, ldr;
  int out_mode;
  int act;
  int splitk;
  int force_bm, force_bn;
  int stages;
  int xcd_remap;
  int algo;
  const void* S0; const void* S1; const void* Ws; const float* bias2;
  int SK0, SK1;
  void* kall; void* vtall;
  int att_T, att_S, att_Tkp;
  unsigned long long* trace;
  int res_f32;
  float* stats;
  const void* Wfrag; const void* Wsfrag;
  int a_raw;
  const float* gn_coeff; const void* gn_x0; const void* gn_x1; int gn_C0, gn_act;
  unsigned long long* st_trace;
  int st_tm, st_rb, st_mtiles, st_buf;
};

struct IgemmStatsInfo { int rows_per_image; };
int igemm_stats_rows_per_image(const IgemmParams& p, int dtype);

int launch_igemm(const IgemmParams& p, int dtype, hipStream_t stream);
bool conv3_halo_supported(const IgemmParams& p, int dtype, int bm);
inline bool conv3_algo_fuses_gn(int algo) { return algo == 11 || algo == 12; }
int conv3_halo_tiles_per_image(const IgemmParams& p, int bm);
int launch_conv3_halo(const IgemmParams& p, int dtype, int bm, int splitk, hipStream_t stream);
int launch_conv3_halo_trace(const IgemmParams& p, int dtype, hipStream_t stream);
bool gemm8_supported(const IgemmParams& p, int dtype, int bm);
bool gemm8_spec_supported(int dtype);
int gemm8_tiles_per_image(const IgemmParams& p, int bm);
int launch_gemm8(const IgemmParams& p, int dtype, int bm, int splitk, hipStream_t stream);
bool stream_supported(const IgemmParams& p, int dtype, int mb);
int stream_mtiles(const IgemmParams& p, int mb);
int launch_stream(const IgemmParams& p, int dtype, int mb, int splitk, hipStream_t stream);
long stream_launch_count();
long loop_capture_count();
long loop_launch_count();
size_t stream_frag_bytes(int Npad, int taps, int Kc, int dtype);
int launch_stream_repack(const void* W, void* out, int Npad, int taps, int Kc, int dtype, hipStream_t stream);
void igemm_set_gemm_algo(int v);
void igemm_set_conv_algo(int v);
void igemm_set_default_stages(int v);
void igemm_set_xcd_remap(int v);
void attention_set_pipe(int v);
int igemm_choose_splitk(const IgemmParams& p, int dtype);
```

Baseline: 144.4 steps/s.

## Fuse GroupNorm into QKV GEMM, resample into GN, and stem into loop

Adds a GroupNorm-apply path to the gemm8 kernels so the attention QKV projection can normalize its A operand in LDS instead of reading a separately written normalized tensor. This path is gated by K22_FUSE_QKV_GN, which defaults off. Two default-on changes also land: the GN apply kernel writes the resampled raw skip tensor during up/down ResBlocks, removing a separate resample launch, and a paired conv_in kernel reads the loop latent directly. Together these cut memory traffic and kernel launches, at the cost of extra LDS use and more kernel variants.

```diff
diff --git a/include/k22.h b/include/k22.h
--- a/include/k22.h
+++ b/include/k22.h
@@ -154,6 +154,8 @@
                   int dtype, void* stream);
 int k22_qkv_project(const void* x, const void* Wp, const float* bias, void* q_out, void* kall, void* vtall,
                     int B, int H, int T, int S, int K, int bm, int bn, int dtype, void* stream);
+int k22_qkv_project_gn(const void* x_raw, const float* gamma, const float* beta, float eps, void* scratch, const void* Wp, const float* bias,
+                       void* q_out, void* kall, void* vtall, int B, int H, int T, int S, int K, int bm, int stages, int dtype, void* stream);
 int k22_qkv_project_stream(const void* x, const void* Wp, const float* bias, void* q_out, void* kall, void* vtall, void* partial,
                            int B, int H, int T, int S, int K, int bm, int splitk, int dtype, void* stream);
 int k22_linear_smallm(const float* x, const void* W, const float* bias, const float* add, float* out, int M, int N,
diff --git a/kandinsky-2_amd/_lib.py b/kandinsky-2_amd/_lib.py
--- a/kandinsky-2_amd/_lib.py
+++ b/kandinsky-2_amd/_lib.py
@@ -138,6 +138,7 @@
     "k22_groupnorm_scratch_bytes": (_Z, [_I, _I]),
     "k22_attention": (_I, [_P, _P, _P, _P, _P, _I, _I, _I, _I, _I, _P]),
     "k22_qkv_project": (_I, [_P, _P, _P, _P, _P, _P, _I, _I, _I, _I, _I, _I, _I, _I, _P]),
+    "k22_qkv_project_gn": (_I, [_P, _P, _P, _F, _P, _P, _P, _P, _P, _P, _I, _I, _I, _I, _I, _I, _I, _I, _P]),
     "k22_qkv_project_stream": (_I, [_P, _P, _P, _P, _P, _P, _P, _I, _I, _I, _I, _I, _I, _I, _I, _P]),
     "k22_linear_smallm": (_I, [_P, _P, _P, _P, _P, _I, _I, _I, _I, _I, _I, _P]),
     "k22_conv3x3_direct": (_I, [_P, _P, _P, _P, _I, _I, _I, _I, _I, _I, _I, _P]),
diff --git a/kandinsky-2_amd/csrc/capi.hip b/kandinsky-2_amd/csrc/capi.hip
--- a/kandinsky-2_amd/csrc/capi.hip
+++ b/kandinsky-2_amd/csrc/capi.hip
@@ -82,6 +82,7 @@
   if (name && !strcmp(name, "stream_launches")) return stream_launch_count();
   if (name && !strcmp(name, "loop_captures")) return loop_capture_count();
   if (name && !strcmp(name, "loop_launches")) return loop_launch_count();
+  if (name && !strcmp(name, "qkv_gn_fused")) return qkv_gn_fused_count();
   return -1;
 }
 
@@ -375,6 +376,25 @@
   return launch_igemm(p, dtype, reinterpret_cast<hipStream_t>(stream));
 }
 
+int k22_qkv_project_gn(const void* x_raw, const float* gamma, const float* beta, float eps, void* scratch, const void* Wp, const float* bias,
+                       void* q_out, void* kall, void* vtall, int B, int H, int T, int S, int K, int bm, int stages, int dtype, void* stream) {
+  hipStream_t st = reinterpret_cast<hipStream_t>(stream);
+  if (dtype != K22_BF16 && dtype != K22_F16) return k22_set_error(K22_EINVAL, "qkv_project_gn: bf16 / fp16 only");
+  const int C = H * 64, Tkp = (S + T + 63) / 64 * 64;
+  float* part = reinterpret_cast<float*>(scratch);
+  float* coeff = part + (size_t)B * 128 * K * 2;
+  const int rc = launch_gn_stats_coeff(x_raw, nullptr, K, 0, B, T, eps, gamma, beta, nullptr, 0, part, coeff, dtype, st);
+  if (rc) return rc;
+  IgemmParams p = {};
+  p.A0 = x_raw; p.Wp = Wp; p.bias = bias; p.out = q_out; p.kall = kall; p.vtall = vtall;
+  p.M = B * T; p.N = 3 * C; p.Npad = 3 * C; p.Kc = K; p.K0 = K; p.taps = 1; p.lda0 = K; p.lda1 = 0;
+  p.ldo = C; p.ldr = 3 * C; p.out_mode = IG_OUT_QKV; p.act = K22_ACT_NONE; p.splitk = 1; p.force_bm = bm; p.algo = 10; p.stages = stages;
+  p.att_T = T; p.att_S = S; p.att_Tkp = Tkp; p.H = 1; p.W = T;
+  p.gn_coeff = coeff; p.gn_x0 = x_raw; p.gn_C0 = K; p.gn_act = K22_ACT_NONE;
+  if (!gemm8_supported(p, dtype, bm)) return k22_set_error(K22_EINVAL, "qkv_project_gn: unsupported problem (bm = 256 / 128, K % 64 == 0, K <= 1536, 3 * H * 64 % 384 == 0)");
+  return launch_igemm(p, dtype, st);
+}
+
 int k22_qkv_project_stream(const void* x, const void* Wp, const float* bias, void* q_out, void* kall, void* vtall, void* partial,
                            int B, int H, int T, int S, int K, int bm, int splitk, int dtype, void* stream) {
   const int C = H * 64, Tkp = (S + T + 63) / 64 * 64;
diff --git a/kandinsky-2_amd/csrc/conv3_halo.hip b/kandinsky-2_amd/csrc/conv3_halo.hip
--- a/kandinsky-2_amd/csrc/conv3_halo.hip
+++ b/kandinsky-2_amd/csrc/conv3_halo.hip
@@ -236,7 +236,16 @@
   halo_tail<T, BM>(p, acc, smem, bx, bz, img, v0, n0);
 }
 
-template <typename T, int BM, int NST, bool ARAW = false>
+constexpr int gemm8_coef_off(int bm, int nst) {
+  return nst * (bm + HALO_BN) * 128 > bm * (HALO_BN * 4 + 16) ? nst * (bm + HALO_BN) * 128 : bm * (HALO_BN * 4 + 16);
+}
+template <typename T> __device__ __forceinline__ void gemm8_gn_load_cf(float (&cf)[16], const char* tab, int slab, int cch) {
+  const float4* t = reinterpret_cast<const float4*>(tab + slab * (TT<T>::BK * 8) + cch * 64);
+#pragma unroll
+  for (int k = 0; k < 4; ++k) { const float4 q = t[k]; cf[4 * k] = q.x; cf[4 * k + 1] = q.y; cf[4 * k + 2] = q.z; cf[4 * k + 3] = q.w; }
+}
+
+template <typename T, int BM, int NST, bool ARAW = false, bool GNA = false>
 __global__ __launch_bounds__(512) void gemm8_kernel(const IgemmParams p) {
   using TR = TT<T>;
   constexpr int BK = TR::BK, EPC = TR::EPC, KSTEPS = TR::KSTEPS;
@@ -245,6 +254,7 @@
   constexpr int A_SLOTS = BM / 8 / NW, B_SLOTS = BN / 8 / NW, CH = A_SLOTS + B_SLOTS;
   constexpr int A_BYTES = BM * 128, B_BYTES = BN * 128, BUF = A_BYTES + B_BYTES;
   constexpr int GM = 8;
+  static_assert(!GNA || (sizeof(T) == 2 && !ARAW), "gemm8_kernel: the fused GroupNorm-apply operand is a 16-bit form");
   extern __shared__ __attribute__((aligned(16))) char smem[];
 
   const int tid = threadIdx.x, lane = tid & 63;
@@ -320,13 +330,40 @@
   const int sw = (l31 >> 1) & 7;
 
   if (s0 < s1) {
+    [[maybe_unused]] float4 ct0, ct1;
+    [[maybe_unused]] float cf[16];
+    [[maybe_unused]] const char* ctab = smem + gemm8_coef_off(BM, NST);
+    [[maybe_unused]] const int cch = (lane & 7) ^ ((4 * (wave & 1) + (lane >> 4)) & 7);
+    [[maybe_unused]] const int n4 = p.Kc >> 1;
+    if constexpr (GNA) {
+      const float4* src = reinterpret_cast<const float4*>(p.gn_coeff + (int64_t)img * p.Kc * 2);
+      if (tid < n4) ct0 = src[tid];
+      if (tid + 512 < n4) ct1 = src[tid + 512];
+    }
 #pragma unroll
     for (int t = 0; t < NST - 1; ++t) K22_ISSUE_G(s0 + t, t);
+    if constexpr (GNA) {
+      float4* dst = reinterpret_cast<float4*>(smem + gemm8_coef_off(BM, NST));
+      if (tid < n4) dst[tid] = ct0;
+      if (tid + 512 < n4) dst[tid + 512] = ct1;
+      asm volatile("s_waitcnt lgkmcnt(0)" ::: "memory");
+      raw_barrier();
+      gemm8_gn_load_cf<T>(cf, ctab, s0, cch);
+    }
     int cur = 0, fill = NST - 1;
     for (int s = s0; s < s1; ++s) {
       wait_vmcnt<(NST - 2) * CH>();
+      if constexpr (GNA) {
+#pragma unroll
+        for (int i = 0; i < A_SLOTS; ++i) {
+          u32x4_t* a_ = reinterpret_cast<u32x4_t*>(smem + cur * BUF + wave * 1024 + i * NW * 1024 + lane * 16);
+          *a_ = gn_rewrite16(T{}, *a_, cf, K22_ACT_NONE, false);
+        }
+        asm volatile("s_waitcnt lgkmcnt(0)" ::: "memory");
+      }
       raw_barrier();
       K22_ISSUE_G(s + NST - 1, fill);
+      if constexpr (GNA) gemm8_gn_load_cf<T>(cf, ctab, s + 1 < s1 ? s + 1 : s1 - 1, cch);
       const char* St = smem + cur * BUF;
 #pragma unroll
       for (int ks = 0; ks < KSTEPS; ++ks) {
@@ -349,7 +386,7 @@
   halo_tail<T, BM, true>(p, acc, smem, bx, bz, img, v0, n0);
 }
 
-template <typename T, int BM, int NST>
+template <typename T, int BM, int NST, bool GNA = false>
 __global__ __launch_bounds__(512) void gemm8_spec_kernel(const IgemmParams p) {
   using TR = TT<T>;
   static_assert(sizeof(T) == 2, "gemm8_spec_kernel: 16-bit operands");
@@ -400,6 +437,14 @@
       for (int r = 0; r < 16; ++r) acc[mi][ni][r] = 0.f;
 
   if (s0 < s1) {
+    [[maybe_unused]] float4 ct0, ct1;
+    [[maybe_unused]] const int n4 = p.Kc >> 1;
+    [[maybe_unused]] float4* ctab_w = reinterpret_cast<float4*>(smem + gemm8_coef_off(BM, NST));
+    if constexpr (GNA) {
+      const float4* src = reinterpret_cast<const float4*>(p.gn_coeff + (int64_t)img * p.Kc * 2);
+      if (tid < n4) ct0 = src[tid];
+      if (tid + 512 < n4) ct1 = src[tid + 512];
+    }
     if (producer) {
       const int lw = wave - 4;
       const T* __restrict__ A = reinterpret_cast<const T*>(p.A0) + (int64_t)img * HW * p.lda0;
@@ -432,15 +477,44 @@
       }
 #pragma unroll
       for (int t = 0; t < NST - 1; ++t) K22_ISSUE_GS(s0 + t, t);
+      [[maybe_unused]] float cf[16];
+      [[maybe_unused]] const char* ctab = smem + gemm8_coef_off(BM, NST);
+      [[maybe_unused]] const int cch = (lane & 7) ^ ((4 * (lw & 1) + (lane >> 4)) & 7);
+      if constexpr (GNA) {
+        if (tid < n4) ctab_w[tid] = ct0;
+        if (tid + 512 < n4) ctab_w[tid + 512] = ct1;
+        asm volatile("s_waitcnt lgkmcnt(0)" ::: "memory");
+        raw_barrier();
+        gemm8_gn_load_cf<T>(cf, ctab, s0, cch);
+      }
       int fill = NST - 1;
+      [[maybe_unused]] int cur = 0;
       for (int s = s0; s < s1; ++s) {
         wait_vmcnt<(NST - 2) * CH>();
+        if constexpr (GNA) {
+#pragma unroll
+          for (int i = 0; i < A_SLOTS; ++i) {
+            u32x4_t* a_ = reinterpret_cast<u32x4_t*>(smem + cur * BUF + lw * 1024 + i * NWL * 1024 + lane * 16);
+            *a_ = gn_rewrite16(T{}, *a_, cf, K22_ACT_NONE, false);
+          }
+          asm volatile("s_waitcnt lgkmcnt(0)" ::: "memory");
+        }
         raw_barrier();
         K22_ISSUE_GS(s + NST - 1, fill);
+        if constexpr (GNA) {
+          gemm8_gn_load_cf<T>(cf, ctab, s + 1 < s1 ? s + 1 : s1 - 1, cch);
+          cur = (cur + 1 == NST) ? 0 : cur + 1;
+        }
         fill = (fill + 1 == NST) ? 0 : fill + 1;
       }
 #undef K22_ISSUE_GS
     } else {
+      if constexpr (GNA) {
+        if (tid < n4) ctab_w[tid] = ct0;
+        if (tid + 512 < n4) ctab_w[tid + 512] = ct1;
+        asm volatile("s_waitcnt lgkmcnt(0)" ::: "memory");
+        raw_barrier();
+      }
       const int wm = wave >> 1, wn = wave & 1;
       int arow[MI], brow[NI];
 #pragma unroll
@@ -705,36 +779,40 @@
   if (p.N % 8 || p.ldo % 8 || (p.residual && p.ldr % 8) || p.Kc % BK || p.lda0 % 8) return false;
   const int hw = p.H > 0 ? p.H * p.W : p.M;
   if (hw <= 0 || p.M % hw) return false;
-  if (p.out_mode == IG_OUT_QKV && (p.att_T != hw || p.N % 384)) return false;
+  if (p.out_mode == IG_OUT_QKV && (p.att_T != hw || p.N % 192)) return false;
   if ((int64_t)p.M * p.lda0 >= (1ll << 31) || (int64_t)p.Npad * p.Kc >= (1ll << 31)) return false;
+  if (p.gn_coeff != nullptr && !gemm8_gn_supported(p, dtype)) return false;
   return true;
 }
 
-template <typename T, int BM, int NST, bool ARAW = false>
+template <typename T, int BM, int NST, bool ARAW = false, bool GNA = false>
 static int launch_gemm8_cfg(const IgemmParams& p, int splitk, hipStream_t stream) {
   if constexpr (is_x3<T>::value && !ARAW) { if (p.a_raw) return launch_gemm8_cfg<T, BM, NST, true>(p, splitk, stream); }
-  const size_t smem = gemm8_smem_bytes(BM, NST);
+  if constexpr (sizeof(T) == 2 && !GNA) { if (p.gn_coeff != nullptr) return launch_gemm8_cfg<T, BM, NST, false, true>(p, splitk, stream); }
+  static_assert(gemm8_coef_off(BM, NST) == (BM == 256 ? 3 * 384 * 128 : (NST == 2 ? 128 * 528 : 4 * 256 * 128)), "coefficient table offset");
+  const size_t smem = gemm8_smem_bytes(BM, NST) + (GNA ? (size_t)p.Kc * 8 : 0);
   static LdsAttrGuard attr_guard;
-  if (int rc_ = k22_ensure_lds_attr(attr_guard, reinterpret_cast<const void*>(&gemm8_kernel<T, BM, NST, ARAW>), 160 * 1024, __FILE__, __LINE__)) return rc_;
+  if (int rc_ = k22_ensure_lds_attr(attr_guard, reinterpret_cast<const void*>(&gemm8_kernel<T, BM, NST, ARAW, GNA>), 160 * 1024, __FILE__, __LINE__)) return rc_;
   IgemmParams q = p;
   q.splitk = splitk;
   const int hw = p.H > 0 ? p.H * p.W : p.M;
   const int nblocks = (p.M / hw) * gemm8_tiles_per_image(p, BM) * ((p.N + HALO_BN - 1) / HALO_BN) * splitk;
-  hipLaunchKernelGGL((gemm8_kernel<T, BM, NST, ARAW>), dim3(nblocks), dim3(512), smem, stream, q);
+  hipLaunchKernelGGL((gemm8_kernel<T, BM, NST, ARAW, GNA>), dim3(nblocks), dim3(512), smem, stream, q);
   K22_CHECK_LAUNCH();
   return K22_OK;
 }
 
-template <typename T, int BM, int NST>
+template <typename T, int BM, int NST, bool GNA = false>
 static int launch_gemm8_spec_cfg(const IgemmParams& p, int splitk, hipStream_t stream) {
-  const size_t smem = gemm8_smem_bytes(BM, NST);
+  if constexpr (!GNA) { if (p.gn_coeff != nullptr) return launch_gemm8_spec_cfg<T, BM, NST, true>(p, splitk, stream); }
+  const size_t smem = gemm8_smem_bytes(BM, NST) + (GNA ? (size_t)p.Kc * 8 : 0);
   static LdsAttrGuard attr_guard;
-  if (int rc_ = k22_ensure_lds_attr(attr_guard, reinterpret_cast<const void*>(&gemm8_spec_kernel<T, BM, NST>), 160 * 1024, __FILE__, __LINE__)) return rc_;
+  if (int rc_ = k22_ensure_lds_attr(attr_guard, reinterpret_cast<const void*>(&gemm8_spec_kernel<T, BM, NST, GNA>), 160 * 1024, __FILE__, __LINE__)) return rc_;
   IgemmParams q = p;
   q.splitk = splitk;
   const int hw = p.H > 0 ? p.H * p.W : p.M;
   const int nblocks = (p.M / hw) * gemm8_tiles_per_image(p, BM) * ((p.N + HALO_BN - 1) / HALO_BN) * splitk;
-  hipLaunchKernelGGL((gemm8_spec_kernel<T, BM, NST>), dim3(nblocks), dim3(512), smem, stream, q);
+  hipLaunchKernelGGL((gemm8_spec_kernel<T, BM, NST, GNA>), dim3(nblocks), dim3(512), smem, stream, q);
   K22_CHECK_LAUNCH();
   return K22_OK;
 }
diff --git a/kandinsky-2_amd/csrc/elementwise.h b/kandinsky-2_amd/csrc/elementwise.h
--- a/kandinsky-2_amd/csrc/elementwise.h
+++ b/kandinsky-2_amd/csrc/elementwise.h
@@ -22,6 +22,7 @@
   int act;
   const float* coeff;
   void* out;
+  void* raw_out;
   int out_x3;
 };
 struct ConvInParams {
@@ -30,6 +31,7 @@
   void* out;
   int B, H, W, Cin, Cout;
   int img_premul;
+  int pair;
 };
 struct ConvDirectParams {
   const float* x; const float* w; const float* bias; float* y;
diff --git a/kandinsky-2_amd/csrc/elementwise.hip b/kandinsky-2_amd/csrc/elementwise.hip
--- a/kandinsky-2_amd/csrc/elementwise.hip
+++ b/kandinsky-2_amd/csrc/elementwise.hip
@@ -206,10 +206,23 @@
         for (int q = 0; q < 4; ++q) acc += fast ? apply_act_sel<true>(v[q].get(k) * A[k] + Bc[k], p.act) : apply_act_sel<false>(v[q].get(k) * A[k] + Bc[k], p.act);
         r[k] = acc * 0.25f;
       }
+      if (p.raw_out != nullptr) {
+        Vec16<T> ro;
+#pragma unroll
+        for (int k = 0; k < EPV / 2; ++k) {
+          float s0 = 0.f, s1 = 0.f;
+#pragma unroll
+          for (int q = 0; q < 4; ++q) { s0 += v[q].get(2 * k); s1 += v[q].get(2 * k + 1); }
+          ro.set2(k, s0 * 0.25f, s1 * 0.25f);
+        }
+        *reinterpret_cast<decltype(ro.raw)*>(reinterpret_cast<T*>(p.raw_out) + (((int64_t)b * Ho + yo) * Wo + xo) * C + c) = ro.raw;
+      }
     } else {
       const int yi = p.mode == 2 ? yo >> 1 : yo, xi = p.mode == 2 ? xo >> 1 : xo;
       Vec16<T> v;
       v.raw = *reinterpret_cast<const decltype(v.raw)*>(src + ((int64_t)(b * p.H + yi) * p.W + xi) * ld + cs);
+      if (p.mode == 2 && p.raw_out != nullptr)
+        *reinterpret_cast<decltype(v.raw)*>(reinterpret_cast<T*>(p.raw_out) + (((int64_t)b * Ho + yo) * Wo + xo) * C + c) = v.raw;
 #pragma unroll
       for (int k = 0; k < EPV; ++k) r[k] = fast ? apply_act_sel<true>(v.get(k) * A[k] + Bc[k], p.act) : apply_act_sel<false>(v.get(k) * A[k] + Bc[k], p.act);
     }
@@ -297,6 +310,57 @@
           for (int q = 0; q < 3; ++q) acc += w[c * 9 + r * 3 + q] * patch[c][r][px + q];
       out[((int64_t)(b * p.H + y) * p.W + x0 + px) * p.Cout + n] = from_f32<T>(acc);
     }
+  }
+}
+
+constexpr int CONV_IN_PR = 3, CONV_IN_NCH = 3;
+template <typename T>
+__global__ __launch_bounds__(128) void conv_in_pair_kernel(ConvInParams p) {
+  constexpr int CIN = 4, PT = CONV_IN_PT, PW = PT + 2, PR = CONV_IN_PR, PH = PR + 2, NCH = CONV_IN_NCH;
+  __shared__ float patch[CIN][PH][PW];
+  const int tid = threadIdx.x;
+  const int x0 = blockIdx.x * PT, y0 = blockIdx.y * PR, b = blockIdx.z;
+  const int hw = p.H * p.W, half = p.B / 2;
+  for (int i = tid; i < CIN * PH * PW; i += 128) {
+    const int c = i / (PH * PW), r = (i / PW) % PH, xx = i % PW;
+    const int yy = y0 + r - 1, xs = x0 + xx - 1;
+    float v = 0.f;
+    if (yy >= 0 && yy < p.H && xs >= 0 && xs < p.W) v = p.x[((int64_t)b * 4 + c) * hw + (int64_t)yy * p.W + xs];
+    patch[c][r][xx] = v;
+  }
+  __syncthreads();
+  T* out = reinterpret_cast<T*>(p.out);
+  for (int n0 = tid; n0 < p.Cout; n0 += 128 * NCH) {
+    float w[NCH][CIN * 9], bias[NCH];
+#pragma unroll
+    for (int j = 0; j < NCH; ++j) {
+      const int n = n0 + 128 * j < p.Cout ? n0 + 128 * j : n0;
+#pragma unroll
+      for (int k = 0; k < CIN * 9; ++k) w[j][k] = p.w[(int64_t)k * p.Cout + n];
+      bias[j] = p.bias[n];
+    }
+    for (int py = 0; py < PR && y0 + py < p.H; ++py)
+      for (int px = 0; px < PT && x0 + px < p.W; ++px) {
+        float v[CIN * 9];
+#pragma unroll
+        for (int c = 0; c < CIN; ++c)
+#pragma unroll
+          for (int r = 0; r < 3; ++r)
+#pragma unroll
+            for (int q = 0; q < 3; ++q) v[c * 9 + r * 3 + q] = patch[c][py + r][px + q];
+        const int64_t pix = (int64_t)(y0 + py) * p.W + x0 + px;
+#pragma unroll
+        for (int j = 0; j < NCH; ++j) {
+          float acc = bias[j];
+#pragma unroll
+          for (int k = 0; k < CIN * 9; ++k) acc += w[j][k] * v[k];
+          if (n0 + 128 * j < p.Cout) {
+            const T o = from_f32<T>(acc);
+            out[((int64_t)b * hw + pix) * p.Cout + n0 + 128 * j] = o;
+            out[((int64_t)(b + half) * hw + pix) * p.Cout + n0 + 128 * j] = o;
+          }
+        }
+      }
   }
 }
 
@@ -485,7 +549,7 @@
 
 int launch_gn_stats(const GnStatsParams& p, int dtype, hipStream_t s) {
   const int C = p.C0 + p.C1;
-  if (p.groups != 32 || C % 128 != 0 || p.C0 % 4 != 0) return k22_set_error(K22_EINVAL, "gn_stats: need 32 groups, C % 128 == 0");
+  if (p.groups != 32 || C % 32 != 0 || p.C0 % 4 != 0) return k22_set_error(K22_EINVAL, "gn_stats: need 32 groups, C % 32 == 0");
   if (C / 4 > 768) return k22_set_error(K22_EINVAL, "gn_stats: C too large (max 3072)");
   if (C / 4 < 256 && (256 / (C / 4)) * C > 2048) return k22_set_error(K22_EINVAL, "gn_stats: internal LDS bound");
   dim3 grid(p.nsplit, p.B);
@@ -510,6 +574,7 @@
   const int Wo = p.mode == 1 ? p.W / 2 : (p.mode == 2 ? p.W * 2 : p.W);
   const int Hp = Ho + 2 * p.pad, Wp = Wo + 2 * p.pad;
   if (Hp > 65535 || p.B > 65535) return k22_set_error(K22_EINVAL, "gn_apply: tensor too large");
+  if (p.raw_out != nullptr && p.mode != 1 && p.mode != 2) return k22_set_error(K22_EINVAL, "gn_apply: raw_out is the resampled input (mode 1 / 2)");
   dim3 grid((Wp * (C / epv) + 255) / 256, Hp, p.B);
   if (dtype == K22_BF16) hipLaunchKernelGGL(gn_apply_kernel<bf16_t>, grid, dim3(256), 0, s, p);
   else if (dtype == K22_F16) hipLaunchKernelGGL(gn_apply_kernel<f16_t>, grid, dim3(256), 0, s, p);
@@ -528,6 +593,16 @@
   return K22_OK;
 }
 int launch_conv_in(const ConvInParams& p, int dtype, hipStream_t s) {
+  if (p.pair) {
+    if (p.Cin != 4 || p.B < 2 || p.B % 2) return k22_set_error(K22_EINVAL, "conv_in: the shared-input pair is a 4-channel stem with an even batch");
+    const dim3 pgrid((p.W + CONV_IN_PT - 1) / CONV_IN_PT, (p.H + CONV_IN_PR - 1) / CONV_IN_PR, p.B / 2);
+    if (pgrid.y > 65535 || pgrid.z > 65535) return k22_set_error(K22_EINVAL, "conv_in: tensor too large");
+    if (dtype == K22_BF16) hipLaunchKernelGGL(conv_in_pair_kernel<bf16_t>, pgrid, dim3(128), 0, s, p);
+    else if (dtype == K22_F16) hipLaunchKernelGGL(conv_in_pair_kernel<f16_t>, pgrid, dim3(128), 0, s, p);
+    else hipLaunchKernelGGL(conv_in_pair_kernel<float>, pgrid, dim3(128), 0, s, p);
+    K22_CHECK_LAUNCH();
+    return K22_OK;
+  }
   dim3 grid((p.W + CONV_IN_PT - 1) / CONV_IN_PT, p.H, p.B);
   if (p.Cin == 4) {
     if (dtype == K22_BF16) hipLaunchKernelGGL((conv_in_kernel<bf16_t, 4>), grid, dim3(128), 0, s, p);
diff --git a/kandinsky-2_amd/csrc/engine.hip b/kandinsky-2_amd/csrc/engine.hip
--- a/kandinsky-2_amd/csrc/engine.hip
+++ b/kandinsky-2_amd/csrc/engine.hip
@@ -24,6 +24,8 @@
 long loop_launch_count() { return g_loop_launches.load(); }
 static void loop_count_capture() { g_loop_captures.fetch_add(1); }
 static void loop_count_launch() { g_loop_launches.fetch_add(1); }
+static std::atomic<long> g_qkv_gn_fused{0};
+long qkv_gn_fused_count() { return g_qkv_gn_fused.load(); }
 enum : unsigned long long { K22_LOOP_KIND_P = 0, K22_LOOP_KIND_DDIM = 1, K22_LOOP_KIND_PLMS = 2 };
 static unsigned long long loop_key_ptr(const void* p) { return (unsigned long long)(uintptr_t)p; }
 static unsigned long long loop_key_bits(double v) { unsigned long long b; memcpy(&b, &v, 8); return b; }
@@ -67,8 +69,16 @@
   bool hint_set = false;
   int fuse_skip = 1;
   int fuse_gn = 0;
+  int gn_resample = 1;
   struct GnLink { const Tuned* consumer = nullptr; };
   std::deque<GnLink> gn_links;
+  int fuse_qkv_gn = 0;
+  bool link_fuses(const GnLink* link) const {
+    if (link == nullptr || link->consumer == nullptr) return false;
+    const Tuned& t = *link->consumer;
+    if (t.p.taps == 9) return conv3_algo_fuses_gn(t.cfg.algo);
+    return fuse_qkv_gn && gemm8_algo_fuses_gn(t.cfg.algo) && gemm8_gn_supported(t.p, op_dt(t));
+  }
   int stream_frag = 1;
   struct FragJob { const void* W; Slot* slot; int Npad, taps, Kc; };
   std::vector<FragJob> frag_jobs;
@@ -101,6 +111,8 @@
   int hoist_time = 1;
   const float* film_cur = nullptr;
   const float* film_base() const { return film_cur ? film_cur : ptr<float>(s_film); }
+  const float* loop_x = nullptr;
+  int loop_stem = 1;
   struct TimeW { const float* freqs; const float* w0; const float* b0; const float* w2; const float* b2; const void* we; const float* be; int mc, ted, dt; } tw = {};
   int time_rows(const float* t, float* temb, float* e1, float* emb, float* film, int rows, hipStream_t st) {
     int rc = launch_timestep_embedding(t, tw.freqs, temb, rows, tw.mc / 2, st);
@@ -173,15 +185,21 @@
     return K22_OK;
   }
   int loop_model(const LoopRows& lr, const float* cur, const float* timesteps, int call, hipStream_t s) {
-    const size_t half = (size_t)(B / 2) * 4 * H * W * sizeof(float);
-    if (int rc = copy_d2d(ptr(s_xin), cur, half, s)) return rc;
-    if (int rc = copy_d2d(ptr(s_xin) + half, cur, half, s)) return rc;
+    const bool direct = cfg.in_channels == 4 && loop_stem;
+    if (!direct) {
+      const size_t half = (size_t)(B / 2) * 4 * H * W * sizeof(float);
+      if (int rc = copy_d2d(ptr(s_xin), cur, half, s)) return rc;
+      if (int rc = copy_d2d(ptr(s_xin) + half, cur, half, s)) return rc;
+    }
     if (lr.hoist) {
       film_cur = lr.film + (int64_t)call * B * film_total;
     } else {
       if (int rc = copy_d2d(ptr(s_t), timesteps + (size_t)call * B, (size_t)B * 4, s)) return rc;
     }
-    return exec(s);
+    loop_x = direct ? cur : nullptr;
+    const int rc = exec(s);
+    loop_x = nullptr;
+    return rc;
   }
   template <typename F> int loop_run(const std::vector<unsigned long long>& key, const float* timesteps, const float* inpaint_image,
                                      const float* inpaint_mask, int use_graph, hipStream_t st, F body) {
@@ -221,7 +239,7 @@
   int run_ops(hipStream_t st) { return run_ops_range(st, 0, ops.size()); }
 
   void op_gn(OpList& L, const Act& in, const std::string& pfx, int64_t film_off,
-             int act, int mode, int pad, Slot* dst, const GnLink* link = nullptr) {
+             int act, int mode, int pad, Slot* dst, const GnLink* link = nullptr, Slot* raw_dst = nullptr) {
     const int Bn = B, C = in.C(), HW = in.H * in.W;
     const int nsplit = gn_nsplit(Bn, HW);
     const bool fused = in.st0 != nullptr && (in.s1 == nullptr || in.st1 != nullptr);
@@ -235,7 +253,8 @@
     const Act a = in;
     const int dt = sdt;
     const int x3 = k22_is_split(dtype) ? 1 : 0;
-    const double gn_bytes = (double)Bn * HW * C * esz * (fused ? 1.0 : 2.0) + (double)Bn * (Ho + 2 * pad) * (Wo + 2 * pad) * C * esz;
+    const double gn_bytes = (double)Bn * HW * C * esz * (fused ? 1.0 : 2.0) + (double)Bn * (Ho + 2 * pad) * (Wo + 2 * pad) * C * esz +
+                            (raw_dst ? (double)Bn * Ho * Wo * C * esz : 0.0);
     L.push_back(Op([=](hipStream_t st) {
       const void* x0 = ptr(a.s0);
       const void* x1 = a.s1 ? ptr(a.s1) : nullptr;
@@ -259,9 +278,10 @@
       GnApplyParams ap = {};
       ap.x0 = x0; ap.x1 = x1; ap.C0 = a.C0; ap.C1 = a.C1; ap.B = Bn; ap.H = a.H; ap.W = a.W;
       ap.mode = mode; ap.pad = pad; ap.act = act; ap.coeff = ptr<float>(s_coeff); ap.out = ptr(dst); ap.out_x3 = x3;
+      ap.raw_out = raw_dst ? ptr(raw_dst) : nullptr;
       int rc = launch_gn_coeff(cp, Bn, st);
       if (rc) return rc;
-      if (link != nullptr && link->consumer != nullptr && conv3_algo_fuses_gn(link->consumer->cfg.algo)) return K22_OK;
+      if (link_fuses(link)) return K22_OK;
       return launch_gn_apply(ap, dt, st);
     }, OP_GN, 0.0, gn_bytes, fused ? 2 : 3));
   }
@@ -353,7 +373,8 @@
   }
 
   Tuned* op_gemm(OpList& L, const Act& in, int M, int N, const std::string& pfx,
-                 const Act* residual, Slot* dst, int ldo = 0, int out_mode = IG_OUT_ROWMAJOR, Slot* stats = nullptr, bool a_raw = false) {
+                 const Act* residual, Slot* dst, int ldo = 0, int out_mode = IG_OUT_ROWMAJOR, Slot* stats = nullptr, bool a_raw = false,
+                 const Act* gn_in = nullptr, const GnLink* gn_link = nullptr) {
     tuned.emplace_back();
     Tuned* t = &tuned.back();
     t->dt = gemm_dt(out_mode == IG_OUT_QKV);
@@ -376,10 +397,16 @@
     const Act a = in;
     Slot* rs = residual ? residual->s0 : nullptr;
     const int dt = t->dt;
+    Act ga;
+    if (gn_in) ga = *gn_in;
     t->run = [=](hipStream_t st) {
       IgemmParams q = t->p;
       apply_cfg(q, t->cfg);
       q.A0 = ptr(a.s0); q.A1 = a.s1 ? ptr(a.s1) : nullptr;
+      if (gn_in != nullptr && link_fuses(gn_link)) {
+        q.A0 = ptr(ga.s0); q.gn_coeff = ptr<float>(s_coeff); q.gn_x0 = q.A0; q.gn_C0 = ga.C0; q.gn_act = K22_ACT_NONE;
+        g_qkv_gn_fused.fetch_add(1);
+      }
       q.residual = rs ? ptr(rs) : nullptr; q.out = ptr(dst); q.partial = ptr<float>(s_splitk);
       if (t->aux0) { q.kall = ptr(reinterpret_cast<Slot*>(t->aux0)); q.vtall = ptr(reinterpret_cast<Slot*>(t->aux1)); }
       q.stats = t->want_stats ? ptr<float>(stats) : nullptr;
@@ -395,7 +422,9 @@
     const int Wo = updown == 1 ? in.W / 2 : (updown == 2 ? in.W * 2 : in.W);
     GnLink* l1 = nullptr;
     if (fuse_gn && updown == 0) { gn_links.emplace_back(); l1 = &gn_links.back(); }
-    op_gn(ops, in, pfx + ".in_layers.0", -1, K22_ACT_SILU, updown, 1, s_P1, l1);
+    const bool gn_rs = updown != 0 && gn_resample && !k22_is_split(dtype);
+    if (updown) need(s_S, (size_t)B * Ho * Wo * Cin * esz);
+    op_gn(ops, in, pfx + ".in_layers.0", -1, K22_ACT_SILU, updown, 1, s_P1, l1, gn_rs ? s_S : nullptr);
     Tuned* t1 = op_conv(ops, CONV_IN, s_P1, Ho, Wo, Cin, Cout, pfx + ".in_layers.2", nullptr, s_U1, IG_OUT_ROWMAJOR, s_U1st, nullptr, std::string(),
                         l1 ? &in : nullptr, K22_ACT_SILU);
     if (l1) l1->consumer = t1;
@@ -410,9 +439,10 @@
     skip.H = Ho; skip.W = Wo; skip.C0 = Cout;
     if (updown) {
       if (Cin != Cout || in.s1) { if (err.empty()) err = "updown ResBlock with channel change is not supported"; }
-      need(s_S, (size_t)B * Ho * Wo * Cin * esz);
-      const Act a = in; const int Bn = B, dt = sdt;
-      ops.push_back([=](hipStream_t st) { return launch_resample(ptr(a.s0), ptr(s_S), Bn, a.H, a.W, Cin, updown, dt, st); });
+      if (!gn_rs) {
+        const Act a = in; const int Bn = B, dt = sdt;
+        ops.push_back([=](hipStream_t st) { return launch_resample(ptr(a.s0), ptr(s_S), Bn, a.H, a.W, Cin, updown, dt, st); });
+      }
       skip.s0 = s_S;
     } else if (Cin != Cout) {
       IgemmParams probe = {};
@@ -446,7 +476,10 @@
     const int C = in.C0, T = in.H * in.W, Hh = C / 64, S = cfg.ctx_len;
     const int Tk = S + T, Tkp = (Tk + 63) / 64 * 64;
     n_attn++;
-    op_gn(ops, in, pfx + ".norm", -1, K22_ACT_NONE, 0, 0, s_N);
+    GnLink* ln = nullptr;
+    if (fuse_qkv_gn && k22_esz(dtype) == 2 && !in.s1) { gn_links.emplace_back(); ln = &gn_links.back(); }
+    op_gn(ops, in, pfx + ".norm", -1, K22_ACT_NONE, 0, 0, s_N, ln);
+    const size_t gn_op = ops.size() - 1;
     Act n; n.s0 = s_N; n.C0 = C; n.H = in.H; n.W = in.W;
     Slot* kall = new_slot((size_t)B * Hh * Tkp * 64 * esz);
     Slot* vtall = new_slot((size_t)B * Hh * Tkp * 64 * esz);
@@ -465,9 +498,13 @@
     }
     need(s_QKV, (size_t)B * T * C * esz);
     {
-      Tuned* t = op_gemm(ops, n, B * T, 3 * C, pfx + ".qkv", nullptr, s_QKV, C, IG_OUT_QKV);
+      Tuned* t = op_gemm(ops, n, B * T, 3 * C, pfx + ".qkv", nullptr, s_QKV, C, IG_OUT_QKV, nullptr, false, ln ? &in : nullptr, ln);
       t->p.att_T = T; t->p.att_S = S; t->p.att_Tkp = Tkp;
       t->aux0 = kall; t->aux1 = vtall;
+      if (ln) {
+        ln->consumer = t;
+        if (link_fuses(ln)) { ops[gn_op].bytes -= 2.0 * B * T * C * esz; ops[gn_op].kernels -= 1; }
+      }
     }
     need(s_ATT, (size_t)B * T * C * esz);
     ops.push_back(Op([=](hipStream_t st) {
@@ -574,7 +611,8 @@
       const int premul = (hinted || cfg.head_type == 1) ? 1 : 0;
       ops.push_back([=](hipStream_t st) {
         ConvInParams q = cp;
-        q.x = ptr<float>(s_xin); q.img = inpaint ? ptr<float>(s_img) : (hinted ? ptr<float>(s_hint) : nullptr);
+        q.x = loop_x ? loop_x : ptr<float>(s_xin); q.pair = loop_x ? 1 : 0;
+        q.img = inpaint ? ptr<float>(s_img) : (hinted ? ptr<float>(s_hint) : nullptr);
         q.mask = inpaint ? ptr<float>(s_mask) : nullptr; q.img_premul = premul;
         q.out = ptr(d);
         return launch_conv_in(q, dt, st);
@@ -757,6 +795,9 @@
   u->cfg = *cfg; u->set_dtype(cfg->dtype); u->sdt = k22_storage_dtype(cfg->dtype);
   u->stream_frag = env_flag("K22_STREAM", 1);
   u->fuse_gn = env_flag("K22_FUSE_GN", 0);
+  u->fuse_qkv_gn = env_flag("K22_FUSE_QKV_GN", 0);
+  u->loop_stem = env_flag("K22_LOOP_STEM", 1);
+  u->gn_resample = env_flag("K22_GN_RESAMPLE", 1);
   u->fuse_skip = env_flag("K22_FUSE_SKIP", 1);
   u->hoist_time = env_flag("K22_HOIST_TIME", 1);
   const char* xp = getenv("K22_X2_PLAN");
diff --git a/kandinsky-2_amd/csrc/igemm.hip b/kandinsky-2_amd/csrc/igemm.hip
--- a/kandinsky-2_amd/csrc/igemm.hip
+++ b/kandinsky-2_amd/csrc/igemm.hip
@@ -646,8 +646,8 @@
   }
   if (pl.splitk > 1 && p.partial == nullptr) pl.splitk = 1;
   if (p.res_f32 && pl.halo) return k22_set_error(K22_EINVAL, "igemm: fp32 residual is not supported by the halo kernel");
-  if (p.gn_coeff != nullptr && !conv3_algo_fuses_gn(pl.halo))
-    return k22_set_error(K22_EINVAL, "igemm: the fused GroupNorm-apply input needs the specialised halo kernel (algo 11 / 12)");
+  if (p.gn_coeff != nullptr && !conv3_algo_fuses_gn(pl.halo) && !(gemm8_algo_fuses_gn(pl.halo) && gemm8_gn_supported(p, dtype)))
+    return k22_set_error(K22_EINVAL, "igemm: the fused GroupNorm-apply input needs the specialised halo kernel (algo 11 / 12) or, for a 16-bit GEMM, gemm8 (algo 10)");
   if (p.S0 != nullptr && !pl.halo) return k22_set_error(K22_EINVAL, "igemm: the fused 1x1 skip connection needs the halo kernel");
   if (p.stats != nullptr && pl.splitk == 1 && !pl.halo)
     return k22_set_error(K22_EINVAL, "igemm: GroupNorm partial sums requested from a configuration that cannot produce them");
diff --git a/kandinsky-2_amd/csrc/kernels.h b/kandinsky-2_amd/csrc/kernels.h
--- a/kandinsky-2_amd/csrc/kernels.h
+++ b/kandinsky-2_amd/csrc/kernels.h
@@ -73,6 +73,10 @@
 bool gemm8_supported(const IgemmParams& p, int dtype, int bm);
 bool gemm8_spec_supported(int dtype);
 int gemm8_tiles_per_image(const IgemmParams& p, int bm);
+inline bool gemm8_algo_fuses_gn(int algo) { return algo == 10; }
+inline bool gemm8_gn_supported(const IgemmParams& p, int dtype) {
+  return (dtype == K22_BF16 || dtype == K22_F16) && p.taps == 1 && p.K0 == p.Kc && p.Kc <= 1536 && p.splitk <= 1 && p.lda0 == p.Kc && p.H > 0;
+}
 int launch_gemm8(const IgemmParams& p, int dtype, int bm, int splitk, hipStream_t stream);
 bool stream_supported(const IgemmParams& p, int dtype, int mb);
 int stream_mtiles(const IgemmParams& p, int mb);
@@ -80,6 +84,7 @@
 long stream_launch_count();
 long loop_capture_count();
 long loop_launch_count();
+long qkv_gn_fused_count();
 size_t stream_frag_bytes(int Npad, int taps, int Kc, int dtype);
 int launch_stream_repack(const void* W, void* out, int Npad, int taps, int Kc, int dtype, hipStream_t stream);
 void igemm_set_gemm_algo(int v);
```

After: 145.1 steps/s (median of 6 runs). About the same (+0.5%).
